# maxjaritz/mvpnet

Hardware: AMD Instinct MI355X
Metric: chunks/sec (8192 pts, 3x160x120 views) fwd+bwd (higher is better)
Workload: dtype f32; 1 GPU; configs[2]: MVPNet lifting (unproject + pixel k-NN + gather) + FeatureAggregation + PN2SSG full train step (fwd+loss+bwd+Adam), 2D CNN replaced by a resident 64-ch feature map; cfg=mvpnet_3d_unet_resnet34_pn2ssg.yaml, chunks_per_gpu=32, points=8192, views=3x160x120, feature_channels=64, k=3, parallelism=dp1 (one process per GPU, 1 grad all-reduce/step), launch=eager, cpu_affinity=32 logical cpus of 256 (0 .. 183)

## Files before the change

### include/mvp_hip.h

```cpp
#ifndef MVP_HIP_H_
#define MVP_HIP_H_

#include <stddef.h>
#include <stdint.h>

#ifdef __cplusplus
extern "C" {
#endif

typedef void* mvp_stream_t;

#define MVP_OK 0
#define MVP_EINVAL (-1)
#define MVP_EUNSUPPORTED (-2)
#define MVP_ENULL (-3)

const char* mvp_version(void);
const char* mvp_strerror(int code);

int mvp_set_fps_mode(int mode);

int mvp_fps_f32(const float* points, int64_t B, int64_t N, int64_t D, int64_t M, int64_t* index, mvp_stream_t stream);
int mvp_fps_f64(const double* points, int64_t B, int64_t N, int64_t D, int64_t M, int64_t* index, mvp_stream_t stream);
int mvp_fps_shape_f32(const float* points, int64_t B, int64_t N, int64_t D, int64_t M, int64_t* index, int shape, mvp_stream_t stream);
// ... 198 lines not shown
int mvp_gather_rows_backward_csr_f32(const float* grad_out, const int32_t* offsets, const int32_t* slots, const float* weight,
                                     int64_t B, int64_t N, int64_t C, int64_t E, int64_t S, int64_t ld, float* grad_feature,
                                     mvp_stream_t stream);
int mvp_gather_rows_backward_csr_finish_f32(const float* dz, const float* y, const float* mean, const float* invstd, const float* gamma,
                                            const double* stat, int training, const int32_t* offsets, const int32_t* slots, const float* weight,
                                            int64_t B, int64_t N, int64_t C, int64_t E, int64_t S, int64_t ld, float* grad_feature,
                                            mvp_stream_t stream);
int mvp_interp_add_rows_f32(const float* feature, const int64_t* index, const float* weight, const float* add, int64_t B, int64_t N1,
                            int64_t C, int64_t N2, float* out, double* stat, double* partial, mvp_stream_t stream);
int mvp_interp_add_rows_bn_f32(const float* feature, const int64_t* index, const float* weight, const float* add, int64_t B, int64_t N1,
                               int64_t C, int64_t N2, float* out, double* stat, double* partial, float eps, float momentum, float* mean,
                               float* invstd, float* running_mean, float* running_var, int64_t* num_batches_tracked, mvp_stream_t stream);
int mvp_interp_rows_backward_f32(const float* grad_out, const int64_t* index, const float* weight, int64_t B, int64_t N1,
                                 int64_t C, int64_t N2, int64_t ld, float* grad_feature, mvp_stream_t stream);
int mvp_bn_rows_forward_f32(const float* y, const float* gamma, const float* beta, int64_t G, int64_t K, int64_t C,
                            int training, float eps, float momentum, int relu, float* running_mean, float* running_var,
                            double* stat, float* mean, float* invstd, float* out, uint8_t* arg, double* partial,
                            mvp_stream_t stream);
int mvp_bn_rows_backward_f32(const float* dsrc, const float* out, const uint8_t* arg, const float* y, const float* mean,
                             const float* invstd, const float* gamma, const float* beta, int64_t G, int64_t K, int64_t C,
                             int relu, int training, double* stat, float* dy, float* dgamma, float* dbeta, double* partial,
                             mvp_stream_t stream);
int mvp_bn_rows_forward_dropout_f32(const float* y, const float* gamma, const float* beta, int64_t R, int64_t C, int training, float eps,
                                    float momentum, int relu, float* running_mean, float* running_var, double* stat, float* mean,
                                    float* invstd, float* out, double* partial, float drop_p, uint64_t seed, mvp_stream_t stream);
int mvp_bn_rows_backward_dropout_f32(const float* dsrc, const float* y, const float* mean, const float* invstd, const float* gamma,
                                     const float* beta, int64_t R, int64_t C, int relu, int training, double* stat, float* dy,
                                     float* dgamma, float* dbeta, double* partial, float drop_p, uint64_t seed, mvp_stream_t stream);
int mvp_bn_rows_backward_finish_f32(const float* dz, const float* y, const float* mean, const float* invstd,
                                    const float* gamma, const float* beta, int64_t R, int64_t C, int training,
                                    const double* stat, float* dy, float* dgamma, float* dbeta, mvp_stream_t stream);
int mvp_bn_finalize_f32(const double* stat, int64_t R, int64_t C, float eps, float momentum, float* mean, float* invstd,
                        float* running_mean, float* running_var, int64_t* num_batches_tracked, mvp_stream_t stream);
int mvp_sa_fused_forward_f32(const float* zf, const float* xyz, const float* centre, const int64_t* index, const float* wxyz, int64_t B,
                             int64_t N, int64_t M, int64_t K, int64_t C1, const float* bn1_mean, const float* bn1_invstd,
                             const float* bn1_gamma, const float* bn1_beta, const float* W2, int64_t C2, const float* bn2_mean,
                             const float* bn2_invstd, const float* bn2_gamma, const float* bn2_beta, const float* W3, int64_t C3,
                             const float* bn3_mean, const float* bn3_invstd, const float* bn3_gamma, const float* bn3_beta, float* out,
                             uint8_t* arg, mvp_stream_t stream);

int mvp_set_mlp_precision(int terms, int min_width);
int mvp_get_mlp_precision(void);
int mvp_set_mlp_precision_backward(int terms);
int mvp_get_mlp_precision_backward(void);
int mvp_mlp_precision_scope(int terms, int terms_backward);
int mvp_adam_step_f32(void* const* params, const void* const* grads, void* const* exp_avg, void* const* exp_avg_sq, const int64_t* numel,
                      int64_t n, double lr, double beta1, double beta2, double eps, double weight_decay, double step, mvp_stream_t stream);
int mvp_sgd_step_f32(void* const* params, const void* const* grads, void* const* momentum_buf, const int64_t* numel, const uint8_t* first,
                     int64_t n, double lr, double momentum, double dampening, double weight_decay, int nesterov, const float* grad_scale,
                     mvp_stream_t stream);
int64_t mvp_grad_clip_partials_count(const int64_t* numel, int64_t n);
int mvp_grad_sqnorm_partials_f32(const void* const* grads, const int64_t* numel, int64_t n, float* partials, int64_t* n_partials_out,
                                 mvp_stream_t stream);
int mvp_grad_clip_finish_f32(void* const* grads, const int64_t* numel, int64_t n, const float* partials, int64_t n_partials, double max_norm,
                             float* total_norm_out, float* coef_out, mvp_stream_t stream);

int mvp_mlp_forward_bf16(const uint16_t* X, int64_t R, int64_t Cin, int64_t ldx, const float* W, int64_t ldw, int64_t Cout,
                         const float* bias, const float* scale, const float* shift, int relu, uint16_t* Y, int64_t ldy,
                         mvp_stream_t stream);

int mvp_set_mlp_stream(int on);

int mvp_mlp_forward_f32(const float* X, int64_t R, int64_t Cin, int64_t ldx, const float* W, int64_t ldw, int64_t Cout,
                        const float* act_mean, const float* act_invstd, const float* act_gamma, const float* act_beta,
                        const float* bias, float* Y, double* stat, double* partial, mvp_stream_t stream);
int mvp_mlp_forward_bn_f32(const float* X, int64_t R, int64_t Cin, int64_t ldx, const float* W, int64_t ldw, int64_t Cout,
                           const float* act_mean, const float* act_invstd, const float* act_gamma, const float* act_beta, float* Y,
                           double* stat, double* partial, float eps, float momentum, float* mean, float* invstd, float* running_mean,
                           float* running_var, int64_t* num_batches_tracked, mvp_stream_t stream);
int mvp_mlp_forward_rel_bn_f32(const float* X, int64_t R, int64_t Cin, int64_t ldx, const float* W, int64_t ldw, int64_t Cout, const float* rel,
                               const float* wrel, float* Y, double* stat, double* partial, float eps, float momentum, float* mean,
                               float* invstd, float* running_mean, float* running_var, int64_t* num_batches_tracked, mvp_stream_t stream);
int mvp_relation4_rows_f32(const float* src_xyz, const float* tgt_xyz, int64_t R, int64_t K, float* out, mvp_stream_t stream);
int mvp_mlp_forward_pool_f32(const float* X, int64_t R, int64_t Cin, int64_t ldx, const float* W, int64_t ldw, int64_t Cout,
                             const float* act_mean, const float* act_invstd, const float* act_gamma, const float* act_beta, float* ymax,
                             float* ymin, uint8_t* amax, uint8_t* amin, double* stat, double* partial, float eps, float momentum,
                             float* mean, float* invstd, float* running_mean, float* running_var, int64_t* num_batches_tracked,
                             mvp_stream_t stream);
int mvp_pool_finalize_f32(const float* ymax, const float* ymin, const uint8_t* amax, const uint8_t* amin, const float* mean,
                          const float* invstd, const float* gamma, const float* beta, int64_t G, int64_t C, int relu, float* out,
                          uint8_t* arg, float* ysel, mvp_stream_t stream);
int mvp_pool_backward_stats_f32(const float* dout, const float* out, const float* ysel, const float* mean, const float* invstd,
                                int64_t G, int64_t C, int relu, double* stat, double* partial, mvp_stream_t stream);
int mvp_mlp_input_grad_f32(const float* dY, int64_t R, int64_t Cout, const float* W, int64_t Cin, const float* y_prev,
                           const float* mean, const float* invstd, const float* gamma, const float* beta, float* dZ,
                           double* stat, double* partial, mvp_stream_t stream);
int mvp_mlp_input_grad_dropout_f32(const float* dY, int64_t R, int64_t Cout, const float* W, int64_t Cin, const float* y_prev,
                                   const float* mean, const float* invstd, const float* gamma, const float* beta, float drop_p,
                                   uint64_t drop_seed, float* dZ, double* stat, double* partial, mvp_stream_t stream);

int64_t mvp_mlp_layer_backward_partial_count(int64_t R, int64_t Cp);
int mvp_mlp_layer_backward_f32(const float* G, const float* Yi, const float* mean_i, const float* invstd_i, const float* gamma_i,
                               const double* stat_i, float* dgamma_i, float* dbeta_i, int training, const float* X, int64_t ldx,
                               const float* act_mean, const float* act_invstd, const float* act_gamma, const float* act_beta,
                               const float* W, int64_t ldw, int64_t R, int64_t C, int64_t Cp, float* dW, int64_t lddw, float* dZ,
                               double* stat_prev, double* partial, const float* pool_dout, const float* pool_out,
                               const uint8_t* pool_arg, mvp_stream_t stream);
int mvp_mlp_layer_backward_ws_f32(const float* G, const float* Yi, const float* mean_i, const float* invstd_i, const float* gamma_i,
                               const double* stat_i, float* dgamma_i, float* dbeta_i, int training, const float* X, int64_t ldx,
                               const float* act_mean, const float* act_invstd, const float* act_gamma, const float* act_beta,
                               const float* W, int64_t ldw, int64_t R, int64_t C, int64_t Cp, float* dW, int64_t lddw, float* dZ,
                               double* stat_prev, double* partial, const float* pool_dout, const float* pool_out,
                               const uint8_t* pool_arg, float* workspace, int64_t workspace_floats, mvp_stream_t stream);
int mvp_mlp_layer_backward_wide_p_f32(const float* G, const float* Yi, const float* mean_i, const float* invstd_i, const float* gamma_i,
                                      const float* beta_i, const double* stat_i, float* dgamma_i, float* dbeta_i, int training, int mode,
                                      float drop_p, uint64_t drop_seed, const float* X, int64_t ldx, const float* act_mean,
                                      const float* act_invstd, const float* act_gamma, const float* act_beta, const float* W, int64_t ldw,
                                      int64_t R, int64_t C, int64_t Cp, float* dW, int64_t lddw, float* dZ, double* stat_prev, int* ticket,
                                      float* workspace, int64_t workspace_floats, int precision, int precision_backward, mvp_stream_t stream);
int mvp_mlp_layer_backward_wide_pooled_p_f32(const float* G, const float* Yi, const float* mean_i, const float* invstd_i, const float* gamma_i,
                                             const float* beta_i, const double* stat_i, float* dgamma_i, float* dbeta_i, int training, int mode,
                                             int64_t pool_k, float drop_p, uint64_t drop_seed, const float* X, int64_t ldx, const float* act_mean,
                                             const float* act_invstd, const float* act_gamma, const float* act_beta, const float* W, int64_t ldw,
                                             int64_t R, int64_t C, int64_t Cp, float* dW, int64_t lddw, float* dZ, double* stat_prev, int* ticket,
                                             float* workspace, int64_t workspace_floats, int precision, int precision_backward, mvp_stream_t stream);
int mvp_mlp_weight_grad_finish_p_f32(const float* dZ, const float* Y, const float* mean, const float* invstd, const float* gamma, const double* stat,
                                     int training, const float* X, int64_t R, int64_t Cout, int64_t Cin, int64_t ldx, float* dW, int64_t lddw,
                                     float* workspace, int64_t workspace_floats, int precision, int precision_backward, mvp_stream_t stream);
int mvp_mlp_weight_grad_finish_rel_p_f32(const float* dZ, const float* Y, const float* mean, const float* invstd, const float* gamma, const double* stat,
                                         int training, const float* X, int64_t R, int64_t Cout, int64_t Cin, int64_t ldx, const float* REL, float* dW,
                                         float* dWrel, int64_t lddw, int precision, int precision_backward, mvp_stream_t stream);
int mvp_mlp_weight_grad_finish_act_p_f32(const float* dZ, const float* Y, const float* mean, const float* invstd, const float* gamma, const double* stat,
                                         int training, const float* X, int64_t R, int64_t Cout, int64_t Cin, int64_t ldx, const float* act_mean,
                                         const float* act_invstd, const float* act_gamma, const float* act_beta, float* dW, int64_t lddw,
                                         float* workspace, int64_t workspace_floats, int precision, int precision_backward, mvp_stream_t stream);
int64_t mvp_mlp_input_grad_wide_workspace_bytes(int64_t C, int64_t Cp);
int mvp_mlp_input_grad_wide_p_f32(const float* G, const float* Yi, const float* mean_i, const float* invstd_i, const float* gamma_i,
                                  const double* stat_i, float* dgamma_i, float* dbeta_i, int training, const float* X, int64_t ldx,
                                  const float* act_mean, const float* act_invstd, const float* act_gamma, const float* act_beta, const float* W,
                                  int64_t ldw, int64_t R, int64_t C, int64_t Cp, float* dZ, double* stat_prev, void* workspace,
                                  int64_t workspace_bytes, int precision, int precision_backward, mvp_stream_t stream);
int mvp_mlp_weight_grad_f32(const float* dY, const float* X, int64_t R, int64_t Cout, int64_t Cin, int64_t ldx,
                            const float* act_mean, const float* act_invstd, const float* act_gamma, const float* act_beta,
                            float* dW, int64_t lddw, mvp_stream_t stream);
int64_t mvp_mlp_weight_grad_workspace_floats(void);
int mvp_mlp_weight_grad_ws_f32(const float* dY, const float* X, int64_t R, int64_t Cout, int64_t Cin, int64_t ldx,
                               const float* act_mean, const float* act_invstd, const float* act_gamma, const float* act_beta,
                               float* dW, int64_t lddw, float* workspace, int64_t workspace_floats, mvp_stream_t stream);

int mvp_sa_train_forward_f32(int stage, const float* zf, const float* xyz, const float* centre, const int64_t* index, const float* wxyz,
                             int64_t B, int64_t N, int64_t M, int64_t K, int64_t C1, const float* bn1_mean, const float* bn1_invstd,
                             const float* bn1_gamma, const float* bn1_beta, const float* W2, int64_t C2, const float* bn2_mean,
                             const float* bn2_invstd, const float* bn2_gamma, const float* bn2_beta, const float* W3, int64_t C3,
                             double* stat, float eps, float momentum, float* mean, float* invstd, float* running_mean,
                             float* running_var, int64_t* num_batches_tracked, float* ymax, float* ymin, uint8_t* amax, uint8_t* amin,
                             mvp_stream_t stream);
int mvp_sa_train_backward_f32(int layer, const float* zf, const float* xyz, const float* centre, const int64_t* index, const float* wxyz,
                              int64_t B, int64_t N, int64_t M, int64_t K, int64_t C1, const float* bn1_mean, const float* bn1_invstd,
                              const float* bn1_gamma, const float* bn1_beta, const float* W2, int64_t C2, const float* bn2_mean,
                              const float* bn2_invstd, const float* bn2_gamma, const float* bn2_beta, const float* W3, int64_t C3,
                              const float* mean_i, const float* invstd_i, const float* gamma_i, const double* stat_i, float* dgamma_i,
                              float* dbeta_i, int training, const float* G, const float* pool_dout, const float* pool_out,
                              const uint8_t* pool_arg, float* dW, int64_t lddw, float* dZ, double* stat_prev, float* tsum, mvp_stream_t stream);
int mvp_sa_train_backward1_f32(const float* dz1, const int32_t* offsets, const int32_t* slots, const float* zf, const float* dsum,
                               const float* wxyz, const float* tsum, const double* zsum, const double* gsum, int64_t B, int64_t N, int64_t M,
                               int64_t K, int64_t C1, const float* mean, const float* invstd, const float* gamma, const double* stat,
                               int training, float* dgamma, float* dbeta, float* gz, float* dWxyz, int64_t lddw, mvp_stream_t stream);
int mvp_sa_geom_sums_f32(const int32_t* offsets, const int32_t* slots, const float* xyz, const float* centre, int64_t B, int64_t N, int64_t M,
                         int64_t K, float* dsum, double* gsum, mvp_stream_t stream);
int mvp_sa_train_stats1_f32(const float* zf, const float* dsum, const float* wxyz, const double* gsum, int64_t B, int64_t N, int64_t M, int64_t K,
                            int64_t C1, double* stat, double* zsum, float eps, float momentum, float* mean, float* invstd, float* running_mean,
                            float* running_var, int64_t* num_batches_tracked, mvp_stream_t stream);
int mvp_sa_train_stats1_ws_f32(const float* zf, const float* dsum, const float* wxyz, const double* gsum, int64_t B, int64_t N, int64_t M, int64_t K,
                               int64_t C1, double* stat, double* zsum, float eps, float momentum, float* mean, float* invstd, float* running_mean,
                               float* running_var, int64_t* num_batches_tracked, double* scratch, int64_t scratch_doubles, mvp_stream_t stream);

int mvp_mlp_forward_p_f32(const float* X, int64_t R, int64_t Cin, int64_t ldx, const float* W, int64_t ldw, int64_t Cout, const
    float* act_mean, const float* act_invstd, const float* act_gamma, const float* act_beta, const float* bias, float* Y,
    double* stat, double* partial, int precision, int precision_backward, mvp_stream_t stream);
int mvp_mlp_forward_bn_p_f32(const float* X, int64_t R, int64_t Cin, int64_t ldx, const float* W, int64_t ldw, int64_t Cout,
    const float* act_mean, const float* act_invstd, const float* act_gamma, const float* act_beta, float* Y, double* stat,
    double* partial, float eps, float momentum, float* mean, float* invstd, float* running_mean, float* running_var, int64_t*
    num_batches_tracked, int precision, int precision_backward, mvp_stream_t stream);
int mvp_mlp_forward_rel_bn_p_f32(const float* X, int64_t R, int64_t Cin, int64_t ldx, const float* W, int64_t ldw, int64_t Cout,
    const float* rel, const float* wrel, float* Y, double* stat, double* partial, float eps, float momentum, float* mean, float*
    invstd, float* running_mean, float* running_var, int64_t* num_batches_tracked, int precision, int precision_backward,
    mvp_stream_t stream);
int mvp_mlp_forward_pool_p_f32(const float* X, int64_t R, int64_t Cin, int64_t ldx, const float* W, int64_t ldw, int64_t Cout,
    const float* act_mean, const float* act_invstd, const float* act_gamma, const float* act_beta, float* ymax, float* ymin,
    uint8_t* amax, uint8_t* amin, double* stat, double* partial, float eps, float momentum, float* mean, float* invstd, float*
    running_mean, float* running_var, int64_t* num_batches_tracked, int precision, int precision_backward, mvp_stream_t stream);
int mvp_mlp_input_grad_p_f32(const float* dY, int64_t R, int64_t Cout, const float* W, int64_t Cin, const float* y_prev, const
    float* mean, const float* invstd, const float* gamma, const float* beta, float* dZ, double* stat, double* partial, int
    precision, int precision_backward, mvp_stream_t stream);
int mvp_mlp_input_grad_dropout_p_f32(const float* dY, int64_t R, int64_t Cout, const float* W, int64_t Cin, const float* y_prev, const
    float* mean, const float* invstd, const float* gamma, const float* beta, float drop_p, uint64_t drop_seed, float* dZ, double* stat,
    double* partial, int precision, int precision_backward, mvp_stream_t stream);
int mvp_mlp_weight_grad_p_f32(const float* dY, const float* X, int64_t R, int64_t Cout, int64_t Cin, int64_t ldx, const float*
    act_mean, const float* act_invstd, const float* act_gamma, const float* act_beta, float* dW, int64_t lddw, int precision,
    int precision_backward, mvp_stream_t stream);
int mvp_mlp_weight_grad_ws_p_f32(const float* dY, const float* X, int64_t R, int64_t Cout, int64_t Cin, int64_t ldx, const
    float* act_mean, const float* act_invstd, const float* act_gamma, const float* act_beta, float* dW, int64_t lddw, float*
    workspace, int64_t workspace_floats, int precision, int precision_backward, mvp_stream_t stream);
int mvp_mlp_layer_backward_p_f32(const float* G, const float* Yi, const float* mean_i, const float* invstd_i, const float*
    gamma_i, const double* stat_i, float* dgamma_i, float* dbeta_i, int training, const float* X, int64_t ldx, const float*
    act_mean, const float* act_invstd, const float* act_gamma, const float* act_beta, const float* W, int64_t ldw, int64_t R,
    int64_t C, int64_t Cp, float* dW, int64_t lddw, float* dZ, double* stat_prev, double* partial, const float* pool_dout, const
    float* pool_out, const uint8_t* pool_arg, int precision, int precision_backward, mvp_stream_t stream);
int mvp_mlp_layer_backward_ws_p_f32(const float* G, const float* Yi, const float* mean_i, const float* invstd_i, const float*
    gamma_i, const double* stat_i, float* dgamma_i, float* dbeta_i, int training, const float* X, int64_t ldx, const float*
    act_mean, const float* act_invstd, const float* act_gamma, const float* act_beta, const float* W, int64_t ldw, int64_t R,
    int64_t C, int64_t Cp, float* dW, int64_t lddw, float* dZ, double* stat_prev, double* partial, const float* pool_dout, const
    float* pool_out, const uint8_t* pool_arg, float* workspace, int64_t workspace_floats, int precision, int precision_backward,
    mvp_stream_t stream);
int mvp_sa_fused_forward_p_f32(const float* zf, const float* xyz, const float* centre, const int64_t* index, const float* wxyz,
    int64_t B, int64_t N, int64_t M, int64_t K, int64_t C1, const float* bn1_mean, const float* bn1_invstd, const float*
    bn1_gamma, const float* bn1_beta, const float* W2, int64_t C2, const float* bn2_mean, const float* bn2_invstd, const float*
    bn2_gamma, const float* bn2_beta, const float* W3, int64_t C3, const float* bn3_mean, const float* bn3_invstd, const float*
    bn3_gamma, const float* bn3_beta, float* out, uint8_t* arg, int precision, int precision_backward, mvp_stream_t stream);

int mvp_sa_train_forward_p_f32(int stage, const float* zf, const float* xyz, const float* centre, const int64_t* index, const
    float* wxyz, int64_t B, int64_t N, int64_t M, int64_t K, int64_t C1, const float* bn1_mean, const float* bn1_invstd, const
    float* bn1_gamma, const float* bn1_beta, const float* W2, int64_t C2, const float* bn2_mean, const float* bn2_invstd, const
    float* bn2_gamma, const float* bn2_beta, const float* W3, int64_t C3, double* stat, float eps, float momentum, float* mean,
    float* invstd, float* running_mean, float* running_var, int64_t* num_batches_tracked, float* ymax, float* ymin, uint8_t*
    amax, uint8_t* amin, int precision, int precision_backward, mvp_stream_t stream);
int mvp_sa_train_backward_p_f32(int layer, const float* zf, const float* xyz, const float* centre, const int64_t* index, const
    float* wxyz, int64_t B, int64_t N, int64_t M, int64_t K, int64_t C1, const float* bn1_mean, const float* bn1_invstd, const
    float* bn1_gamma, const float* bn1_beta, const float* W2, int64_t C2, const float* bn2_mean, const float* bn2_invstd, const
    float* bn2_gamma, const float* bn2_beta, const float* W3, int64_t C3, const float* mean_i, const float* invstd_i, const
    float* gamma_i, const double* stat_i, float* dgamma_i, float* dbeta_i, int training, const float* G, const float* pool_dout,
    const float* pool_out, const uint8_t* pool_arg, float* dW, int64_t lddw, float* dZ, double* stat_prev, float* tsum, int precision, int
    precision_backward, mvp_stream_t stream);

int mvp_pn2_plan_f32(const float* xyz, int64_t B, int64_t N, int64_t levels, const int64_t* centroids, const float* radius,
                     const int64_t* neighbours, const int32_t* geom, int fps_shape, int flags, float knn_eps, void* const* buffers,
                     int64_t n_buffers, void* const* events, int* fps_status, mvp_stream_t stream);

int mvp_vote_accumulate_f32(const float* logit, int64_t ld_r, int64_t ld_c, const int64_t* chunk_ind, int64_t n,
                            int64_t C, float* sum, int32_t* count, mvp_stream_t stream);
int mvp_vote_gather_f32(const float* logit, int64_t ld_chunk, int64_t ld_r, int64_t ld_c, const int64_t* chunk_offsets, int64_t num_chunks,
                        const int32_t* point_offsets, const int32_t* point_slots, int64_t n_pts, int64_t C, float* sum, int32_t* count,
                        mvp_stream_t stream);
int mvp_vote_finish_f32(const float* sum, const int32_t* count, int64_t n_pts, int64_t C, float* mean, int64_t* label,
                        mvp_stream_t stream);
int64_t mvp_vote_nearest_workspace(int64_t V, int64_t nb);
int mvp_vote_nearest_f32(const float* points, int64_t n, const float* key, int64_t V, int64_t nb, const float* logit, int64_t ld_vote,
                         int64_t ld_r, int64_t ld_c, int64_t C, float* sum, int64_t* nn_index, int32_t* swept, void* workspace,
                         int64_t workspace_bytes, mvp_stream_t stream);

int mvp_seg_loss_f32(const float* logit, int64_t B, int64_t C, int64_t N, int64_t ld_b, int64_t ld_c, int64_t ld_n,
                     const int64_t* label, const float* weight, int64_t ignore_index, double* acc, float* loss, mvp_stream_t stream);
int mvp_seg_loss_backward_f32(const float* logit, int64_t B, int64_t C, int64_t N, int64_t ld_b, int64_t ld_c, int64_t ld_n,
                              const int64_t* label, const float* weight, int64_t ignore_index, const double* acc,
                              const float* grad_out, float* grad_logit, int64_t gld_b, int64_t gld_c, int64_t gld_n,
                              mvp_stream_t stream);
int mvp_seg_confusion_f32(const float* logit, int64_t B, int64_t C, int64_t N, int64_t ld_b, int64_t ld_c, int64_t ld_n,
                          const int64_t* label, int64_t ignore_index, int64_t* mat, mvp_stream_t stream);

#ifdef __cplusplus
}
#endif
#endif
```

### mvpnet_amd/_lib.py

```python
import ctypes
import os

import torch

_HERE = os.path.dirname(os.path.abspath(__file__))
LIB_PATH = os.environ.get('MVP_LIBRARY') or os.path.join(_HERE, 'libmvp_hip.so')
_lib = None
MLP_PRECISIONS = {'fp32': 0, 'bf16': 1, 'bf16x3': 3, 'bf16x6': 6}

_i64 = ctypes.c_int64
_ptr = ctypes.c_void_p
_f32 = ctypes.c_float

_SIGNATURES = {
    'mvp_fps_f32': [_ptr, _i64, _i64, _i64, _i64, _ptr, _ptr],
    'mvp_fps_f64': [_ptr, _i64, _i64, _i64, _i64, _ptr, _ptr],
    'mvp_fps_shape_f32': [_ptr, _i64, _i64, _i64, _i64, _ptr, ctypes.c_int, _ptr],
    'mvp_fps_shape_f64': [_ptr, _i64, _i64, _i64, _i64, _ptr, ctypes.c_int, _ptr],
    'mvp_fps_checked_f32': [_ptr, _i64, _i64, _i64, _i64, _ptr, ctypes.c_int, _ptr, _ptr],
    'mvp_fps_centroid_levels_f32': [_ptr, _ptr, _i64, _i64, _i64, _i64, _i64, _ptr, _ptr, _ptr],
    'mvp_ball_query_f32': [_ptr, _ptr, _i64, _i64, _i64, _f32, _i64, _ptr, _ptr],
    'mvp_ball_query_f64': [_ptr, _ptr, _i64, _i64, _i64, _f32, _i64, _ptr, _ptr],
    'mvp_ball_query_distance_f32': [_ptr, _ptr, _i64, _i64, _i64, _f32, _i64, _ptr, _ptr, _ptr],
    'mvp_ball_query_distance_f64': [_ptr, _ptr, _i64, _i64, _i64, _f32, _i64, _ptr, _ptr, _ptr],
    'mvp_ball_query_grid_f32': [_ptr, _ptr, _i64, _i64, _i64, _f32, _i64, _ptr, _ptr, _ptr, _i64, _ptr],
    'mvp_knn3_grid_f32': [_ptr, _ptr, _i64, _i64, _i64, _f32, _ptr, _ptr, _ptr, _ptr, _i64, _ptr],
    'mvp_group_points_forward_strided_f32': [_ptr, _i64, _i64, _i64, _ptr, _i64, _i64, _i64, _i64, _i64, _ptr, _ptr],
    'mvp_group_points_backward_strided_f32': [_ptr, _i64, _i64, _i64, _i64, _ptr, _i64, _i64, _i64, _i64, _i64, _ptr, _ptr],
    'mvp_interpolate_forward_strided_f32': [_ptr, _i64, _i64, _i64, _ptr, _ptr, _i64, _i64, _i64, _i64, _ptr, _ptr],
    'mvp_interpolate_backward_strided_f32': [_ptr, _i64, _i64, _i64, _ptr, _ptr, _i64, _i64, _i64, _i64, _ptr, _ptr],
    'mvp_group_points_forward_strided_f64': [_ptr, _i64, _i64, _i64, _ptr, _i64, _i64, _i64, _i64, _i64, _ptr, _ptr],
    'mvp_group_points_forward_strided_bf16': [_ptr, _i64, _i64, _i64, _ptr, _i64, _i64, _i64, _i64, _i64, _ptr, _ptr],
    'mvp_group_points_backward_strided_f64': [_ptr, _i64, _i64, _i64, _i64, _ptr, _i64, _i64, _i64, _i64, _i64, _ptr, _ptr],
    'mvp_group_points_backward_strided_bf16': [_ptr, _i64, _i64, _i64, _i64, _ptr, _i64, _i64, _i64, _i64, _i64, _ptr, _ptr],
    'mvp_interpolate_forward_strided_f64': [_ptr, _i64, _i64, _i64, _ptr, _ptr, _i64, _i64, _i64, _i64, _ptr, _ptr],
    'mvp_interpolate_forward_strided_bf16': [_ptr, _i64, _i64, _i64, _ptr, _ptr, _i64, _i64, _i64, _i64, _ptr, _ptr],
    'mvp_interpolate_backward_strided_f64': [_ptr, _i64, _i64, _i64, _ptr, _ptr, _i64, _i64, _i64, _i64, _ptr, _ptr],
    'mvp_interpolate_backward_strided_bf16': [_ptr, _i64, _i64, _i64, _ptr, _ptr, _i64, _i64, _i64, _i64, _ptr, _ptr],
    'mvp_group_points_forward_f32': [_ptr, _ptr, _i64, _i64, _i64, _i64, _i64, _ptr, _ptr],
    'mvp_group_points_forward_f64': [_ptr, _ptr, _i64, _i64, _i64, _i64, _i64, _ptr, _ptr],
    'mvp_group_points_forward_bf16': [_ptr, _ptr, _i64, _i64, _i64, _i64, _i64, _ptr, _ptr],
    'mvp_group_points_backward_f32': [_ptr, _ptr, _i64, _i64, _i64, _i64, _i64, _ptr, _ptr],
    'mvp_group_points_backward_f64': [_ptr, _ptr, _i64, _i64, _i64, _i64, _i64, _ptr, _ptr],
    'mvp_group_points_backward_bf16': [_ptr, _ptr, _i64, _i64, _i64, _i64, _i64, _ptr, _ptr],
    'mvp_knn_distance_f32': [_ptr, _ptr, _i64, _i64, _i64, _i64, _ptr, _ptr, _ptr],
    'mvp_knn_distance_f64': [_ptr, _ptr, _i64, _i64, _i64, _i64, _ptr, _ptr, _ptr],
    'mvp_knn3_weights_f32': [_ptr, _ptr, _i64, _i64, _i64, _f32, _ptr, _ptr, _ptr, _ptr],
    'mvp_interpolate_forward_f32': [_ptr, _ptr, _ptr, _i64, _i64, _i64, _i64, _ptr, _ptr],
    'mvp_interpolate_forward_f64': [_ptr, _ptr, _ptr, _i64, _i64, _i64, _i64, _ptr, _ptr],
    'mvp_interpolate_forward_bf16': [_ptr, _ptr, _ptr, _i64, _i64, _i64, _i64, _ptr, _ptr],
    'mvp_interpolate_backward_f32': [_ptr, _ptr, _ptr, _i64, _i64, _i64, _i64, _ptr, _ptr],
    'mvp_interpolate_backward_f64': [_ptr, _ptr, _ptr, _i64, _i64, _i64, _i64, _ptr, _ptr],
    'mvp_interpolate_backward_bf16': [_ptr, _ptr, _ptr, _i64, _i64, _i64, _i64, _ptr, _ptr],
    'mvp_unproject_f32': [_ptr, _ptr, _ptr, _ptr, _i64, _i64, _i64, _i64, _ptr, _ptr, _ptr],
    'mvp_unproject_u16': [_ptr, _ptr, _ptr, _ptr, _i64, _i64, _i64, _i64, _ptr, _ptr, _ptr],
    'mvp_pixel_knn_bruteforce_f32': [_ptr, _ptr, _ptr, _i64, _i64, _i64, _i64, _ptr, _ptr, _ptr],
    'mvp_pixel_knn_projective_f32': [_ptr, _ptr, _ptr, _ptr, _ptr, _i64, _i64, _i64, _i64, _i64, _i64, _ptr, _ptr, _ptr],
    'mvp_lift_gather_f32': [_ptr, _ptr, _ptr, _i64, _i64, _i64, _i64, _i64, _ptr, _ptr, _ptr],
    'mvp_lift_gather_backward_f32': [_ptr, _ptr, _i64, _i64, _i64, _i64, _i64, _ptr, _ptr],
    'mvp_lift_f32': [_ptr, ctypes.c_int, _ptr, _ptr, _ptr, _ptr, _ptr, _ptr, _i64, _i64, _i64, _i64, _i64, _i64, _i64, _ptr,
                     _ptr, _ptr, _ptr, _ptr, _ptr, _ptr],
    'mvp_lift_aug_f32': [_ptr, ctypes.c_int, _ptr, _ptr, _ptr, _ptr, _ptr, _ptr, _i64, _i64, _i64, _i64, _i64, _i64, _i64, _ptr,
                         _ptr, _ptr, _ptr, _ptr, _ptr, _ptr, _ptr, _ptr, _ptr],
    'mvp_rotate_rows_f32': [_ptr, _ptr, _i64, _i64, _ptr, _ptr],
    'mvp_copy_slices_f32': [_ptr, _i64, _ptr],
    'mvp_group_rows_f32': [_ptr, _ptr, _ptr, _ptr, _i64, _i64, _i64, _i64, _i64, _i64, _ptr, _ptr],
    'mvp_group_rows_backward_f32': [_ptr, _ptr, _i64, _i64, _i64, _i64, _i64, _i64, _ptr, _ptr],
    'mvp_group_lin_rows_f32': [_ptr, _ptr, _ptr, _ptr, _ptr, _i64, _i64, _i64, _i64, _i64, _ptr, _ptr, _ptr, _ptr, _ptr],
    'mvp_group_lin_rows_bn_f32': [_ptr, _ptr, _ptr, _ptr, _ptr, _i64, _i64, _i64, _i64, _i64, _ptr, _ptr, _ptr, _ptr, _f32, _f32, _ptr, _ptr, _ptr, _ptr, _ptr, _ptr],
    'mvp_colstats_f32': [_ptr, _i64, _i64, _ptr, _ptr, _ptr],
    'mvp_relation_rows_f32': [_ptr, _ptr, _ptr, _i64, _i64, _i64, _ptr, _ptr],
    'mvp_interp_rows_f32': [_ptr, _ptr, _ptr, _i64, _i64, _i64, _i64, _i64, _ptr, _ptr],
    'mvp_mlp_forward_bf16': [_ptr, _i64, _i64, _i64, _ptr, _i64, _i64, _ptr, _ptr, _ptr, ctypes.c_int, _ptr, _i64, _ptr],
    'mvp_adam_step_f32': [_ptr, _ptr, _ptr, _ptr, _ptr, _i64] + [ctypes.c_double] * 6 + [_ptr],
    'mvp_sgd_step_f32': [_ptr, _ptr, _ptr, _ptr, _ptr, _i64] + [ctypes.c_double] * 4 + [ctypes.c_int, _ptr, _ptr],
    'mvp_grad_sqnorm_partials_f32': [_ptr, _ptr, _i64, _ptr, _ptr, _ptr],
    'mvp_grad_clip_finish_f32': [_ptr, _ptr, _i64, _ptr, _i64, ctypes.c_double, _ptr, _ptr, _ptr],
    'mvp_csr_build_i64': [_ptr, _i64, _i64, _i64, _ptr, _ptr, _ptr, _ptr],
    'mvp_csr_build_sorted_i64': [_ptr, _i64, _i64, _i64, _ptr, _ptr, _ptr, _ptr],
    'mvp_gather_rows_backward_csr_f32': [_ptr, _ptr, _ptr, _ptr, _i64, _i64, _i64, _i64, _i64, _i64, _ptr, _ptr],
    'mvp_gather_rows_backward_csr_finish_f32': [_ptr, _ptr, _ptr, _ptr, _ptr, _ptr, ctypes.c_int, _ptr, _ptr, _ptr, _i64, _i64, _i64, _i64, _i64, _i64, _ptr, _ptr],
    'mvp_interp_add_rows_f32': [_ptr, _ptr, _ptr, _ptr, _i64, _i64, _i64, _i64, _ptr, _ptr, _ptr, _ptr],
    'mvp_interp_add_rows_bn_f32': [_ptr, _ptr, _ptr, _ptr, _i64, _i64, _i64, _i64, _ptr, _ptr, _ptr, _f32, _f32, _ptr, _ptr, _ptr, _ptr, _ptr, _ptr],
    'mvp_interp_rows_backward_f32': [_ptr, _ptr, _ptr, _i64, _i64, _i64, _i64, _i64, _ptr, _ptr],
    'mvp_bn_rows_forward_f32': [_ptr, _ptr, _ptr, _i64, _i64, _i64, ctypes.c_int, _f32, _f32, ctypes.c_int, _ptr, _ptr, _ptr, _ptr,
                                _ptr, _ptr, _ptr, _ptr, _ptr],
    'mvp_bn_rows_backward_f32': [_ptr, _ptr, _ptr, _ptr, _ptr, _ptr, _ptr, _ptr, _i64, _i64, _i64, ctypes.c_int, ctypes.c_int, _ptr,
                                 _ptr, _ptr, _ptr, _ptr, _ptr],
    'mvp_bn_rows_forward_dropout_f32': [_ptr, _ptr, _ptr, _i64, _i64, ctypes.c_int, _f32, _f32, ctypes.c_int, _ptr, _ptr, _ptr, _ptr, _ptr, _ptr,
                                        _ptr, _f32, ctypes.c_uint64, _ptr],
    'mvp_bn_rows_backward_dropout_f32': [_ptr, _ptr, _ptr, _ptr, _ptr, _ptr, _i64, _i64, ctypes.c_int, ctypes.c_int, _ptr, _ptr, _ptr, _ptr,
                                         _ptr, _f32, ctypes.c_uint64, _ptr],
    'mvp_bn_rows_backward_finish_f32': [_ptr, _ptr, _ptr, _ptr, _ptr, _ptr, _i64, _i64, ctypes.c_int, _ptr, _ptr, _ptr, _ptr, _ptr],
    'mvp_bn_finalize_f32': [_ptr, _i64, _i64, _f32, _f32, _ptr, _ptr, _ptr, _ptr, _ptr, _ptr],
    'mvp_mlp_weight_grad_f32': [_ptr, _ptr, _i64, _i64, _i64, _i64, _ptr, _ptr, _ptr, _ptr, _ptr, _i64, _ptr],
    'mvp_mlp_weight_grad_ws_f32': [_ptr, _ptr, _i64, _i64, _i64, _i64, _ptr, _ptr, _ptr, _ptr, _ptr, _i64, _ptr, _i64, _ptr],
    'mvp_mlp_input_grad_f32': [_ptr, _i64, _i64, _ptr, _i64, _ptr, _ptr, _ptr, _ptr, _ptr, _ptr, _ptr, _ptr, _ptr],
    'mvp_mlp_input_grad_dropout_f32': [_ptr, _i64, _i64, _ptr, _i64, _ptr, _ptr, _ptr, _ptr, _ptr, _f32, ctypes.c_uint64, _ptr, _ptr, _ptr, _ptr],
    'mvp_mlp_layer_backward_f32': [_ptr, _ptr, _ptr, _ptr, _ptr, _ptr, _ptr, _ptr, ctypes.c_int, _ptr, _i64, _ptr, _ptr, _ptr, _ptr, _ptr, _i64,
                                   _i64, _i64, _i64, _ptr, _i64, _ptr, _ptr, _ptr, _ptr, _ptr, _ptr, _ptr],
    'mvp_mlp_layer_backward_ws_f32': [_ptr, _ptr, _ptr, _ptr, _ptr, _ptr, _ptr, _ptr, ctypes.c_int, _ptr, _i64, _ptr, _ptr, _ptr, _ptr, _ptr, _i64,
                                   _i64, _i64, _i64, _ptr, _i64, _ptr, _ptr, _ptr, _ptr, _ptr, _ptr, _ptr, _i64, _ptr],
    'mvp_mlp_forward_pool_f32': [_ptr, _i64, _i64, _i64, _ptr, _i64, _i64, _ptr, _ptr, _ptr, _ptr, _ptr, _ptr, _ptr, _ptr, _ptr, _ptr, _f32, _f32,
                                 _ptr, _ptr, _ptr, _ptr, _ptr, _ptr],
    'mvp_pool_finalize_f32': [_ptr, _ptr, _ptr, _ptr, _ptr, _ptr, _ptr, _ptr, _i64, _i64, ctypes.c_int, _ptr, _ptr, _ptr, _ptr],
    'mvp_pool_backward_stats_f32': [_ptr, _ptr, _ptr, _ptr, _ptr, _i64, _i64, ctypes.c_int, _ptr, _ptr, _ptr],
    'mvp_sa_fused_forward_f32': [_ptr, _ptr, _ptr, _ptr, _ptr, _i64, _i64, _i64, _i64, _i64, _ptr, _ptr, _ptr, _ptr, _ptr, _i64, _ptr, _ptr, _ptr,
                                 _ptr, _ptr, _i64, _ptr, _ptr, _ptr, _ptr, _ptr, _ptr, _ptr],
    'mvp_sa_train_forward_f32': [ctypes.c_int, _ptr, _ptr, _ptr, _ptr, _ptr, _i64, _i64, _i64, _i64, _i64, _ptr, _ptr, _ptr, _ptr, _ptr, _i64, _ptr, _ptr,
                                 _ptr, _ptr, _ptr, _i64, _ptr, _f32, _f32, _ptr, _ptr, _ptr, _ptr, _ptr, _ptr, _ptr, _ptr, _ptr, _ptr],
    'mvp_sa_train_backward_f32': [ctypes.c_int, _ptr, _ptr, _ptr, _ptr, _ptr, _i64, _i64, _i64, _i64, _i64, _ptr, _ptr, _ptr, _ptr, _ptr, _i64, _ptr, _ptr,
                                  _ptr, _ptr, _ptr, _i64, _ptr, _ptr, _ptr, _ptr, _ptr, _ptr, ctypes.c_int, _ptr, _ptr, _ptr, _ptr, _ptr, _i64, _ptr, _ptr,
                                  _ptr, _ptr],
    'mvp_sa_train_backward1_f32': [_ptr, _ptr, _ptr, _ptr, _ptr, _ptr, _ptr, _ptr, _ptr, _i64, _i64, _i64, _i64, _i64, _ptr, _ptr, _ptr, _ptr,
                                   ctypes.c_int, _ptr, _ptr, _ptr, _ptr, _i64, _ptr],
    'mvp_pn2_plan_f32': [_ptr, _i64, _i64, _i64, _ptr, _ptr, _ptr, _ptr, ctypes.c_int, ctypes.c_int, _f32, _ptr, _i64, _ptr, _ptr, _ptr],
    'mvp_sa_geom_sums_f32': [_ptr, _ptr, _ptr, _ptr, _i64, _i64, _i64, _i64, _ptr, _ptr, _ptr],
    'mvp_sa_train_stats1_f32': [_ptr, _ptr, _ptr, _ptr, _i64, _i64, _i64, _i64, _i64, _ptr, _ptr, _f32, _f32, _ptr, _ptr, _ptr, _ptr, _ptr, _ptr],
    'mvp_sa_train_stats1_ws_f32': [_ptr, _ptr, _ptr, _ptr, _i64, _i64, _i64, _i64, _i64, _ptr, _ptr, _f32, _f32, _ptr, _ptr, _ptr, _ptr, _ptr, _ptr, _i64, _ptr],
    'mvp_mlp_forward_bn_f32': [_ptr, _i64, _i64, _i64, _ptr, _i64, _i64, _ptr, _ptr, _ptr, _ptr, _ptr, _ptr, _ptr, _f32, _f32, _ptr, _ptr, _ptr,
                               _ptr, _ptr, _ptr],
    'mvp_mlp_forward_rel_bn_f32': [_ptr, _i64, _i64, _i64, _ptr, _i64, _i64, _ptr, _ptr, _ptr, _ptr, _ptr, _f32, _f32, _ptr, _ptr, _ptr, _ptr, _ptr, _ptr],
    'mvp_relation4_rows_f32': [_ptr, _ptr, _i64, _i64, _ptr, _ptr],
    'mvp_mlp_forward_f32': [_ptr, _i64, _i64, _i64, _ptr, _i64, _i64, _ptr, _ptr, _ptr, _ptr, _ptr, _ptr, _ptr, _ptr, _ptr],
    'mvp_vote_accumulate_f32': [_ptr, _i64, _i64, _ptr, _i64, _i64, _ptr, _ptr, _ptr],
    'mvp_vote_gather_f32': [_ptr, _i64, _i64, _i64, _ptr, _i64, _ptr, _ptr, _i64, _i64, _ptr, _ptr, _ptr],
    'mvp_vote_finish_f32': [_ptr, _ptr, _i64, _i64, _ptr, _ptr, _ptr],
    'mvp_vote_nearest_f32': [_ptr, _i64, _ptr, _i64, _i64, _ptr, _i64, _i64, _i64, _i64, _ptr, _ptr, _ptr, _ptr, _i64, _ptr],
    'mvp_seg_loss_f32': [_ptr, _i64, _i64, _i64, _i64, _i64, _i64, _ptr, _ptr, _i64, _ptr, _ptr, _ptr],
    'mvp_seg_loss_backward_f32': [_ptr, _i64, _i64, _i64, _i64, _i64, _i64, _ptr, _ptr, _i64, _ptr, _ptr, _ptr, _i64, _i64, _i64, _ptr],
    'mvp_seg_confusion_f32': [_ptr, _i64, _i64, _i64, _i64, _i64, _i64, _ptr, _i64, _ptr, _ptr],
    'mvp_frame_overlap_f32': [_ptr, _ptr, _ptr, _ptr, _i64, _i64, _i64, _i64, _f32, _ptr, _ptr],
    'mvp_frame_overlap_u16': [_ptr, _ptr, _ptr, _ptr, _i64, _i64, _i64, _i64, _f32, _ptr, _ptr],
    'mvp_select_frames_u32': [_ptr, _ptr, _i64, _i64, _i64, _i64, _ptr, _ptr, _ptr],
    'mvp_select_frames_ranges_u32': [_ptr, _ptr, _ptr, _ptr, _i64, _i64, _i64, _i64, _ptr, _ptr, _ptr],
    'mvp_sample_chunks_f32': [_ptr] * 6 + [_i64] * 6 + [ctypes.c_double] * 5 + [ctypes.c_int, ctypes.c_uint64] + [_ptr] * 9 + [_i64, _ptr],
    'mvp_sample_scenes_f32': [_ptr, _ptr] + [_i64] * 4 + [ctypes.c_uint64] + [_ptr] * 4 + [_i64, _ptr],
    'mvp_gather_cloud_f32': [_ptr] * 7 + [_i64] * 4 + [_ptr] * 4,
    'mvp_scene_chunks_count_f32': [_ptr, _i64, _ptr, _i64] + [ctypes.c_double] * 4 + [_ptr, _ptr, _ptr],
    'mvp_scene_chunks_fill_f32': [_ptr, _i64, _ptr, _i64] + [ctypes.c_double] * 4 + [_ptr, _ptr, _i64, _ptr, _i64, _ptr, _i64, _ptr, _ptr, _ptr],
    'mvp_pack_chunks_f32': [_ptr, _i64, _ptr, _i64, _ptr, _i64, _ptr, _ptr, _ptr, _ptr, ctypes.c_uint64, _ptr, _i64, _ptr],
    'mvp_prepare_frames_u8': [_ptr, _i64, _i64, _i64, _ptr, _i64, _ptr, _ptr, _ptr, _ptr, ctypes.c_int, _ptr, _ptr, _ptr],
    'mvp_resize_bilinear_table': [_i64, _i64, _ptr, _ptr, _ptr, _ptr],
    'mvp_resize_nearest_table': [_i64, _i64, _ptr],
    'mvp_resize_frames_u8': [_ptr, _i64, _i64, _i64, _ptr, _i64, _i64, _i64, _ptr, _ptr, _ptr, _ptr],
    'mvp_prepare_labels_u16': [_ptr, _i64, _i64, _i64, _ptr, _i64, _i64, _i64, _ptr, _ptr, _ptr, _ptr, _i64, _i64, _ptr, _ptr],
}
for _n in ['mvp_mlp_forward_f32', 'mvp_mlp_forward_bn_f32', 'mvp_mlp_forward_rel_bn_f32', 'mvp_mlp_forward_pool_f32', 'mvp_mlp_input_grad_f32', 'mvp_mlp_input_grad_dropout_f32',
           'mvp_mlp_weight_grad_f32', 'mvp_mlp_weight_grad_ws_f32', 'mvp_mlp_layer_backward_f32', 'mvp_mlp_layer_backward_ws_f32',
           'mvp_sa_fused_forward_f32', 'mvp_sa_train_forward_f32', 'mvp_sa_train_backward_f32']:
    _SIGNATURES[_n[:-4] + '_p_f32'] = _SIGNATURES[_n][:-1] + [ctypes.c_int, ctypes.c_int, _ptr]
_SIGNATURES['mvp_mlp_layer_backward_wide_p_f32'] = [_ptr] * 9 + [ctypes.c_int, ctypes.c_int, _f32, ctypes.c_uint64, _ptr, _i64, _ptr, _ptr, _ptr, _ptr, _ptr, _i64,
                                                    _i64, _i64, _i64, _ptr, _i64, _ptr, _ptr, _ptr, _ptr, _i64, ctypes.c_int, ctypes.c_int, _ptr]
_SIGNATURES['mvp_mlp_layer_backward_wide_pooled_p_f32'] = [_ptr] * 9 + [ctypes.c_int, ctypes.c_int, _i64, _f32, ctypes.c_uint64, _ptr, _i64, _ptr, _ptr, _ptr, _ptr, _ptr, _i64,
                                                           _i64, _i64, _i64, _ptr, _i64, _ptr, _ptr, _ptr, _ptr, _i64, ctypes.c_int, ctypes.c_int, _ptr]
_SIGNATURES['mvp_mlp_weight_grad_finish_p_f32'] = [_ptr] * 6 + [ctypes.c_int, _ptr, _i64, _i64, _i64, _i64, _ptr, _i64, _ptr, _i64, ctypes.c_int, ctypes.c_int, _ptr]
_SIGNATURES['mvp_mlp_weight_grad_finish_rel_p_f32'] = [_ptr] * 6 + [ctypes.c_int, _ptr, _i64, _i64, _i64, _i64, _ptr, _ptr, _ptr, _i64, ctypes.c_int, ctypes.c_int, _ptr]
_SIGNATURES['mvp_mlp_weight_grad_finish_act_p_f32'] = [_ptr] * 6 + [ctypes.c_int, _ptr, _i64, _i64, _i64, _i64, _ptr, _ptr, _ptr, _ptr, _ptr, _i64, _ptr, _i64, ctypes.c_int,
                                                        ctypes.c_int, _ptr]
_SIGNATURES['mvp_mlp_input_grad_wide_p_f32'] = [_ptr] * 8 + [ctypes.c_int, _ptr, _i64, _ptr, _ptr, _ptr, _ptr, _ptr, _i64, _i64, _i64, _i64, _ptr, _ptr, _ptr, _i64,
                                                 ctypes.c_int, ctypes.c_int, _ptr]
EXPORTS = ['mvp_version', 'mvp_strerror', 'mvp_lift_workspace_bytes', 'mvp_ball_query_grid_workspace', 'mvp_knn3_grid_workspace', 'mvp_vote_nearest_workspace', 'mvp_sample_chunks_workspace', 'mvp_sample_scenes_workspace', 'mvp_prepare_frames_workspace', 'mvp_mlp_weight_grad_workspace_floats', 'mvp_mlp_input_grad_wide_workspace_bytes', 'mvp_group_lin_partial_count', 'mvp_colstats_partial_count', 'mvp_grad_clip_partials_count',
           'mvp_set_mlp_precision', 'mvp_get_mlp_precision', 'mvp_mlp_layer_backward_partial_count', 'mvp_set_mlp_stream', 'mvp_set_mlp_precision_backward', 'mvp_get_mlp_precision_backward', 'mvp_mlp_precision_scope', 'mvp_set_fps_mode', 'mvp_fps_debug_spin_limit', 'mvp_fps_last_kernel'] + sorted(_SIGNATURES)


def lib():
    global _lib
    if _lib is None:
        if not os.path.exists(LIB_PATH):
            raise RuntimeError('libmvp_hip.so is not built: run `python -c "import __graft_entry__ as g; g.build()"` '
                               'or `make -C mvpnet_amd/csrc` ({})'.format(LIB_PATH))
        handle = ctypes.CDLL(LIB_PATH)
        handle.mvp_version.restype = ctypes.c_char_p
        handle.mvp_strerror.restype = ctypes.c_char_p
        handle.mvp_strerror.argtypes = [ctypes.c_int]
        handle.mvp_lift_workspace_bytes.restype = ctypes.c_int64
        handle.mvp_lift_workspace_bytes.argtypes = [_i64, _i64, _i64, _i64, _i64]
        handle.mvp_ball_query_grid_workspace.restype = ctypes.c_int64
        handle.mvp_ball_query_grid_workspace.argtypes = [_i64, _i64, _i64]
        handle.mvp_knn3_grid_workspace.restype = ctypes.c_int64
        handle.mvp_knn3_grid_workspace.argtypes = [_i64, _i64, _i64]
        handle.mvp_vote_nearest_workspace.restype = ctypes.c_int64
        handle.mvp_vote_nearest_workspace.argtypes = [_i64, _i64]
        handle.mvp_sample_chunks_workspace.restype = ctypes.c_int64
        handle.mvp_sample_chunks_workspace.argtypes = [_i64, _i64, _i64, _i64]
        handle.mvp_sample_scenes_workspace.restype = ctypes.c_int64
        handle.mvp_sample_scenes_workspace.argtypes = [_i64, _i64, _i64]
        handle.mvp_prepare_frames_workspace.restype = ctypes.c_size_t
        handle.mvp_prepare_frames_workspace.argtypes = [_i64]
        handle.mvp_group_lin_partial_count.restype = ctypes.c_int64
        handle.mvp_group_lin_partial_count.argtypes = [_i64, _i64, _i64, _i64]
        handle.mvp_mlp_weight_grad_workspace_floats.restype = ctypes.c_int64
        handle.mvp_mlp_weight_grad_workspace_floats.argtypes = []
        handle.mvp_mlp_input_grad_wide_workspace_bytes.restype = ctypes.c_int64
        handle.mvp_mlp_input_grad_wide_workspace_bytes.argtypes = [ctypes.c_int64, ctypes.c_int64]
        handle.mvp_colstats_partial_count.restype = ctypes.c_int64
        handle.mvp_colstats_partial_count.argtypes = [_i64, _i64]
        handle.mvp_grad_clip_partials_count.restype = ctypes.c_int64
        handle.mvp_grad_clip_partials_count.argtypes = [_ptr, _i64]
        handle.mvp_set_mlp_precision.restype = ctypes.c_int
        handle.mvp_set_mlp_precision.argtypes = [ctypes.c_int, ctypes.c_int]
        handle.mvp_get_mlp_precision.restype = ctypes.c_int
        handle.mvp_get_mlp_precision.argtypes = []
        handle.mvp_mlp_layer_backward_partial_count.restype = ctypes.c_int64
        handle.mvp_mlp_layer_backward_partial_count.argtypes = [_i64, _i64]
        for name, argtypes in _SIGNATURES.items():
            fn = getattr(handle, name)
            fn.argtypes = argtypes
            fn.restype = ctypes.c_int
        _lib = handle
        handle.mvp_set_mlp_stream.restype = ctypes.c_int
        handle.mvp_set_mlp_stream.argtypes = [ctypes.c_int]
        handle.mvp_set_fps_mode.restype = ctypes.c_int
        handle.mvp_set_fps_mode.argtypes = [ctypes.c_int]
        handle.mvp_fps_debug_spin_limit.restype = ctypes.c_int
        handle.mvp_fps_debug_spin_limit.argtypes = [ctypes.c_int]
        handle.mvp_fps_last_kernel.restype = ctypes.c_int
        handle.mvp_fps_last_kernel.argtypes = []
        if os.environ.get('MVP_MLP_STREAM') is not None:
            handle.mvp_set_mlp_stream(int(os.environ['MVP_MLP_STREAM']))
        handle.mvp_set_mlp_precision_backward.restype = ctypes.c_int
        handle.mvp_set_mlp_precision_backward.argtypes = [ctypes.c_int]
        handle.mvp_get_mlp_precision_backward.restype = ctypes.c_int
        handle.mvp_get_mlp_precision_backward.argtypes = []
        handle.mvp_mlp_precision_scope.restype = ctypes.c_int
        handle.mvp_mlp_precision_scope.argtypes = [ctypes.c_int, ctypes.c_int]
        if os.environ.get('MVP_MLP_PRECISION_BWD'):
            check(handle.mvp_set_mlp_precision_backward(MLP_PRECISIONS[os.environ['MVP_MLP_PRECISION_BWD']]), 'mvp_set_mlp_precision_backward')
        env = os.environ.get('MVP_MLP_PRECISION')
        if env:
            set_mlp_precision(env, int(os.environ.get('MVP_MLP_MIN_WIDTH', '0')))
    return _lib




def set_mlp_precision(name, min_width=0):
    if name not in MLP_PRECISIONS:
        raise ValueError('mlp precision must be one of {}'.format(sorted(MLP_PRECISIONS)))
    check(lib().mvp_set_mlp_precision(MLP_PRECISIONS[name], int(min_width)), 'mvp_set_mlp_precision')
    global _mlp_min_width
    _mlp_min_width = int(min_width)


_mlp_min_width = 0


def mlp_min_width():
    return _mlp_min_width


def set_mlp_precision_backward(name):
    if name not in ('bf16', 'bf16x3', 'bf16x6'):
        raise ValueError("backward mlp precision must be 'bf16', 'bf16x3' or 'bf16x6'")
    check(lib().mvp_set_mlp_precision_backward(MLP_PRECISIONS[name]), 'mvp_set_mlp_precision_backward')


class mlp_precision:

    def __init__(self, forward=None, backward=None):
        self.terms = -1 if forward is None else MLP_PRECISIONS[forward]
        self.bwd = -1 if backward is None else MLP_PRECISIONS[backward]
        if self.bwd == 0:
            raise ValueError("backward mlp precision must be 'bf16', 'bf16x3' or 'bf16x6'")

    def __enter__(self):
        old = lib().mvp_mlp_precision_scope(self.terms, self.bwd)
        if old < 0:
            check(old, 'mvp_mlp_precision_scope')
        self.old = (old // 16 - 1, old % 16 - 1)
        return self

    def __exit__(self, *exc):
        lib().mvp_mlp_precision_scope(*self.old)


def current_precision():
    h = lib()
    return (h.mvp_get_mlp_precision(), h.mvp_get_mlp_precision_backward())


def get_mlp_precision():
    terms = lib().mvp_get_mlp_precision()
    return {v: k for k, v in MLP_PRECISIONS.items()}[terms]


_FPS_STATUS = {}


def fps_status(device):
    t = _FPS_STATUS.get(device)
    if t is None:
        t = _FPS_STATUS[device] = torch.zeros(1, dtype=torch.int32, device=device)
    return t


def fps_timed_out(device=None, reset=False):
    device = torch.device('cuda', torch.cuda.current_device()) if device is None else torch.device(device)
    t = _FPS_STATUS.get(device)
    if t is None:
        return False
    hit = bool(int(t.item()))
    if reset:
        t.zero_()
    return hit


def check(code, what):
    if code != 0:
        raise RuntimeError('{} failed: {} (code {})'.format(what, lib().mvp_strerror(code).decode(), code))


def stream_of(t):
    return ctypes.c_void_p(torch.cuda.current_stream(t.device).cuda_stream)


def ptr(t):
    return None if t is None else t.data_ptr()


def ptr_at(t, element_offset):
    return t.data_ptr() + int(element_offset) * t.element_size()


def require_gpu(*tensors):
    for t in tensors:
        if t is None:
            continue
        if not t.is_cuda:
            raise RuntimeError('mvpnet_amd ops run on the GPU only (got a {} tensor); there is no CPU fallback'.format(t.device))
        if not t.is_contiguous():
            raise RuntimeError('tensor must be contiguous')


def suffix(t):
    if t.dtype == torch.float32:
        return 'f32'
    if t.dtype == torch.float64:
        return 'f64'
    raise RuntimeError('expected a float32 or float64 tensor, got {}'.format(t.dtype))


def value_suffix(t):
    return 'bf16' if t.dtype == torch.bfloat16 else suffix(t)


_FN = {}
_raw_stream = getattr(torch._C, '_cuda_getCurrentRawStream', None)
_raw_device = getattr(torch._C, '_cuda_getDevice', None)


def _fn(name):
    f = _FN.get(name)
    if f is None:
        f = _FN[name] = getattr(_lib if _lib is not None else lib(), name)
    return f


DW_WORKSPACE = os.environ.get('MVP_DETERMINISTIC', '0') == '1'


def set_deterministic(flag):
    global DW_WORKSPACE
    old, DW_WORKSPACE = DW_WORKSPACE, bool(flag)
    return old


_DW_WS = {}
_DW_WS_NAMES = {'mvp_mlp_weight_grad_f32': 'mvp_mlp_weight_grad_ws_f32', 'mvp_mlp_layer_backward_f32': 'mvp_mlp_layer_backward_ws_f32'}


def dw_workspace(index, stream_handle):
    ws = _DW_WS.get((index, stream_handle))
    if ws is None:
        ws = _DW_WS[(index, stream_handle)] = torch.empty(lib().mvp_mlp_weight_grad_workspace_floats(), dtype=torch.float32,
                                                          device=torch.device('cuda', index))
    return ws


def current_dw_workspace(device):
    if not DW_WORKSPACE:
        return None, 0
    index = device.index
    handle = _raw_stream(index) if (_raw_stream is not None and index == _raw_device()) else torch.cuda.current_stream(device).cuda_stream
    ws = dw_workspace(index, handle)
    return ws.data_ptr(), ws.numel()


def _with_dw_workspace(index, stream_handle, args):
    ws = dw_workspace(index, stream_handle)
    return args + (ws.data_ptr(), ws.numel())


def call_on(stream, name, *args, prec=None):
    if DW_WORKSPACE and name in _DW_WS_NAMES:
        name, args = _DW_WS_NAMES[name], _with_dw_workspace(stream.device.index, stream.cuda_stream, args)
    if prec is not None:
        name, args = name[:-4] + '_p_f32', args + prec
    code = _fn(name)(*args, stream.cuda_stream)
    if code != 0:
        check(code, name)


def call(name, tensor_for_device, *args, prec=None):
    index = tensor_for_device.device.index
    if DW_WORKSPACE and name in _DW_WS_NAMES:
        handle = _raw_stream(index) if _raw_stream is not None else torch.cuda.current_stream(tensor_for_device.device).cuda_stream
        name, args = _DW_WS_NAMES[name], _with_dw_workspace(index, handle, args)
    if prec is not None:
        name, args = name[:-4] + '_p_f32', args + prec
    if _raw_stream is not None and index == _raw_device():
        code = _fn(name)(*args, _raw_stream(index))
    elif index == torch.cuda.current_device():
        code = _fn(name)(*args, torch.cuda.current_stream(tensor_for_device.device).cuda_stream)
    else:
        with torch.cuda.device(tensor_for_device.device):
            code = _fn(name)(*args, stream_of(tensor_for_device))
    if code != 0:
        check(code, name)
```

### mvpnet_amd/csrc/mlp_prec.hip

```cpp
#include "mlp_common.h"

namespace {
struct PrecisionArg {
  int old_terms, old_bwd;
  bool ok;
  PrecisionArg(int terms, int bwd) : old_terms(tl_mlp_terms), old_bwd(tl_mlp_terms_bwd) {
    ok = (terms == -1 || terms == 0 || terms == 1 || terms == 3 || terms == 6) && (bwd == -1 || bwd == 1 || bwd == 3 || bwd == 6);
    if (ok && terms >= 0) tl_mlp_terms = terms;
    if (ok && bwd >= 0) tl_mlp_terms_bwd = bwd;
  }
  ~PrecisionArg() {
    tl_mlp_terms = old_terms;
    tl_mlp_terms_bwd = old_bwd;
  }
};
}

#define MVP_WITH_PRECISION(call)             \
  PrecisionArg scope(precision, precision_backward); \
  if (!scope.ok) return MVP_EINVAL;          \
  return call

MVP_API int mvp_mlp_forward_p_f32(const float* X, int64_t R, int64_t Cin, int64_t ldx, const float* W, int64_t ldw, int64_t Cout,
                                  const float* act_mean, const float* act_invstd, const float* act_gamma, const float* act_beta,
                                  const float* bias, float* Y, double* stat, double* partial, int precision, int precision_backward,
                                  mvp_stream_t stream) {
  MVP_WITH_PRECISION(mvp_mlp_forward_f32(X, R, Cin, ldx, W, ldw, Cout, act_mean, act_invstd, act_gamma, act_beta, bias, Y, stat, partial, stream));
}
MVP_API int mvp_mlp_forward_bn_p_f32(const float* X, int64_t R, int64_t Cin, int64_t ldx, const float* W, int64_t ldw, int64_t Cout,
                                     const float* act_mean, const float* act_invstd, const float* act_gamma, const float* act_beta, float* Y,
                                     double* stat, double* partial, float eps, float momentum, float* mean, float* invstd,
                                     float* running_mean, float* running_var, int64_t* num_batches_tracked, int precision,
                                     int precision_backward, mvp_stream_t stream) {
  MVP_WITH_PRECISION(mvp_mlp_forward_bn_f32(X, R, Cin, ldx, W, ldw, Cout, act_mean, act_invstd, act_gamma, act_beta, Y, stat, partial, eps, momentum,
                                            mean, invstd, running_mean, running_var, num_batches_tracked, stream));
}
MVP_API int mvp_mlp_forward_rel_bn_p_f32(const float* X, int64_t R, int64_t Cin, int64_t ldx, const float* W, int64_t ldw, int64_t Cout,
                                         const float* rel, const float* wrel, float* Y, double* stat, double* partial, float eps, float momentum,
                                         float* mean, float* invstd, float* running_mean, float* running_var, int64_t* num_batches_tracked,
                                         int precision, int precision_backward, mvp_stream_t stream) {
  MVP_WITH_PRECISION(mvp_mlp_forward_rel_bn_f32(X, R, Cin, ldx, W, ldw, Cout, rel, wrel, Y, stat, partial, eps, momentum, mean, invstd, running_mean,
                                                running_var, num_batches_tracked, stream));
}
MVP_API int mvp_mlp_forward_pool_p_f32(const float* X, int64_t R, int64_t Cin, int64_t ldx, const float* W, int64_t ldw, int64_t Cout,
                                       const float* act_mean, const float* act_invstd, const float* act_gamma, const float* act_beta,
                                       float* ymax, float* ymin, uint8_t* amax, uint8_t* amin, double* stat, double* partial, float eps,
                                       float momentum, float* mean, float* invstd, float* running_mean, float* running_var,
                                       int64_t* num_batches_tracked, int precision, int precision_backward, mvp_stream_t stream) {
  MVP_WITH_PRECISION(mvp_mlp_forward_pool_f32(X, R, Cin, ldx, W, ldw, Cout, act_mean, act_invstd, act_gamma, act_beta, ymax, ymin, amax, amin, stat,
                                              partial, eps, momentum, mean, invstd, running_mean, running_var, num_batches_tracked, stream));
}
MVP_API int mvp_mlp_input_grad_p_f32(const float* dY, int64_t R, int64_t Cout, const float* W, int64_t Cin, const float* y_prev,
                                     const float* mean, const float* invstd, const float* gamma, const float* beta, float* dZ, double* stat,
                                     double* partial, int precision, int precision_backward, mvp_stream_t stream) {
  MVP_WITH_PRECISION(mvp_mlp_input_grad_f32(dY, R, Cout, W, Cin, y_prev, mean, invstd, gamma, beta, dZ, stat, partial, stream));
}
MVP_API int mvp_mlp_input_grad_dropout_p_f32(const float* dY, int64_t R, int64_t Cout, const float* W, int64_t Cin, const float* y_prev,
                                             const float* mean, const float* invstd, const float* gamma, const float* beta, float drop_p,
                                             uint64_t drop_seed, float* dZ, double* stat, double* partial, int precision, int precision_backward,
                                             mvp_stream_t stream) {
  MVP_WITH_PRECISION(mvp_mlp_input_grad_dropout_f32(dY, R, Cout, W, Cin, y_prev, mean, invstd, gamma, beta, drop_p, drop_seed, dZ, stat, partial, stream));
}
MVP_API int mvp_mlp_weight_grad_p_f32(const float* dY, const float* X, int64_t R, int64_t Cout, int64_t Cin, int64_t ldx,
                                      const float* act_mean, const float* act_invstd, const float* act_gamma, const float* act_beta,
                                      float* dW, int64_t lddw, int precision, int precision_backward, mvp_stream_t stream) {
  MVP_WITH_PRECISION(mvp_mlp_weight_grad_f32(dY, X, R, Cout, Cin, ldx, act_mean, act_invstd, act_gamma, act_beta, dW, lddw, stream));
}
MVP_API int mvp_mlp_weight_grad_ws_p_f32(const float* dY, const float* X, int64_t R, int64_t Cout, int64_t Cin, int64_t ldx,
                                         const float* act_mean, const float* act_invstd, const float* act_gamma, const float* act_beta,
                                         float* dW, int64_t lddw, float* workspace, int64_t workspace_floats, int precision,
                                         int precision_backward, mvp_stream_t stream) {
  MVP_WITH_PRECISION(mvp_mlp_weight_grad_ws_f32(dY, X, R, Cout, Cin, ldx, act_mean, act_invstd, act_gamma, act_beta, dW, lddw, workspace,
                                                workspace_floats, stream));
}
MVP_API int mvp_mlp_layer_backward_p_f32(const float* G, const float* Yi, const float* mean_i, const float* invstd_i, const float* gamma_i,
                                         const double* stat_i, float* dgamma_i, float* dbeta_i, int training, const float* X, int64_t ldx,
                                         const float* act_mean, const float* act_invstd, const float* act_gamma, const float* act_beta,
                                         const float* W, int64_t ldw, int64_t R, int64_t C, int64_t Cp, float* dW, int64_t lddw, float* dZ,
                                         double* stat_prev, double* partial, const float* pool_dout, const float* pool_out,
                                         const uint8_t* pool_arg, int precision, int precision_backward, mvp_stream_t stream) {
  MVP_WITH_PRECISION(mvp_mlp_layer_backward_f32(G, Yi, mean_i, invstd_i, gamma_i, stat_i, dgamma_i, dbeta_i, training, X, ldx, act_mean, act_invstd,
                                                act_gamma, act_beta, W, ldw, R, C, Cp, dW, lddw, dZ, stat_prev, partial, pool_dout,
                                                    pool_out, pool_arg,
                                                stream));
}
MVP_API int mvp_mlp_layer_backward_ws_p_f32(const float* G, const float* Yi, const float* mean_i, const float* invstd_i, const float* gamma_i,
                                            const double* stat_i, float* dgamma_i, float* dbeta_i, int training, const float* X, int64_t ldx,
                                            const float* act_mean, const float* act_invstd, const float* act_gamma, const float* act_beta,
                                            const float* W, int64_t ldw, int64_t R, int64_t C, int64_t Cp, float* dW, int64_t lddw, float* dZ,
                                            double* stat_prev, double* partial, const float* pool_dout, const float* pool_out,
                                            const uint8_t* pool_arg, float* workspace, int64_t workspace_floats, int precision,
                                            int precision_backward, mvp_stream_t stream) {
  MVP_WITH_PRECISION(mvp_mlp_layer_backward_ws_f32(G, Yi, mean_i, invstd_i, gamma_i, stat_i, dgamma_i, dbeta_i, training, X, ldx, act_mean,
      act_invstd,
                                                   act_gamma, act_beta, W, ldw, R, C, Cp, dW, lddw, dZ, stat_prev, partial, pool_dout, pool_out,
                                                   pool_arg, workspace, workspace_floats, stream));
}
MVP_API int mvp_sa_fused_forward_p_f32(const float* zf, const float* xyz, const float* centre, const int64_t* index, const float* wxyz,
                                       int64_t B, int64_t N, int64_t M, int64_t K, int64_t C1, const float* bn1_mean, const float* bn1_invstd,
                                       const float* bn1_gamma, const float* bn1_beta, const float* W2, int64_t C2, const float* bn2_mean,
                                       const float* bn2_invstd, const float* bn2_gamma, const float* bn2_beta, const float* W3, int64_t C3,
                                       const float* bn3_mean, const float* bn3_invstd, const float* bn3_gamma, const float* bn3_beta,
                                       float* out, uint8_t* arg, int precision, int precision_backward, mvp_stream_t stream) {
  MVP_WITH_PRECISION(mvp_sa_fused_forward_f32(zf, xyz, centre, index, wxyz, B, N, M, K, C1, bn1_mean, bn1_invstd, bn1_gamma, bn1_beta, W2,
      C2, bn2_mean,
                                              bn2_invstd, bn2_gamma, bn2_beta, W3, C3, bn3_mean, bn3_invstd, bn3_gamma, bn3_beta, out, arg, stream));
}
MVP_API int mvp_sa_train_forward_p_f32(int stage, const float* zf, const float* xyz, const float* centre, const int64_t* index, const float*
    wxyz, int64_t B, int64_t N, int64_t M, int64_t K, int64_t C1, const float* bn1_mean, const float* bn1_invstd, const float* bn1_gamma,
    const float* bn1_beta, const float* W2, int64_t C2, const float* bn2_mean, const float* bn2_invstd, const float* bn2_gamma, const float*
    bn2_beta, const float* W3, int64_t C3, double* stat, float eps, float momentum, float* mean, float* invstd, float* running_mean, float*
    running_var, int64_t* num_batches_tracked, float* ymax, float* ymin, uint8_t* amax, uint8_t* amin, int precision, int
    precision_backward, mvp_stream_t stream) {
  MVP_WITH_PRECISION(mvp_sa_train_forward_f32(stage, zf, xyz, centre, index, wxyz, B, N, M, K, C1, bn1_mean, bn1_invstd, bn1_gamma,
      bn1_beta, W2, C2, bn2_mean, bn2_invstd, bn2_gamma, bn2_beta, W3, C3, stat, eps, momentum, mean, invstd, running_mean, running_var,
      num_batches_tracked, ymax, ymin, amax, amin, stream));
}

MVP_API int mvp_sa_train_backward_p_f32(int layer, const float* zf, const float* xyz, const float* centre, const int64_t* index, const
    float* wxyz, int64_t B, int64_t N, int64_t M, int64_t K, int64_t C1, const float* bn1_mean, const float* bn1_invstd, const float*
    bn1_gamma, const float* bn1_beta, const float* W2, int64_t C2, const float* bn2_mean, const float* bn2_invstd, const float* bn2_gamma,
    const float* bn2_beta, const float* W3, int64_t C3, const float* mean_i, const float* invstd_i, const float* gamma_i, const double*
    stat_i, float* dgamma_i, float* dbeta_i, int training, const float* G, const float* pool_dout, const float* pool_out, const uint8_t*
    pool_arg, float* dW, int64_t lddw, float* dZ, double* stat_prev, float* tsum, int precision, int precision_backward, mvp_stream_t stream) {
  MVP_WITH_PRECISION(mvp_sa_train_backward_f32(layer, zf, xyz, centre, index, wxyz, B, N, M, K, C1, bn1_mean, bn1_invstd, bn1_gamma,
      bn1_beta, W2, C2, bn2_mean, bn2_invstd, bn2_gamma, bn2_beta, W3, C3, mean_i, invstd_i, gamma_i, stat_i, dgamma_i, dbeta_i, training,
      G, pool_dout, pool_out, pool_arg, dW, lddw, dZ, stat_prev, tsum, stream));
}
```

### mvpnet_amd/csrc/sa_common.h

```cpp
#pragma once
#include "mlp_common.h"
#include <algorithm>
#include <climits>

namespace {

constexpr int kFT = 256;
constexpr int kFLd = 36;

__device__ __forceinline__ constexpr int acc_row(int q, int h) { return (q & 3) + 8 * (q >> 2) + 4 * h; }

template <int NS>
__device__ __forceinline__ void stage_weight(unsigned char* Wl, const float* __restrict__ W, int Cout, int Cin, int cols, int slabs, int tid) {
  for (int t = tid; t < cols * slabs * 8; t += kFT) {
    const int co = t % cols, kqi = t / cols;
    const int k = 4 * kqi;
    float v[4];
#pragma unroll
    for (int e = 0; e < 4; ++e) v[e] = (co < Cout && k + e < Cin) ? W[(size_t)co * Cin + k + e] : 0.f;
    unsigned lo[NS], hi[NS];
    split_pair<NS>(v[0], v[1], lo);
    split_pair<NS>(v[2], v[3], hi);
    const int slab = kqi >> 3, kq = (kqi & 7) * 4;
    const int tt = kq >> 3, hh = (kq >> 2) & 1;
// ... 71 lines not shown

template <int C1B>
struct BallRows {
  float4 z[C1B][4];
  float p[3], q[3];
  bool ok;
};
template <int C1B, bool NOZF = false>
__device__ __forceinline__ void gather_issue(const SaSrc& p, int g, int64_t j, int lh, BallRows<C1B>& r) {
  const int b = g / p.M;
  r.ok = j >= 0 && j < p.N;
  const unsigned jj = r.ok ? (unsigned)j : 0u;
  if (!NOZF || p.zf) {
    const float* zr = p.zf + (size_t)b * p.N * p.C1 + jj * (unsigned)p.C1;
#pragma unroll
    for (int sl = 0; sl < C1B; ++sl)
#pragma unroll
      for (int tt = 0; tt < 4; ++tt) r.z[sl][tt] = *reinterpret_cast<const float4*>(zr + min(32 * sl + 8 * tt + 4 * lh, p.C1 - 4));
  }
  const float* pp = p.xyz + (size_t)b * p.N * 3 + jj * 3u;
  const float* qc = p.centre + (size_t)g * 3;
  r.p[0] = pp[0]; r.p[1] = pp[1]; r.p[2] = pp[2];
  r.q[0] = qc[0]; r.q[1] = qc[1]; r.q[2] = qc[2];
}
template <int C1B>
__device__ __forceinline__ void gather_finish(const BallRows<C1B>& r, int lh, const float (*Wx)[4], float (&v)[C1B][4][4], float (&diff)[3]) {
  const bool ok = r.ok;
  const float dx = r.p[0] - r.q[0], dy = r.p[1] - r.q[1], dz = r.p[2] - r.q[2];
  diff[0] = ok ? dx : 0.f;
  diff[1] = ok ? dy : 0.f;
  diff[2] = ok ? dz : 0.f;
#pragma unroll
  for (int sl = 0; sl < C1B; ++sl)
#pragma unroll
    for (int tt = 0; tt < 4; ++tt) {
      const int k = 32 * sl + 8 * tt + 4 * lh;
      const float zz[4] = {r.z[sl][tt].x, r.z[sl][tt].y, r.z[sl][tt].z, r.z[sl][tt].w};
#pragma unroll
      for (int e = 0; e < 4; ++e) {
        const float4 w = *reinterpret_cast<const float4*>(&Wx[k + e][0]);
        float y = (w.x * dx + w.y * dy) + w.z * dz;
        y = y + zz[e];
        v[sl][tt][e] = ok ? y : 0.f;
      }
    }
}

template <int C1B, bool PF, bool NOZF = false>
struct BallPipe {
  BallRows<C1B> rn;
  int64_t jn;
  int64_t t_end;
  __device__ __forceinline__ int begin(const SaSrc& p, int64_t tiles_per_wg, int wave, int li, int lh) {
    const int64_t t_begin = (int64_t)blockIdx.x * tiles_per_wg;
    t_end = min(p.G, t_begin + tiles_per_wg);
    const int g = __builtin_amdgcn_readfirstlane((int)(t_begin + wave));
    jn = -1;
    if (PF) {
      if (g < t_end) gather_issue<C1B, NOZF>(p, g, p.index[(size_t)g * 32 + li], lh, rn);
      if (g + 4 < t_end) jn = p.index[(size_t)(g + 4) * 32 + li];
    } else if (g < t_end) {
      jn = p.index[(size_t)g * 32 + li];
    }
    return g;
  }
  __device__ __forceinline__ void rows(const SaSrc& p, int g, int li, int lh, BallRows<C1B>& rc) {
    if (PF) {
      rc = rn;
      if (g + 4 < t_end) {
        gather_issue<C1B, NOZF>(p, g + 4, jn, lh, rn);
        if (g + 8 < t_end) jn = p.index[(size_t)(g + 8) * 32 + li];
      }
    } else {
      const int64_t j = jn;
      if (g + 4 < t_end) jn = p.index[(size_t)(g + 4) * 32 + li];
      gather_issue<C1B, NOZF>(p, g, j, lh, rc);
    }
  }
};

template <int C1B>
__device__ __forceinline__ void act_rows(float (&v)[C1B][4][4], const float* P1, int lh) {
#pragma unroll
  for (int sl = 0; sl < C1B; ++sl)
#pragma unroll
    for (int tt = 0; tt < 4; ++tt) {
      const int k = 32 * sl + 8 * tt + 4 * lh;
      const float4 mm = *reinterpret_cast<const float4*>(P1 + 0 * (C1B * 32) + k), ii = *reinterpret_cast<const float4*>(P1 + 1 * (C1B * 32) + k);
      const float4 gg = *reinterpret_cast<const float4*>(P1 + 2 * (C1B * 32) + k), bb = *reinterpret_cast<const float4*>(P1 + 3 * (C1B * 32) + k);
      const float pm[4] = {mm.x, mm.y, mm.z, mm.w}, pi[4] = {ii.x, ii.y, ii.z, ii.w};
      const float pg[4] = {gg.x, gg.y, gg.z, gg.w}, pb[4] = {bb.x, bb.y, bb.z, bb.w};
#pragma unroll
      for (int e = 0; e < 4; ++e) {
        const float a = ((v[sl][tt][e] - pm[e]) * pi[e]) * pg[e] + pb[e];
        v[sl][tt][e] = a > 0.f ? a : 0.f;
      }
    }
}

template <int NB>
struct LaneBn {
  float m[NB], i[NB], g[NB], b[NB];
  __device__ __forceinline__ void load(const float* const (&bn)[4], int C, int li) {
#pragma unroll
    for (int j = 0; j < NB; ++j) {
      const int col = min(32 * j + li, C - 1);
      m[j] = bn[0][col]; i[j] = bn[1][col]; g[j] = bn[2][col]; b[j] = bn[3][col];
    }
  }
  __device__ __forceinline__ float act(int j, float y) const {
    const float a = ((y - m[j]) * i[j]) * g[j] + b[j];
    return a > 0.f ? a : 0.f;
  }
};

template <int NB>
__device__ __forceinline__ void act_tile_rows(const f32x16 (&acc)[NB], const LaneBn<NB>& bn, float* st, int li, int lh, float (&v)[NB][4][4]) {
#pragma unroll
  for (int jb = 0; jb < NB; ++jb) {
#pragma unroll
    for (int i = 0; i < 16; ++i) st[acc_row(i, lh) * kFLd + li] = bn.act(jb, acc[jb][i]);
    __builtin_amdgcn_wave_barrier();
#pragma unroll
    for (int tt = 0; tt < 4; ++tt) {
      const float4 a = *reinterpret_cast<const float4*>(st + li * kFLd + 8 * tt + 4 * lh);
      v[jb][tt][0] = a.x; v[jb][tt][1] = a.y; v[jb][tt][2] = a.z; v[jb][tt][3] = a.w;
    }
    __builtin_amdgcn_wave_barrier();
  }
}

template <int NS>
__device__ __forceinline__ void tile_row_frags(const float* tile, int c, int h, int s, u32x4 (&f)[NS]) {
  const float4 v0 = *reinterpret_cast<const float4*>(tile + c * kFLd + 16 * s + 4 * h);
  const float4 v1 = *reinterpret_cast<const float4*>(tile + c * kFLd + 16 * s + 8 + 4 * h);
  unsigned q0[NS], q1[NS], q2[NS], q3[NS];
  split_pair<NS>(v0.x, v0.y, q0);
  split_pair<NS>(v0.z, v0.w, q1);
  split_pair<NS>(v1.x, v1.y, q2);
  split_pair<NS>(v1.z, v1.w, q3);
#pragma unroll
  for (int pc = 0; pc < NS; ++pc) f[pc] = u32x4{q0[pc], q1[pc], q2[pc], q3[pc]};
}

inline int blocks_of(int64_t c) { return c <= 32 ? 1 : c <= 64 ? 2 : 4; }

struct SaLevel {
  SaSrc s;
  int c1b, c2b, c3b;
};

inline int sa_level(const float* zf, bool zf_required, const float* xyz, const float* centre, const int64_t* index, const float* wxyz, int64_t B,
                    int64_t N, int64_t M, int64_t K, int64_t C1, const float* const (&bn1)[4], const float* W2, int64_t C2, int64_t C3,
                    bool own_sizes, bool own_ok, SaLevel* lv) {
  if (zf_required) MVP_NONNULL(zf);
  MVP_NONNULL(xyz);
  MVP_NONNULL(centre);
  MVP_NONNULL(index);
  MVP_NONNULL(wxyz);
  for (const float* q : bn1) MVP_NONNULL(q);
  MVP_NONNULL(W2);
  MVP_REQUIRE(B >= 0 && N > 0 && M >= 0 && K > 0 && C1 > 0 && C2 > 0 && C3 >= 0 && own_sizes);
  const bool widths = K == 32 && C1 >= 4 && C1 <= 64 && C2 <= 64 && C3 <= 128 && C1 % 4 == 0 && C2 % 4 == 0 && C3 % 4 == 0;
  if (!own_ok || !widths) return MVP_EUNSUPPORTED;
  constexpr int64_t kBalls = (int64_t(1) << 31) - 16, kOffsets = (int64_t(1) << 32) - 1;
  if (N > INT_MAX || M > INT_MAX || (M > 0 && B > kBalls / M) || N > kOffsets / std::max<int64_t>(C1, 3)) return MVP_EUNSUPPORTED;
  lv->s = SaSrc{zf, xyz, centre, index, wxyz, {bn1[0], bn1[1], bn1[2], bn1[3]}, B * M, (int)N, (int)M, (int)C1};
  lv->c1b = blocks_of(C1); lv->c2b = blocks_of(C2); lv->c3b = C3 ? blocks_of(C3) : 1;
  return MVP_OK;
}

template <int... V>
struct SaRow { static constexpr int v[sizeof...(V)] = {V...}; };
template <class... Rows>
struct SaTable {};
template <int... V>
inline bool sa_row_is(SaRow<V...>, const int (&key)[sizeof...(V)]) {
  int i = 0;
  return ((key[i++] == V) && ...);
}
template <class... Rows, int N, class F>
inline bool sa_pick(SaTable<Rows...>, const int (&key)[N], F&& f) {
  return ((sa_row_is(Rows{}, key) ? (f(Rows{}), true) : false) || ...);
}
using SaShapes3 = SaTable<SaRow<1, 1, 1>, SaRow<1, 1, 2>, SaRow<1, 2, 1>, SaRow<1, 2, 2>, SaRow<2, 1, 1>, SaRow<2, 1, 2>, SaRow<2, 2, 1>, SaRow<2, 2, 2>,
                          SaRow<2, 2, 4>>;
using SaShapes2 = SaTable<SaRow<1, 1, 1>, SaRow<1, 2, 1>, SaRow<2, 1, 1>, SaRow<2, 2, 1>>;
using SaPieces = SaTable<SaRow<1>, SaRow<2>, SaRow<3>>;

inline unsigned sa_grid(int64_t G, int64_t lds_bytes, int64_t max_per_cu, int64_t max_wgs, int64_t* tiles_per_wg) {
  const int64_t per_cu = std::max<int64_t>(1, std::min<int64_t>(max_per_cu, (150 * 1024) / lds_bytes));
  const int64_t wgs = std::max<int64_t>(1, std::min<int64_t>(std::min<int64_t>(max_wgs, 256 * per_cu), cdiv(G, 16)));
  *tiles_per_wg = cdiv(cdiv(G, wgs), 4) * 4;
  return (unsigned)cdiv(G, *tiles_per_wg);
}

}
```

### mvpnet_amd/csrc/sa_train.hip

```cpp
#include "sa_common.h"
#include "stats_reduce.h"
#include <algorithm>
#include <stdlib.h>

namespace {

template <int NB>
__device__ __forceinline__ void stats_tail(const float (&ssum)[NB], const float (&qsum)[NB], double (*sred)[4][NB * 32], double* stat, int C,
                                           const BnFinalize& fin, bool finalize) {
  const int tid = threadIdx.x, lane = tid & 63, wave = tid >> 6, li = lane & 31;
#pragma unroll
  for (int j = 0; j < NB; ++j) {
    const float s = ssum[j] + __shfl_xor(ssum[j], 32, kWave), q = qsum[j] + __shfl_xor(qsum[j], 32, kWave);
    if (lane < 32) {
      sred[0][wave][32 * j + li] = (double)s;
      sred[1][wave][32 * j + li] = (double)q;
    }
  }
  __syncthreads();
  for (int col = tid; col < NB * 32; col += kFT)
    if (col < C) {
      atomicAdd(stat + col, sred[0][0][col] + sred[0][1][col] + sred[0][2][col] + sred[0][3][col]);
      atomicAdd(stat + C + col, sred[1][0][col] + sred[1][1][col] + sred[1][2][col] + sred[1][3][col]);
    }
  if (!finalize) return;
  __shared__ unsigned last;
  wait_vm_complete();
  __syncthreads();
  unsigned* ticket = reinterpret_cast<unsigned*>(stat + 2 * C);
  if (tid == 0) last = atomicAdd(ticket, 1u) == gridDim.x - 1 ? 1u : 0u;
  __syncthreads();
  if (!last) return;
  for (int c = tid; c < C; c += kFT) {
    const double s1 = __hip_atomic_load(stat + c, __ATOMIC_RELAXED, __HIP_MEMORY_SCOPE_AGENT);
    const double s2 = __hip_atomic_load(stat + C + c, __ATOMIC_RELAXED, __HIP_MEMORY_SCOPE_AGENT);
    const double m = s1 / (double)fin.rows;
    double var = s2 / (double)fin.rows - m * m;
    if (var < 0.0) var = 0.0;
    fin.mean[c] = (float)m;
    fin.invstd[c] = (float)(1.0 / sqrt(var + (double)fin.eps));
    if (fin.running_mean) {
      const double unbiased = fin.rows > 1 ? var * ((double)fin.rows / (double)(fin.rows - 1)) : var;
      fin.running_mean[c] = (float)((1.0 - fin.momentum) * (double)fin.running_mean[c] + fin.momentum * m);
      fin.running_var[c] = (float)((1.0 - fin.momentum) * (double)fin.running_var[c] + fin.momentum * unbiased);
    }
  }
  if (tid == 0) {
    if (fin.num_batches_tracked) *fin.num_batches_tracked += 1;
    *ticket = 0u;
  }
}

struct SaFwdArgs {
  SaSrc s;
  const float* W2;
  const float* bn2[4];
  const float* W3;
  int C2, C3;
  double* stat;
  BnFinalize fin;
  float* ymax;
  float* ymin;
  uint8_t* amax;
  uint8_t* amin;
  int64_t tiles_per_wg;
};

template <int C1B, int C2B, int C3B, int NS, int STAGE>
__global__ __launch_bounds__(kFT) void sa_train_fwd_kernel(SaFwdArgs p) {
  constexpr bool PF = STAGE == 2;
  constexpr int kW2 = C1B * NS * C2B * 32 * 64;
  constexpr int kW3 = STAGE == 3 ? C2B * NS * C3B * 32 * 64 : 16;
  constexpr int NBS = STAGE == 3 ? C3B : C2B;
  __shared__ __attribute__((aligned(16))) unsigned char W2l[kW2];
  __shared__ __attribute__((aligned(16))) unsigned char W3l[kW3];
  __shared__ __attribute__((aligned(16))) float P1[4 * C1B * 32];
  __shared__ __attribute__((aligned(16))) float Wx[C1B * 32][4];
  __shared__ __attribute__((aligned(16))) float tiles[4][32 * kFLd];
  __shared__ double sred[2][4][NBS * 32];
  const int tid = threadIdx.x, lane = tid & 63, wave = tid >> 6;
  const int li = lane & 31, lh = lane >> 5;
  const int C1 = p.s.C1, C2 = p.C2, C3 = p.C3;
  stage_weight<NS>(W2l, p.W2, C2, C1, C2B * 32, C1B, tid);
  if constexpr (STAGE == 3) stage_weight<NS>(W3l, p.W3, C3, C2, C3B * 32, C2B, tid);
  stage_layer1<C1B>(p.s, P1, Wx, tid);
  LaneBn<C2B> bn2;
  if constexpr (STAGE == 3) bn2.load(p.bn2, C2, li);
  float ssum[NBS], qsum[NBS];
#pragma unroll
  for (int j = 0; j < NBS; ++j) ssum[j] = qsum[j] = 0.f;
  __syncthreads();
  float* st = tiles[wave];
  BallPipe<C1B, PF> pipe;
  for (int g = pipe.begin(p.s, p.tiles_per_wg, wave, li, lh); g < pipe.t_end; g += 4) {
    BallRows<C1B> rc;
    pipe.rows(p.s, g, li, lh, rc);
    float v1[C1B][4][4], dif[3];
    gather_finish<C1B>(rc, lh, Wx, v1, dif);
    act_rows<C1B>(v1, P1, lh);
    f32x16 acc2[C2B];
    layer_mfma<C1B, C2B, NS>(v1, W2l, li, lh, acc2);
    if constexpr (STAGE == 2) {
#pragma unroll
      for (int jb = 0; jb < C2B; ++jb) {
        float s = 0.f, q = 0.f;
#pragma unroll
        for (int i = 0; i < 16; ++i) {
          const float y = acc2[jb][i];
          s += y;
          q += y * y;
        }
        ssum[jb] += s;
        qsum[jb] += q;
      }
    } else {
      float v2[C2B][4][4];
#pragma unroll
      for (int jb = 0; jb < C2B; ++jb) {
#pragma unroll
        for (int i = 0; i < 16; ++i) st[acc_row(i, lh) * kFLd + li] = bn2.act(jb, acc2[jb][i]);
        __builtin_amdgcn_wave_barrier();
#pragma unroll
        for (int tt = 0; tt < 4; ++tt) {
          const float4 a = *reinterpret_cast<const float4*>(st + li * kFLd + 8 * tt + 4 * lh);
          v2[jb][tt][0] = a.x; v2[jb][tt][1] = a.y; v2[jb][tt][2] = a.z; v2[jb][tt][3] = a.w;
        }
        __builtin_amdgcn_wave_barrier();
      }
      f32x16 acc3[C3B];
      layer_mfma<C2B, C3B, NS>(v2, W3l, li, lh, acc3);
#pragma unroll
      for (int jb = 0; jb < C3B; ++jb) {
        const bool cok = 32 * jb + li < C3;
        float s = 0.f, q = 0.f;
        float vmax = -INFINITY, vmin = INFINITY;
        int rmax = 0, rmin = 0;
#pragma unroll
        for (int i = 0; i < 16; ++i) {
          const int m = acc_row(i, lh);
          const float y = acc3[jb][i];
          s += y;
          q += y * y;
          if (y > vmax) { vmax = y; rmax = m; }
          if (y < vmin) { vmin = y; rmin = m; }
        }
        const float omax = __shfl_xor(vmax, 32, kWave), omin = __shfl_xor(vmin, 32, kWave);
        const int ormax = __shfl_xor(rmax, 32, kWave), ormin = __shfl_xor(rmin, 32, kWave);
        if (omax > vmax || (omax == vmax && ormax < rmax)) { vmax = omax; rmax = ormax; }
        if (omin < vmin || (omin == vmin && ormin < rmin)) { vmin = omin; rmin = ormin; }
        if (lh == 0 && cok) {
          const size_t ob = (size_t)g * C3;
          const unsigned o = (unsigned)(32 * jb + li);
          (p.ymax + ob)[o] = vmax;
          (p.ymin + ob)[o] = vmin;
          (p.amax + ob)[o] = (uint8_t)rmax;
          (p.amin + ob)[o] = (uint8_t)rmin;
        }
        if (!cok) s = q = 0.f;
        ssum[jb] += s;
        qsum[jb] += q;
      }
    }
  }
  stats_tail<NBS>(ssum, qsum, sred, p.stat, STAGE == 3 ? C3 : C2, p.fin, true);
}

struct SaBwdArgs {
  SaSrc s;
  const float* W2;
  const float* bn2[4];
  const float* W3;
  int C2, C3;
  const float* mean_i;
  const float* invstd_i;
  const float* gamma_i;
  const double* stat_i;
  float* dgamma_i;
  float* dbeta_i;
  float inv_rows;
  const float* G;
  const float* pool_dout;
  const float* pool_out;
  const uint8_t* pool_arg;
  float* dW;
  int lddw;
  float* dZ;
  double* stat_prev;
  float* tsum;
  int64_t tiles_per_wg;
};

template <int C1B, int C2B, int C3B, int NS, int LAYER, int NSF>
__global__ __launch_bounds__(kFT, ((LAYER == 3 ? C1B * C2B * C3B <= 2 : C1B * C2B == 1) ? 2 : 1)) void sa_train_bwd_kernel(SaBwdArgs p) {
  using SP = SplitPairs<NS>;
  constexpr bool PF = LAYER == 3;
  constexpr int CB = LAYER == 3 ? C3B : C2B;
  constexpr int CPB = LAYER == 3 ? C2B : C1B;
  constexpr int kW2f = C1B * NSF * C2B * 32 * 64;
  constexpr int kW3f = LAYER == 3 ? C2B * NS * C3B * 32 * 64 : 0;
  constexpr int kWb = NS * CB * CPB * 32 * 64;
  constexpr int kTileBytes = 4 * 32 * kFLd * 4;
  constexpr int kRedBytes = 2 * CB * CPB * 16 * 64 * 4;
  constexpr int kMain = kW2f + kW3f + kWb + kTileBytes;
  constexpr int kLds = kMain > kRedBytes ? kMain : kRedBytes;
  __shared__ __attribute__((aligned(16))) unsigned char lds[kLds];
  __shared__ __attribute__((aligned(16))) float P1[4 * C1B * 32];
  __shared__ __attribute__((aligned(16))) float Wx[C1B * 32][4];
  __shared__ __attribute__((aligned(16))) float dtile[4][32][4];
  __shared__ double sred[2][4][CPB * 32];
  unsigned char* W2f = lds;
  unsigned char* W3f = lds + kW2f;
  unsigned char* Wb = lds + kW2f + kW3f;
  const int tid = threadIdx.x, lane = tid & 63, wave = tid >> 6;
  const int c = lane & 31, h = lane >> 5;
  float* tile = reinterpret_cast<float*>(lds + kW2f + kW3f + kWb) + wave * 32 * kFLd;
  const int C1 = p.s.C1, C2 = p.C2, C3 = p.C3;
  const int C = LAYER == 3 ? C3 : C2, Cp = LAYER == 3 ? C2 : C1;
  const float* W = LAYER == 3 ? p.W3 : p.W2;

  stage_weight<NSF>(W2f, p.W2, C2, C1, C2B * 32, C1B, tid);
  if constexpr (LAYER == 3) stage_weight<NS>(W3f, p.W3, C3, C2, C3B * 32, C2B, tid);
  stage_layer1<C1B>(p.s, P1, Wx, tid);
  {
    const int quads = CB * 8;
    for (int t = tid; t < quads * CPB * 32; t += kFT) {
      const int ci = t % (CPB * 32), cq = t / (CPB * 32);
      const int co = 4 * cq;
      float v[4];
#pragma unroll
      for (int e = 0; e < 4; ++e) v[e] = (co + e < C && ci < Cp) ? W[(size_t)(co + e) * Cp + ci] : 0.f;
      unsigned lo[NS], hi[NS];
      split_pair<NS>(v[0], v[1], lo);
      split_pair<NS>(v[2], v[3], hi);
      const int a = cq >> 3, coq = cq & 7;
      const int tt = coq >> 1, hh = coq & 1;
      const int unit = 2 * (tt >> 1) + hh, half = tt & 1;
      const int sw = (ci >> 2) & 3;
#pragma unroll
      for (int pc = 0; pc < NS; ++pc)
        *reinterpret_cast<uint2*>(Wb + ((size_t)(pc * CB + a) * (CPB * 32) + ci) * 64 + ((unit ^ sw) * 16) + half * 8) = make_uint2(lo[pc], hi[pc]);
    }
  }
  if (p.dgamma_i && blockIdx.x == 0)
    for (int col = tid; col < C; col += kFT) {
      p.dbeta_i[col] = (float)p.stat_i[col];
      p.dgamma_i[col] = (float)p.stat_i[C + col];
    }
  float sc[CB], mu[CB], is[CB], db[CB], dg[CB];
  bool cok[CB];
#pragma unroll
  for (int a = 0; a < CB; ++a) {
    const int col = 32 * a + c;
    cok[a] = col < C;
    sc[a] = mu[a] = is[a] = db[a] = dg[a] = 0.f;
    if (cok[a]) {
      mu[a] = p.mean_i[col];
      is[a] = p.invstd_i[col];
      sc[a] = p.gamma_i[col] * is[a];
      db[a] = (float)p.stat_i[col] * p.inv_rows;
      dg[a] = (float)p.stat_i[C + col] * p.inv_rows;
    }
  }
  const float* const act_mean = LAYER == 3 ? p.bn2[0] : p.s.bn1[0];
  const float* const act_invstd = LAYER == 3 ? p.bn2[1] : p.s.bn1[1];
  const float* const act_gamma = LAYER == 3 ? p.bn2[2] : p.s.bn1[2];
  const float* const act_beta = LAYER == 3 ? p.bn2[3] : p.s.bn1[3];
  float pm[CPB], pi[CPB], pg[CPB], pb[CPB];
  bool xok[CPB];
#pragma unroll
  for (int b = 0; b < CPB; ++b) {
    const int col = 32 * b + c;
    xok[b] = col < Cp;
    pm[b] = pi[b] = pg[b] = pb[b] = 0.f;
    if (xok[b]) {
      pm[b] = act_mean[col];
      pi[b] = act_invstd[col];
      pg[b] = act_gamma[col];
      pb[b] = act_beta[col];
    }
  }
  f32x16 accw[CB][CPB];
#pragma unroll
  for (int a = 0; a < CB; ++a)
#pragma unroll
    for (int b = 0; b < CPB; ++b)
#pragma unroll
      for (int i = 0; i < 16; ++i) accw[a][b][i] = 0.f;
  float ssum[CPB], tsum[CPB], txs[CPB][3];
#pragma unroll
  for (int b = 0; b < CPB; ++b) ssum[b] = tsum[b] = txs[b][0] = txs[b][1] = txs[b][2] = 0.f;
  __syncthreads();

  BallPipe<C1B, PF> pipe;
  for (int g = pipe.begin(p.s, p.tiles_per_wg, wave, c, h); g < pipe.t_end; g += 4) {
    BallRows<C1B> rc;
    pipe.rows(p.s, g, c, h, rc);
    float gn[16];
    auto load_g = [&](int a) {
      const float* Gt = p.G + (size_t)g * 32 * C;
      const int col = min(32 * a + c, C - 1);
#pragma unroll
      for (int q = 0; q < 16; ++q) gn[q] = Gt[(unsigned)(acc_row(q, h) * C + col)];
    };
    if constexpr (LAYER == 2) load_g(0);
    float v1[C1B][4][4], dif[3];
    gather_finish<C1B>(rc, h, Wx, v1, dif);
    if constexpr (LAYER == 2) {
      if (h == 0) *reinterpret_cast<float4*>(&dtile[wave][c][0]) = make_float4(dif[0], dif[1], dif[2], 0.f);
    }
    float x[CPB][16];
    f32x16 y2[C2B];
    if constexpr (LAYER == 2) {
#pragma unroll
      for (int sl = 0; sl < C1B; ++sl) {
#pragma unroll
        for (int tt = 0; tt < 4; ++tt)
          *reinterpret_cast<float4*>(tile + c * kFLd + 8 * tt + 4 * h) = make_float4(v1[sl][tt][0], v1[sl][tt][1], v1[sl][tt][2], v1[sl][tt][3]);
        __builtin_amdgcn_wave_barrier();
#pragma unroll
        for (int q = 0; q < 16; ++q) x[sl][q] = tile[acc_row(q, h) * kFLd + c];
        __builtin_amdgcn_wave_barrier();
      }
    }
    act_rows<C1B>(v1, P1, h);
    layer_mfma<C1B, C2B, NSF>(v1, W2f, c, h, y2);
    if constexpr (LAYER == 3) {
#pragma unroll
      for (int b = 0; b < CPB; ++b)
#pragma unroll
        for (int q = 0; q < 16; ++q) x[b][q] = y2[b][q];
    }
    u32x4 fb[CPB][2][NS];
    u32x4 far[LAYER == 3 ? CPB : 1][2][NS];
#pragma unroll
    for (int b = 0; b < CPB; ++b) {
      float av[16];
#pragma unroll
      for (int q = 0; q < 16; ++q) {
        const float z = ((x[b][q] - pm[b]) * pi[b]) * pg[b] + pb[b];
        av[q] = (xok[b] && z > 0.f) ? z : 0.f;
      }
#pragma unroll
      for (int s = 0; s < 2; ++s) {
        unsigned qq[4][NS];
#pragma unroll
        for (int jj = 0; jj < 4; ++jj) split_pair<NS>(av[8 * s + 2 * jj], av[8 * s + 2 * jj + 1], qq[jj]);
#pragma unroll
        for (int pc = 0; pc < NS; ++pc) fb[b][s][pc] = u32x4{qq[0][pc], qq[1][pc], qq[2][pc], qq[3][pc]};
      }
      if constexpr (LAYER == 3) {
#pragma unroll
        for (int q = 0; q < 16; ++q) tile[acc_row(q, h) * kFLd + c] = av[q];
        __builtin_amdgcn_wave_barrier();
#pragma unroll
        for (int s = 0; s < 2; ++s) tile_row_frags<NS>(tile, c, h, s, far[b][s]);
        __builtin_amdgcn_wave_barrier();
      }
    }
    f32x16 accz[CPB];
#pragma unroll
    for (int b = 0; b < CPB; ++b)
#pragma unroll
      for (int i = 0; i < 16; ++i) accz[b][i] = 0.f;
#pragma unroll
    for (int a = 0; a < CB; ++a) {
      __builtin_amdgcn_sched_barrier(0);
      float dyv[16];
      if constexpr (LAYER == 3) {
        f32x16 yl;
#pragma unroll
        for (int i = 0; i < 16; ++i) yl[i] = 0.f;
        const int co = 32 * a + c;
#pragma unroll
        for (int b = 0; b < CPB; ++b)
#pragma unroll
          for (int s = 0; s < 2; ++s) {
            u32x4 wf[NS];
#pragma unroll
            for (int pc = 0; pc < NS; ++pc)
              wf[pc] = *reinterpret_cast<const u32x4*>(W3f + ((size_t)(b * NS + pc) * (C3B * 32) + co) * 64 + (((2 * s + h) ^ ((co >> 2) & 3)) * 16));
#pragma unroll
            for (int qd = 0; qd < SP::N; ++qd)
              yl = __builtin_amdgcn_mfma_f32_32x32x16_bf16(__builtin_bit_cast(bf16x8, far[b][s][SP::A[qd]]),
                                                          __builtin_bit_cast(bf16x8, wf[SP::B[qd]]), yl, 0, 0, 0);
          }
        const size_t gb = (size_t)g * C;
        const unsigned go = (unsigned)min(co, C - 1);
        const float dd = ((p.pool_out + gb)[go] > 0.f) ? (p.pool_dout + gb)[go] : 0.f;
        const int ar = (int)(p.pool_arg + gb)[go];
#pragma unroll
        for (int q = 0; q < 16; ++q) {
          const float xh = (yl[q] - mu[a]) * is[a];
          const float d = sc[a] * (((ar == acc_row(q, h) ? dd : 0.f) - db[a]) - xh * dg[a]);
          dyv[q] = cok[a] ? d : 0.f;
        }
      } else {
#pragma unroll
        for (int q = 0; q < 16; ++q) {
          const float xh = (y2[a][q] - mu[a]) * is[a];
          const float d = sc[a] * ((gn[q] - db[a]) - xh * dg[a]);
          dyv[q] = cok[a] ? d : 0.f;
        }
        if (a + 1 < CB) load_g(a + 1);
      }
#pragma unroll
      for (int s = 0; s < 2; ++s) {
        unsigned qq[4][NS];
#pragma unroll
        for (int jj = 0; jj < 4; ++jj) split_pair<NS>(dyv[8 * s + 2 * jj], dyv[8 * s + 2 * jj + 1], qq[jj]);
        u32x4 fa[NS];
#pragma unroll
        for (int pc = 0; pc < NS; ++pc) fa[pc] = u32x4{qq[0][pc], qq[1][pc], qq[2][pc], qq[3][pc]};
#pragma unroll
        for (int qd = 0; qd < SP::N; ++qd)
#pragma unroll
          for (int b = 0; b < CPB; ++b)
            accw[a][b] = __builtin_amdgcn_mfma_f32_32x32x16_bf16(__builtin_bit_cast(bf16x8, fa[SP::A[qd]]),
                                                                __builtin_bit_cast(bf16x8, fb[b][s][SP::B[qd]]), accw[a][b], 0, 0, 0);
      }
#pragma unroll
      for (int q = 0; q < 16; ++q) tile[acc_row(q, h) * kFLd + c] = dyv[q];
      __builtin_amdgcn_wave_barrier();
#pragma unroll
      for (int s = 0; s < 2; ++s) {
        u32x4 fr[NS];
        tile_row_frags<NS>(tile, c, h, s, fr);
#pragma unroll
        for (int b = 0; b < CPB; ++b) {
          const int ci = 32 * b + c;
          u32x4 wf[NS];
#pragma unroll
          for (int pc = 0; pc < NS; ++pc)
            wf[pc] = *reinterpret_cast<const u32x4*>(Wb + ((size_t)(pc * CB + a) * (CPB * 32) + ci) * 64 + (((2 * s + h) ^ ((ci >> 2) & 3)) * 16));
#pragma unroll
          for (int qd = 0; qd < SP::N; ++qd)
            accz[b] = __builtin_amdgcn_mfma_f32_32x32x16_bf16(__builtin_bit_cast(bf16x8, fr[SP::A[qd]]),
                                                             __builtin_bit_cast(bf16x8, wf[SP::B[qd]]), accz[b], 0, 0, 0);
        }
      }
      __builtin_amdgcn_wave_barrier();
    }
    float* const Zb = p.dZ + (size_t)g * 32 * Cp;
#pragma unroll
    for (int b = 0; b < CPB; ++b) {
      float s = 0.f, tq = 0.f;
#pragma unroll
      for (int q = 0; q < 16; ++q) {
        float d = accz[b][q];
        const float xh = (x[b][q] - pm[b]) * pi[b];
        d = (xok[b] && xh * pg[b] + pb[b] > 0.f) ? d : 0.f;
        s += d;
        tq += d * xh;
        tile[acc_row(q, h) * kFLd + c] = d;
        if constexpr (LAYER == 2) {
          const float4 dd = *reinterpret_cast<const float4*>(&dtile[wave][acc_row(q, h)][0]);
          txs[b][0] += d * dd.x;
          txs[b][1] += d * dd.y;
          txs[b][2] += d * dd.z;
        }
      }
      ssum[b] += s;
      tsum[b] += tq;
      __builtin_amdgcn_wave_barrier();
#pragma unroll
      for (int pp = 0; pp < 4; ++pp) {
        const int row = pp * 8 + (lane >> 3), c4 = (lane & 7) * 4;
        const f32x4 v = *reinterpret_cast<const f32x4*>(tile + row * kFLd + c4);
        const int cc = 32 * b + c4;
        if (cc < Cp) __builtin_nontemporal_store(v, reinterpret_cast<f32x4*>(Zb + (unsigned)(row * Cp + cc)));
      }
      __builtin_amdgcn_wave_barrier();
    }
  }

  stats_tail<CPB>(ssum, tsum, sred, p.stat_prev, Cp, BnFinalize{}, false);
  if constexpr (LAYER == 2) {
    __syncthreads();
    float* tred = reinterpret_cast<float*>(&sred[0][0][0]);
#pragma unroll
    for (int b = 0; b < CPB; ++b) {
      const float v0 = txs[b][0] + __shfl_xor(txs[b][0], 32, kWave), v1 = txs[b][1] + __shfl_xor(txs[b][1], 32, kWave);
      const float v2 = txs[b][2] + __shfl_xor(txs[b][2], 32, kWave);
      if (lane < 32) *reinterpret_cast<float4*>(tred + ((size_t)wave * (CPB * 32) + 32 * b + c) * 4) = make_float4(v0, v1, v2, 0.f);
    }
    __syncthreads();
    float* dst = p.tsum + (size_t)(blockIdx.x & 15) * (Cp * 4);
    for (int t = tid; t < Cp * 4; t += kFT)
      if ((t & 3) < 3) atomicAdd(dst + t, (tred[t] + tred[CPB * 32 * 4 + t]) + (tred[2 * CPB * 32 * 4 + t] + tred[3 * CPB * 32 * 4 + t]));
  }
  float* red = reinterpret_cast<float*>(lds);
  constexpr int kSlot = CB * CPB * 16 * 64;
  auto publish = [&](int slot) {
#pragma unroll
    for (int a = 0; a < CB; ++a)
#pragma unroll
      for (int b = 0; b < CPB; ++b)
#pragma unroll
        for (int i = 0; i < 16; ++i) red[slot * kSlot + ((a * CPB + b) * 16 + i) * 64 + lane] = accw[a][b][i];
  };
  auto absorb = [&](int slot) {
#pragma unroll
    for (int a = 0; a < CB; ++a)
#pragma unroll
      for (int b = 0; b < CPB; ++b)
#pragma unroll
        for (int i = 0; i < 16; ++i) accw[a][b][i] += red[slot * kSlot + ((a * CPB + b) * 16 + i) * 64 + lane];
  };
  if (wave >= 2) publish(wave - 2);
  __syncthreads();
  if (wave < 2) absorb(wave);
  __syncthreads();
  if (wave == 1) publish(0);
  __syncthreads();
  if (wave == 0) {
    absorb(0);
#pragma unroll
    for (int a = 0; a < CB; ++a)
#pragma unroll
      for (int b = 0; b < CPB; ++b) {
        const int ci = 32 * b + c;
#pragma unroll
        for (int i = 0; i < 16; ++i) {
          const int co = 32 * a + acc_row(i, h);
          if (co < C && ci < Cp) atomicAdd(p.dW + (size_t)co * p.lddw + ci, accw[a][b][i]);
        }
      }
  }
}

__global__ __launch_bounds__(256) void sa_geom_sums_kernel(const int* __restrict__ offsets, const int* __restrict__ slots, const float* __restrict__ xyz,
                                                           const float* __restrict__ centre, int B, int N, int M, float4* __restrict__ dsum,
                                                           double* __restrict__ gsum) {
  __shared__ float red[256][9];
  const int64_t E = (int64_t)M * 32, total = (int64_t)B * N;
  float acc[9];
#pragma unroll
  for (int u = 0; u < 9; ++u) acc[u] = 0.f;
  for (int64_t t = (int64_t)blockIdx.x * 256 + threadIdx.x; t < total; t += (int64_t)gridDim.x * 256) {
    const int64_t b = t / N;
    const int j = (int)(t - b * N);
    const int* o = offsets + (size_t)b * (N + 1) + j;
    const int p0 = o[0], p1 = o[1];
    const int* sl = slots + (size_t)b * E;
    const float* cen = centre + (size_t)b * M * 3;
    const float px = xyz[(size_t)t * 3 + 0], py = xyz[(size_t)t * 3 + 1], pz = xyz[(size_t)t * 3 + 2];
    float dx = 0.f, dy = 0.f, dz = 0.f;
    auto add_slot = [&](const float* c0) {
      const float ex = px - c0[0], ey = py - c0[1], ez = pz - c0[2];
      dx += ex; dy += ey; dz += ez;
      acc[3] += ex * ex; acc[4] += ex * ey; acc[5] += ex * ez; acc[6] += ey * ey; acc[7] += ey * ez; acc[8] += ez * ez;
    };
    int q = p0;
    for (; q + 3 < p1; q += 4) {
      const int e0 = sl[q], e1 = sl[q + 1], e2 = sl[q + 2], e3 = sl[q + 3];
      const float* c0 = cen + (size_t)(e0 >> 5) * 3;
      const float* c1 = cen + (size_t)(e1 >> 5) * 3;
      const float* c2 = cen + (size_t)(e2 >> 5) * 3;
      const float* c3 = cen + (size_t)(e3 >> 5) * 3;
      const float a0[3] = {c0[0], c0[1], c0[2]}, a1[3] = {c1[0], c1[1], c1[2]}, a2[3] = {c2[0], c2[1], c2[2]}, a3[3] = {c3[0], c3[1], c3[2]};
      add_slot(a0); add_slot(a1); add_slot(a2); add_slot(a3);
    }
    for (; q < p1; ++q) add_slot(cen + (size_t)(sl[q] >> 5) * 3);
    dsum[t] = make_float4(dx, dy, dz, (float)(p1 - p0));
    acc[0] += dx; acc[1] += dy; acc[2] += dz;
  }
#pragma unroll
  for (int u = 0; u < 9; ++u) red[threadIdx.x][u] = acc[u];
  __syncthreads();
  if (threadIdx.x < 9) {
    double tsum = 0.0;
    for (int i = 0; i < 256; ++i) tsum += (double)red[i][threadIdx.x];
    atomicAdd(gsum + threadIdx.x, tsum);
  }
}

struct SaStats1Args {
  const float* zf;
  const float4* dsum;
  const float* wxyz;
  const double* gsum;
  double* stat;
  double* zsum;
  double* rep;
  int nrep;
  BnFinalize fin;
  int64_t total;
  int C1;
};

__global__ __launch_bounds__(256) void sa_train_stats1_kernel(SaStats1Args p) {
  __shared__ float red[256][20];
  const int C1 = p.C1, C4 = C1 >> 2;
  const int ppw = 256 / C4;
  const int c4 = threadIdx.x % C4, pg = threadIdx.x / C4;
  const int c = c4 * 4;
  float w[4][3];
#pragma unroll
  for (int i = 0; i < 4; ++i)
#pragma unroll
    for (int k = 0; k < 3; ++k) w[i][k] = p.wxyz[(c + i) * 3 + k];
  float acc[20];
#pragma unroll
  for (int u = 0; u < 20; ++u) acc[u] = 0.f;
  auto add_point = [&](const float4& z4, const float4& d) {
    const float z[4] = {z4.x, z4.y, z4.z, z4.w};
#pragma unroll
    for (int i = 0; i < 4; ++i) {
      const float wd = (w[i][0] * d.x + w[i][1] * d.y) + w[i][2] * d.z;
      acc[i] += d.w * z[i];
      acc[4 + i] += z[i] * (d.w * z[i] + 2.f * wd);
      acc[8 + 3 * i + 0] += z[i] * d.x;
      acc[8 + 3 * i + 1] += z[i] * d.y;
      acc[8 + 3 * i + 2] += z[i] * d.z;
    }
  };
  if (pg < ppw) {
    const int64_t stride = (int64_t)gridDim.x * ppw;
    int64_t t = (int64_t)blockIdx.x * ppw + pg;
    for (; t + 3 * stride < p.total; t += 4 * stride) {
      float4 z4[4], d[4];
#pragma unroll
      for (int u = 0; u < 4; ++u) {
        z4[u] = *reinterpret_cast<const float4*>(p.zf + (size_t)(t + u * stride) * C1 + c);
        d[u] = p.dsum[t + u * stride];
      }
#pragma unroll
      for (int u = 0; u < 4; ++u) add_point(z4[u], d[u]);
    }
    for (; t < p.total; t += stride) add_point(*reinterpret_cast<const float4*>(p.zf + (size_t)t * C1 + c), p.dsum[t]);
  }
#pragma unroll
  for (int u = 0; u < 20; ++u) red[threadIdx.x][u] = acc[u];
  __syncthreads();
  if (pg == 0) {
    double tot[20];
#pragma unroll
    for (int u = 0; u < 20; ++u) tot[u] = 0.0;
    for (int gq = 0; gq < ppw; ++gq)
#pragma unroll
      for (int u = 0; u < 20; ++u) tot[u] += (double)red[gq * C4 + c4][u];
    if (blockIdx.x == 0) {
      const double* S = p.gsum;
#pragma unroll
      for (int i = 0; i < 4; ++i) {
        const double a = w[i][0], b = w[i][1], cc = w[i][2];
        tot[i] += a * S[0] + b * S[1] + cc * S[2];
        tot[4 + i] += a * a * S[3] + b * b * S[6] + cc * cc * S[8] + 2.0 * (a * b * S[4] + a * cc * S[5] + b * cc * S[7]);
      }
    }
    double* s1 = p.rep ? p.rep + (size_t)(blockIdx.x % p.nrep) * 5 * C1 : p.stat;
    double* zz = p.rep ? s1 + 2 * C1 : p.zsum;
#pragma unroll
    for (int i = 0; i < 4; ++i) {
      atomicAdd(s1 + c + i, tot[i]);
      atomicAdd(s1 + C1 + c + i, tot[4 + i]);
#pragma unroll
      for (int k = 0; k < 3; ++k) atomicAdd(zz + (c + i) * 3 + k, tot[8 + 3 * i + k]);
    }
  }
  __shared__ unsigned last;
  wait_vm_complete();
  __syncthreads();
  unsigned* ticket = reinterpret_cast<unsigned*>(p.stat + 2 * C1);
  if (threadIdx.x == 0) last = atomicAdd(ticket, 1u) == gridDim.x - 1 ? 1u : 0u;
  __syncthreads();
  if (!last) return;
  const BnFinalize& fin = p.fin;
  if (p.rep) {
    for (int e = threadIdx.x; e < 5 * C1; e += 256) {
      double t = 0.0;
      for (int r = 0; r < p.nrep; ++r) t += __hip_atomic_load(p.rep + (size_t)r * 5 * C1 + e, __ATOMIC_RELAXED, __HIP_MEMORY_SCOPE_AGENT);
      if (e < 2 * C1) __hip_atomic_store(p.stat + e, t, __ATOMIC_RELAXED, __HIP_MEMORY_SCOPE_AGENT);
      else p.zsum[e - 2 * C1] = t;
    }
    __syncthreads();
  }
  for (int col = threadIdx.x; col < C1; col += 256) {
    const double s1 = __hip_atomic_load(p.stat + col, __ATOMIC_RELAXED, __HIP_MEMORY_SCOPE_AGENT);
    const double s2 = __hip_atomic_load(p.stat + C1 + col, __ATOMIC_RELAXED, __HIP_MEMORY_SCOPE_AGENT);
    const double m = s1 / (double)fin.rows;
    double var = s2 / (double)fin.rows - m * m;
    if (var < 0.0) var = 0.0;
    fin.mean[col] = (float)m;
    fin.invstd[col] = (float)(1.0 / sqrt(var + (double)fin.eps));
    if (fin.running_mean) {
      const double unbiased = fin.rows > 1 ? var * ((double)fin.rows / (double)(fin.rows - 1)) : var;
      fin.running_mean[col] = (float)((1.0 - fin.momentum) * (double)fin.running_mean[col] + fin.momentum * m);
      fin.running_var[col] = (float)((1.0 - fin.momentum) * (double)fin.running_var[col] + fin.momentum * unbiased);
    }
  }
  if (threadIdx.x == 0) {
    if (fin.num_batches_tracked) *fin.num_batches_tracked += 1;
    *ticket = 0u;
  }
}

struct SaBwd1Args {
  const float* dz1;
  const int* offsets;
  const int* slots;
  const float* zf;
  const float4* dsum;
  const float* wxyz;
  const float* mean;
  const float* invstd;
  const float* gamma;
  const double* stat;
  const float* tsum;
  const double* zsum;
  const double* gsum;
  float inv_rows;
  float* dgamma;
  float* dbeta;
  float* gz;
  float* dWx;
  int lddw;
  int B, N, M, C1;
};

__global__ __launch_bounds__(256) void sa_train_bwd1_kernel(SaBwd1Args p) {
  const int C1 = p.C1, C4 = C1 >> 2;
  if (blockIdx.x == 0 && blockIdx.y == 0) {
    const double* S = p.gsum;
    for (int t = threadIdx.x; t < C1 * 3; t += 256) {
      const int col = t / 3, k = t - col * 3;
      const double is = p.invstd[col], sc = (double)p.gamma[col] * is, mu = p.mean[col];
      const double db = p.stat[col] * (double)p.inv_rows, dg = p.stat[C1 + col] * (double)p.inv_rows;
      const double w0 = p.wxyz[col * 3 + 0], w1 = p.wxyz[col * 3 + 1], w2 = p.wxyz[col * 3 + 2];
      const double s2k0 = k == 0 ? S[3] : k == 1 ? S[4] : S[5], s2k1 = k == 0 ? S[4] : k == 1 ? S[6] : S[7], s2k2 = k == 0 ? S[5] : k == 1 ? S[7] : S[8];
      const double q = is * (p.zsum[col * 3 + k] + (w0 * s2k0 + w1 * s2k1 + w2 * s2k2) - mu * S[k]);
      double T = 0.0;
      for (int slot = 0; slot < 16; ++slot) T += (double)p.tsum[(size_t)slot * C1 * 4 + col * 4 + k];
      const double g = sc * ((T - db * S[k]) - dg * q);
      p.dWx[(size_t)col * p.lddw + k] += (float)g;
    }
    if (p.dgamma)
      for (int col = threadIdx.x; col < C1; col += 256) {
        p.dbeta[col] = (float)p.stat[col];
        p.dgamma[col] = (float)p.stat[C1 + col];
      }
  }
  const int b = blockIdx.y;
  const int64_t t = (int64_t)blockIdx.x * 256 + threadIdx.x;
  const int64_t j = t / C4;
  const int c = (int)(t - j * C4) * 4;
  if (j >= p.N) return;
  const int64_t E = (int64_t)p.M * 32;
  const int* o = p.offsets + (size_t)b * (p.N + 1) + j;
  const int p0 = o[0], p1 = o[1];
  const int* sl = p.slots + (size_t)b * E;
  const float* g = p.dz1 + (size_t)b * E * C1;
  float4 acc = make_float4(0.f, 0.f, 0.f, 0.f);
  int q = p0;
  for (; q + 3 < p1; q += 4) {
    int e[4];
#pragma unroll
    for (int u = 0; u < 4; ++u) e[u] = sl[q + u];
    float4 a[4];
#pragma unroll
    for (int u = 0; u < 4; ++u) a[u] = *reinterpret_cast<const float4*>(g + (size_t)e[u] * C1 + c);
#pragma unroll
    for (int u = 0; u < 4; ++u) {
      acc.x += a[u].x; acc.y += a[u].y; acc.z += a[u].z; acc.w += a[u].w;
    }
  }
  for (; q < p1; ++q) {
    const float4 a = *reinterpret_cast<const float4*>(g + (size_t)sl[q] * C1 + c);
    acc.x += a.x; acc.y += a.y; acc.z += a.z; acc.w += a.w;
  }
  const size_t pt = (size_t)b * p.N + j;
  const float4 z4 = *reinterpret_cast<const float4*>(p.zf + pt * C1 + c);
  const float4 d = p.dsum[pt];
  const float A[4] = {acc.x, acc.y, acc.z, acc.w}, z[4] = {z4.x, z4.y, z4.z, z4.w};
  float out[4];
#pragma unroll
  for (int i = 0; i < 4; ++i) {
    const int col = c + i;
    const float is = p.invstd[col], sc = p.gamma[col] * is, mu = p.mean[col];
    const float db = (float)p.stat[col] * p.inv_rows, dg = (float)p.stat[C1 + col] * p.inv_rows;
    const float wd = (p.wxyz[col * 3 + 0] * d.x + p.wxyz[col * 3 + 1] * d.y) + p.wxyz[col * 3 + 2] * d.z;
    const float xs = is * (d.w * (z[i] - mu) + wd);
    out[i] = sc * ((A[i] - d.w * db) - dg * xs);
  }
  *reinterpret_cast<float4*>(p.gz + pt * C1 + c) = make_float4(out[0], out[1], out[2], out[3]);
}

}

MVP_API int mvp_sa_train_forward_f32(int stage, const float* zf, const float* xyz, const float* centre, const int64_t* index, const float* wxyz,
                                     int64_t B, int64_t N, int64_t M, int64_t K, int64_t C1, const float* bn1_mean, const float* bn1_invstd,
                                     const float* bn1_gamma, const float* bn1_beta, const float* W2, int64_t C2, const float* bn2_mean,
                                     const float* bn2_invstd, const float* bn2_gamma, const float* bn2_beta, const float* W3, int64_t C3,
                                     double* stat, float eps, float momentum, float* mean, float* invstd, float* running_mean,
                                     float* running_var, int64_t* num_batches_tracked, float* ymax, float* ymin, uint8_t* amax,
                                     uint8_t* amin, mvp_stream_t stream) {
  MVP_NONNULL(stat);
  MVP_NONNULL(mean);
  MVP_NONNULL(invstd);
  if (stage == 3) {
    MVP_NONNULL(bn2_mean);
    MVP_NONNULL(bn2_invstd);
    MVP_NONNULL(bn2_gamma);
    MVP_NONNULL(bn2_beta);
    MVP_NONNULL(W3);
    MVP_NONNULL(ymax);
    MVP_NONNULL(ymin);
    MVP_NONNULL(amax);
    MVP_NONNULL(amin);
  }
  const bool sizes = stage == 3 ? C3 > 0 : stage == 2;
  if (stage != 3) C3 = 0;
  const int ns = mlp_fwd_pieces();
  SaLevel lv;
  const int rc = sa_level(zf, true, xyz, centre, index, wxyz, B, N, M, K, C1, {bn1_mean, bn1_invstd, bn1_gamma, bn1_beta}, W2, C2, C3,
                          sizes, ns != 0 && (uintptr_t)zf % 16 == 0, &lv);
  if (rc != MVP_OK || lv.s.G == 0) return rc;
  SaFwdArgs a{lv.s, W2, {bn2_mean, bn2_invstd, bn2_gamma, bn2_beta}, W3, (int)C2, (int)C3, stat,
              BnFinalize{B * M * K, eps, momentum, mean, invstd, running_mean, running_var, num_batches_tracked}, ymax, ymin, amax, amin, 0};
  const int64_t lds = (int64_t)ns * 2048 * (lv.c1b * lv.c2b + (stage == 3 ? lv.c2b * lv.c3b : 0)) + 32 * 1024;
  const unsigned grid = sa_grid(lv.s.G, lds, 4, 1024, &a.tiles_per_wg);
  hipStream_t s = static_cast<hipStream_t>(stream);
  auto launch = [&](auto shapes, auto st) {
    return sa_pick(shapes, {lv.c1b, lv.c2b, lv.c3b}, [&](auto sh) {
      sa_pick(SaPieces{}, {ns}, [&](auto pc) {
        hipLaunchKernelGGL((sa_train_fwd_kernel<decltype(sh)::v[0], decltype(sh)::v[1], decltype(sh)::v[2], decltype(pc)::v[0], decltype(st)::v[0]>),
                           dim3(grid), dim3(kFT), 0, s, a);
      });
    });
  };
  const bool found = stage == 3 ? launch(SaShapes3{}, SaRow<3>{}) : launch(SaShapes2{}, SaRow<2>{});
  return found ? mvp_launch_status() : MVP_EUNSUPPORTED;
}

MVP_API int mvp_sa_train_backward_f32(int layer, const float* zf, const float* xyz, const float* centre, const int64_t* index,
                                      const float* wxyz, int64_t B, int64_t N, int64_t M, int64_t K, int64_t C1, const float* bn1_mean,
                                      const float* bn1_invstd, const float* bn1_gamma, const float* bn1_beta, const float* W2, int64_t C2,
                                      const float* bn2_mean, const float* bn2_invstd, const float* bn2_gamma, const float* bn2_beta,
                                      const float* W3, int64_t C3, const float* mean_i, const float* invstd_i, const float* gamma_i,
                                      const double* stat_i, float* dgamma_i, float* dbeta_i, int training, const float* G,
                                      const float* pool_dout, const float* pool_out, const uint8_t* pool_arg, float* dW, int64_t lddw,
                                      float* dZ, double* stat_prev, float* tsum, mvp_stream_t stream) {
  MVP_NONNULL(mean_i);
  MVP_NONNULL(invstd_i);
  MVP_NONNULL(gamma_i);
  MVP_NONNULL(stat_i);
  MVP_NONNULL(dW);
  MVP_NONNULL(dZ);
  MVP_NONNULL(stat_prev);
  if (layer == 3) {
    MVP_NONNULL(bn2_mean);
    MVP_NONNULL(bn2_invstd);
    MVP_NONNULL(bn2_gamma);
    MVP_NONNULL(bn2_beta);
    MVP_NONNULL(W3);
    MVP_NONNULL(pool_dout);
    MVP_NONNULL(pool_out);
    MVP_NONNULL(pool_arg);
  } else if (layer == 2) {
    MVP_NONNULL(G);
    MVP_NONNULL(tsum);
  }
  const bool sizes = lddw > 0 && lddw < (1 << 24) && (layer == 3 ? C3 > 0 && lddw >= C2 : layer == 2 && lddw >= C1);
  if (layer != 3) C3 = 0;
  const int ns = mlp_bwd_pieces();
  SaLevel lv;
  const int rc = sa_level(zf, true, xyz, centre, index, wxyz, B, N, M, K, C1, {bn1_mean, bn1_invstd, bn1_gamma, bn1_beta}, W2, C2, C3,
                          sizes, ns != 0 && (uintptr_t)zf % 16 == 0 && (uintptr_t)dZ % 16 == 0, &lv);
  if (rc != MVP_OK || lv.s.G == 0) return rc;
  SaBwdArgs a{lv.s, W2, {bn2_mean, bn2_invstd, bn2_gamma, bn2_beta}, W3, (int)C2, (int)C3, mean_i, invstd_i, gamma_i, stat_i,
              dbeta_i ? dgamma_i : nullptr, dbeta_i, training ? 1.0f / (float)(B * M * K) : 0.f, G, pool_dout, pool_out, pool_arg, dW, (int)lddw, dZ,
              stat_prev, tsum, 0};
  const int c1b = lv.c1b, c2b = lv.c2b, c3b = lv.c3b;
  const int cb = layer == 3 ? c3b : c2b, cpb = layer == 3 ? c2b : c1b;
  const int nsf = (mlp_fwd_pieces() == 3) ? 3 : ns;
  const int64_t lds = (int64_t)2048 * (nsf * c1b * c2b + ns * ((layer == 3 ? c2b * c3b : 0) + cb * cpb)) + 32 * 1024;
  const bool narrow = layer == 3 ? c1b * c2b * c3b <= 2 : c1b * c2b == 1;
  const unsigned grid = sa_grid(lv.s.G, lds, narrow ? 2 : 1, 1024, &a.tiles_per_wg);
  hipStream_t s = static_cast<hipStream_t>(stream);
  using Pieces = SaTable<SaRow<1, 1>, SaRow<1, 3>, SaRow<2, 2>, SaRow<2, 3>, SaRow<3, 3>>;
  auto launch = [&](auto shapes, auto ly) {
    return sa_pick(shapes, {c1b, c2b, c3b}, [&](auto sh) {
      sa_pick(Pieces{}, {ns, nsf}, [&](auto pc) {
        hipLaunchKernelGGL((sa_train_bwd_kernel<decltype(sh)::v[0], decltype(sh)::v[1], decltype(sh)::v[2], decltype(pc)::v[0], decltype(ly)::v[0],
                                                decltype(pc)::v[1]>), dim3(grid), dim3(kFT), 0, s, a);
      });
    });
  };
  const bool found = layer == 3 ? launch(SaShapes3{}, SaRow<3>{}) : launch(SaShapes2{}, SaRow<2>{});
  return found ? mvp_launch_status() : MVP_EUNSUPPORTED;
}

MVP_API int mvp_sa_geom_sums_f32(const int32_t* offsets, const int32_t* slots, const float* xyz, const float* centre, int64_t B, int64_t N,
                                 int64_t M, int64_t K, float* dsum, double* gsum, mvp_stream_t stream) {
  MVP_NONNULL(offsets);
  MVP_NONNULL(slots);
  MVP_NONNULL(xyz);
  MVP_NONNULL(centre);
  MVP_NONNULL(dsum);
  MVP_NONNULL(gsum);
  MVP_REQUIRE(B >= 0 && N > 0 && M >= 0);
  if (K != 32 || ((uintptr_t)dsum % 16) != 0) return MVP_EUNSUPPORTED;
  if (B == 0) return MVP_OK;
  const unsigned grid = (unsigned)std::max<int64_t>(1, std::min<int64_t>(1024, cdiv(B * N, 256)));
  hipLaunchKernelGGL(sa_geom_sums_kernel, dim3(grid), dim3(256), 0, static_cast<hipStream_t>(stream), offsets, slots, xyz, centre, (int)B, (int)N,
                     (int)M, reinterpret_cast<float4*>(dsum), gsum);
  return mvp_launch_status();
}

MVP_API int mvp_sa_train_stats1_ws_f32(const float* zf, const float* dsum, const float* wxyz, const double* gsum, int64_t B, int64_t N, int64_t M,
                                       int64_t K, int64_t C1, double* stat, double* zsum, float eps, float momentum, float* mean, float* invstd,
                                       float* running_mean, float* running_var, int64_t* num_batches_tracked, double* scratch,
                                       int64_t scratch_doubles, mvp_stream_t stream) {
  MVP_NONNULL(zf);
  MVP_NONNULL(dsum);
  MVP_NONNULL(wxyz);
  MVP_NONNULL(gsum);
  MVP_NONNULL(stat);
  MVP_NONNULL(zsum);
  MVP_NONNULL(mean);
  MVP_NONNULL(invstd);
  MVP_REQUIRE(B >= 0 && N > 0 && M >= 0 && K > 0 && C1 > 0);
  if (C1 % 4 != 0 || C1 > 1024 || 256 % (C1 / 4) != 0 || ((uintptr_t)zf % 16) != 0 || ((uintptr_t)dsum % 16) != 0) return MVP_EUNSUPPORTED;
  if (B == 0 || M == 0) return MVP_OK;
  MVP_REQUIRE(scratch_doubles >= 0 && (scratch != nullptr || scratch_doubles == 0));
  const int nrep = scratch ? (int)std::min<int64_t>(16, scratch_doubles / (5 * C1)) : 0;
  SaStats1Args a{zf, reinterpret_cast<const float4*>(dsum), wxyz, gsum, stat, zsum, nrep >= 2 ? scratch : nullptr, nrep,
                 BnFinalize{B * M * K, eps, momentum, mean, invstd, running_mean, running_var, num_batches_tracked}, B * N, (int)C1};
  const int64_t ppw = 256 / (C1 / 4);
  static const int wgs = []() { const char* e = getenv("MVP_SA_STATS1_WGS"); return e ? atoi(e) : 256; }();
  const unsigned grid = (unsigned)std::max<int64_t>(1, std::min<int64_t>(wgs, cdiv(B * N, ppw * 8)));
  hipLaunchKernelGGL(sa_train_stats1_kernel, dim3(grid), dim3(256), 0, static_cast<hipStream_t>(stream), a);
  return mvp_launch_status();
}

MVP_API int mvp_sa_train_stats1_f32(const float* zf, const float* dsum, const float* wxyz, const double* gsum, int64_t B, int64_t N, int64_t M,
                                    int64_t K, int64_t C1, double* stat, double* zsum, float eps, float momentum, float* mean, float* invstd,
                                    float* running_mean, float* running_var, int64_t* num_batches_tracked, mvp_stream_t stream) {
  return mvp_sa_train_stats1_ws_f32(zf, dsum, wxyz, gsum, B, N, M, K, C1, stat, zsum, eps, momentum, mean, invstd, running_mean, running_var,
                                    num_batches_tracked, nullptr, 0, stream);
}

MVP_API int mvp_sa_train_backward1_f32(const float* dz1, const int32_t* offsets, const int32_t* slots, const float* zf, const float* dsum,
                                       const float* wxyz, const float* tsum, const double* zsum, const double* gsum, int64_t B, int64_t N,
                                       int64_t M, int64_t K, int64_t C1, const float* mean, const float* invstd, const float* gamma,
                                       const double* stat, int training, float* dgamma, float* dbeta, float* gz, float* dWxyz, int64_t lddw,
                                       mvp_stream_t stream) {
  MVP_NONNULL(dz1);
  MVP_NONNULL(offsets);
  MVP_NONNULL(slots);
  MVP_NONNULL(zf);
  MVP_NONNULL(dsum);
  MVP_NONNULL(wxyz);
  MVP_NONNULL(tsum);
  MVP_NONNULL(zsum);
  MVP_NONNULL(gsum);
  MVP_NONNULL(mean);
  MVP_NONNULL(invstd);
  MVP_NONNULL(gamma);
  MVP_NONNULL(stat);
  MVP_NONNULL(gz);
  MVP_NONNULL(dWxyz);
  MVP_REQUIRE(B >= 0 && B < 65536 && N > 0 && M >= 0 && C1 > 0 && lddw >= 3);
  if (K != 32 || C1 % 4 != 0 || ((uintptr_t)zf % 16) != 0 || ((uintptr_t)dsum % 16) != 0 || ((uintptr_t)dz1 % 16) != 0) return MVP_EUNSUPPORTED;
  if (B == 0) return MVP_OK;
  SaBwd1Args a{dz1, offsets, slots, zf, reinterpret_cast<const float4*>(dsum), wxyz, mean, invstd, gamma, stat, tsum, zsum, gsum,
               training ? 1.0f / (float)(B * M * K) : 0.f, dbeta ? dgamma : nullptr, dbeta, gz, dWxyz, (int)lddw, (int)B, (int)N, (int)M, (int)C1};
  hipLaunchKernelGGL(sa_train_bwd1_kernel, dim3((unsigned)cdiv(N * (C1 / 4), 256), (unsigned)B), dim3(256), 0, static_cast<hipStream_t>(stream), a);
  return mvp_launch_status();
}
```

### mvpnet_amd/rows.py

```python
import os
import weakref

import torch
import torch.nn.functional as F
from torch.autograd.function import once_differentiable

from . import _lib as L


FUSE_BWD_MAX_COUT = int(os.environ.get('MVP_BWD_FUSE_MAXC', '64'))
FUSE_BWD_MAX_CIN = int(os.environ.get('MVP_BWD_FUSE_MAXCIN', '96'))
PARTIAL_MIN_ROWS = int(os.environ.get('MVP_PARTIAL_MIN_ROWS', '65536'))
WIDE_BWD = os.environ.get('MVP_BWD_WIDE', '1') != '0'
WIDE_BWD_MIN_ROWS = int(os.environ.get('MVP_BWD_WIDE_MIN_ROWS', '16384'))


WIDE_BWD_64 = os.environ.get('MVP_BWD_WIDE64', '1') != '0'
WIDE_BWD_POOLED = os.environ.get('MVP_BWD_WIDE_POOLED', '1') != '0'
WIDE_BWD_64_MIN_ROWS = int(os.environ.get('MVP_BWD_WIDE64_MIN_ROWS', '262144'))


DX_WIDE = os.environ.get('MVP_DX_WIDE', '0') == '1'
DX_WIDE_MIN_ROWS = int(os.environ.get('MVP_DX_WIDE_MIN_ROWS', '16384'))
DX_WIDE_MAX_COUT = int(os.environ.get('MVP_DX_WIDE_MAXC', '512'))
# ... 1025 lines not shown
            if route == 'wide':
                step = wk.wide(i, gcur, pending, w, src)
            elif route == 'fuse':
                step = wk.fuse(i, gcur, pending, w, src, need_dz)
            elif route == 'tile':
                step = wk.tile(i, gcur, w, src, need_dz)
            elif route == 'dxw':
                step = wk.dxw(i, gcur, pending, w, src)
            elif w is not None:
                step = wk.rel(gcur, pending, w, src, need_dz, route)
            else:
                step = wk.defer(gcur, pending, ctx.defer) if route == 'defer' else (gcur, None, None, None, None)
            gcur, pending, grads[3 * i], dgam, dbet = step
            if dgam is not None:
                grads[3 * i + 1], grads[3 * i + 2] = dgam, dbet
        dx0 = gcur
        if dx0 is not None and dx0.size(1) != x0.size(1):
            dx0 = F.pad(dx0, (0, x0.size(1) - dx0.size(1)))
        if ctx.dw_use is not None:
            ctx.dw_use.done = True
        return (dx0, None, None, None, None, None, None) + tuple(grads)


class RelationRows(torch.autograd.Function):

    @staticmethod
    def forward(ctx, feature, src_xyz, tgt_xyz):
        L.require_gpu(feature, src_xyz, tgt_xyz)
        B, N, k, C = feature.shape
        out = torch.empty((B, N, k, C + 4), dtype=torch.float32, device=feature.device)
        L.call('mvp_relation_rows_f32', feature, L.ptr(feature), L.ptr(src_xyz), L.ptr(tgt_xyz), B * N, k, C, L.ptr(out))
        ctx.C = C
        return out

    @staticmethod
    @once_differentiable
    def backward(ctx, g):
        return g[..., :ctx.C].contiguous(), None, None


def relation_rows(feature, src_xyz, tgt_xyz):
    return RelationRows.apply(feature.contiguous(), src_xyz.contiguous(), tgt_xyz.contiguous())


class LinearRows(torch.autograd.Function):

    @staticmethod
    def forward(ctx, x, w_full, bias, c0=0, c1=None, sink=None, act_src=None):
        ctx.sink = sink
        info = None if act_src is None else act_src.info
        ctx.act_src = act_src if (info is not None and ActivationHandOver.ENABLED and x.is_cuda and tuple(info[0].shape) == tuple(x.shape)) else None
        prec = ctx.prec = L.current_precision()
        w2 = w_full.detach().reshape(w_full.size(0), -1)
        c1 = w2.size(1) if c1 is None else c1
        R, ldx = x.shape
        cin = c1 - c0
        if w2.is_cuda and w2.dtype == torch.float32:
            w = weight_slices.get(w_full, c0, c1, ldx)
        else:
            w = w2[:, c0:c1]
            if ldx != cin:
                w = torch.nn.functional.pad(w, (0, ldx - cin))
            w = w.contiguous()
        L.require_gpu(x, w, bias)
        cout = w.size(0)
        y = torch.empty((R, cout), dtype=torch.float32, device=x.device)
        L.call('mvp_mlp_forward_f32', x, L.ptr(x), R, ldx, ldx, L.ptr(w), ldx, cout, None, None, None, None, L.ptr(bias), L.ptr(y), None, None, prec=prec)
        ctx.save_for_backward(x, w)
        ctx.has_bias = bias is not None
        ctx.slice = (c0, cin, tuple(w_full.shape))
        ctx.bias_param = bias if (bias is not None and bias.is_leaf) else None
        ctx.dw_use = WeightUse([w_full]) if (DW_SIDE_STREAM and LINEAR_ASIDE and sink is None and c0 == 0 and c1 == w2.size(1) and ctx.needs_input_grad[1]) else None
        return y

    @staticmethod
    @once_differentiable
    def backward(ctx, gy):
        x, w = ctx.saved_tensors
        R, cin = x.shape
        cout = w.size(0)
        gy = gy.contiguous()
        gx = gw = gb = None
        aside = False
        if ctx.needs_input_grad[0]:
            gx = torch.empty_like(x)
            src = ctx.act_src
            if src is not None and src.info is not None:
                yp, pm, pi, pg, pb, drop_p, drop_seed = src.info
                stat = zero_pool.zeros(2 * cin, torch.float64, gy.device)
                part = L.ptr(_partial(R, cin, gy.device) if R > 65536 else None)
                if drop_p > 0:
                    L.call('mvp_mlp_input_grad_dropout_f32', gy, L.ptr(gy), R, cout, L.ptr(w), cin, L.ptr(yp), L.ptr(pm), L.ptr(pi), L.ptr(pg), L.ptr(pb),
                           drop_p, drop_seed, L.ptr(gx), L.ptr(stat), part, prec=ctx.prec)
                else:
                    L.call('mvp_mlp_input_grad_f32', gy, L.ptr(gy), R, cout, L.ptr(w), cin, L.ptr(yp), L.ptr(pm), L.ptr(pi), L.ptr(pg), L.ptr(pb), L.ptr(gx),
                           L.ptr(stat), part, prec=ctx.prec)
                src.stat = stat
            else:
                L.call('mvp_mlp_input_grad_f32', gy, L.ptr(gy), R, cout, L.ptr(w), cin, None, None, None, None, None, L.ptr(gx), None, None, prec=ctx.prec)
        if ctx.needs_input_grad[1]:
            c0, ncol, shape = ctx.slice
            sink = ctx.sink
            if sink is not None:
                buf = sink.buffer(gy.device)
                sink.run(gy.device, 'mvp_mlp_weight_grad_f32', (L.ptr(gy), L.ptr(x), R, cout, ncol, cin, None, None, None, None,
                                                                L.ptr_at(buf, c0), sink.numel // cout), (gy, x), prec=ctx.prec)
                gw = sink.done()
            else:
                gw = zero_pool.zeros(shape, torch.float32, w.device)
                wg_args = (L.ptr(gy), L.ptr(x), R, cout, ncol, cin, None, None, None, None, L.ptr_at(gw, c0), gw.numel() // cout)
                use = ctx.dw_use
                aside = use is not None and DW_SIDE_STREAM and use.aside_ok()
                _weight_grad(aside, gy.device, 'mvp_mlp_weight_grad_f32', wg_args, (gy, x), ctx.prec)
                if use is not None:
                    use.done = True
        if ctx.has_bias and ctx.needs_input_grad[2]:
            st = side_stream.streams.get(gy.device)
            bp = ctx.bias_param
            if (aside and st is not None and gy.device in side_stream.open and bp is not None and bp.grad is None and not bp._backward_hooks
                    and not bp._post_accumulate_grad_hooks):
                gb = torch.empty(cout, dtype=gy.dtype, device=gy.device)
                with torch.cuda.stream(st[0]):
                    torch.sum(gy, 0, out=gb)
            else:
                gb = gy.sum(0)
        return gx, gw, gb, None, None, None, None


def linear_rows(x, weight, bias=None, cols=None, sink=None, act_src=None):
    c0, c1 = (0, None) if cols is None else cols
    return LinearRows.apply(x.contiguous(), weight, bias, c0, c1, sink, act_src)


def linear_rows_bf16(x, weight, bias=None, scale=None, shift=None, relu=False):
    if not (x.is_cuda and weight.is_cuda):
        raise RuntimeError('mvpnet_amd ops run on the GPU only; there is no CPU fallback')
    if x.dtype != torch.bfloat16 or x.dim() != 2 or x.stride(1) != 1:
        raise RuntimeError('linear_rows_bf16: x must be a (R, C_in) bfloat16 tensor with unit column stride')
    w = weight.detach().reshape(weight.size(0), -1)
    if w.dtype != torch.float32 or not w.is_contiguous() or w.size(1) != x.size(1):
        raise RuntimeError('linear_rows_bf16: weight must be contiguous float32 (C_out, C_in)')
    R, cin = x.shape
    cout = w.size(0)
    f = lambda t: None if t is None else t.detach().float().contiguous()
    bias, scale, shift = f(bias), f(scale), f(shift)
    y = torch.empty((R, cout), dtype=torch.bfloat16, device=x.device)
    L.call('mvp_mlp_forward_bf16', x, L.ptr(x), R, cin, x.stride(0), L.ptr(w), cin, cout, L.ptr(bias), L.ptr(scale), L.ptr(shift), int(bool(relu)),
           L.ptr(y), cout)
    return y


SA_TRAIN_FUSED = os.environ.get('MVP_SA_TRAIN', '1') != '0'


STATS1_REPLICAS = int(os.environ.get('MVP_SA_STATS1_REPLICAS', '16'))


def sa_level_train_widths_ok(c1, c2, c3):
    return c1 >= 4 and max(c1, c2) <= 64 and (c3 <= 64 or (c3 <= 128 and min(c1, c2) > 32))


def sa_level_train_ok(zf, mlp, K):
    if not (SA_TRAIN_FUSED and zf is not None and zf.is_cuda and zf.dtype == torch.float32 and len(mlp) == 3 and K == 32 and mlp_chain_is_fused(mlp)):
        return False
    if L.DW_WORKSPACE:
        return False
    ps = parts(mlp)
    c1, c2, c3 = (q.w.size(0) for q in ps)
    return sa_level_train_widths_ok(c1, c2, c3) and all(q.bn.training for q in ps) and L.current_precision()[0] != 0 and \
        all(q.w.is_contiguous() for q in ps)


class SALevelTrain(torch.autograd.Function):

    @staticmethod
    def forward(ctx, zf, xyz, centre, index, offsets, slots, dsum, gsum, w1_full, sink, bns, W2, W3, g1, b1, g2, b2, g3, b3):
        L.require_gpu(zf, xyz, centre, index, W2, W3)
        prec = ctx.prec = L.current_precision()
        ctx.sink = sink
        B, N, C1 = zf.shape
        M, K = index.size(1), index.size(2)
        C2, C3 = W2.size(0), W3.size(0)
        dev = zf.device
        ctot = w1_full.numel() // w1_full.size(0)
        ctx.w_shape = tuple(w1_full.shape)
        wxyz = weight_slices.get(w1_full, ctot - 3, ctot, 3)
        nrep = STATS1_REPLICAS
        arena = zero_pool.zeros(2 * (C1 + C2 + C3) + 3 + 3 * C1 + nrep * 5 * C1, torch.float64, dev)
        stat1, stat2, stat3 = arena[:2 * C1 + 1], arena[2 * C1 + 1:2 * (C1 + C2) + 2], arena[2 * (C1 + C2) + 2:2 * (C1 + C2 + C3) + 3]
        zsum = arena[2 * (C1 + C2 + C3) + 3:2 * (C1 + C2 + C3) + 3 + 3 * C1]
        rep1 = arena[2 * (C1 + C2 + C3) + 3 + 3 * C1:]
        mi = torch.empty(2 * (C1 + C2 + C3), dtype=torch.float32, device=dev)
        m1, i1 = mi[:C1], mi[C1:2 * C1]
        m2, i2 = mi[2 * C1:2 * C1 + C2], mi[2 * C1 + C2:2 * (C1 + C2)]
        m3, i3 = mi[2 * (C1 + C2):2 * (C1 + C2) + C3], mi[2 * (C1 + C2) + C3:]
        (rm1, rv1, nb1, e1, mo1), (rm2, rv2, nb2, e2, mo2), (rm3, rv3, nb3, e3, mo3) = bns
        if offsets is None:
            offsets, slots = build_csr(index, N)
        if dsum is None:
            dsum, gsum = geom_sums(offsets, slots, xyz, centre, K)
        L.call('mvp_sa_train_stats1_ws_f32', zf, L.ptr(zf), L.ptr(dsum), L.ptr(wxyz), L.ptr(gsum), B, N, M, K, C1, L.ptr(stat1), L.ptr(zsum), float(e1),
               float(mo1), L.ptr(m1), L.ptr(i1), L.ptr(rm1), L.ptr(rv1), L.ptr(nb1), L.ptr(rep1) if nrep else None, rep1.numel())
        level = (L.ptr(zf), L.ptr(xyz), L.ptr(centre), L.ptr(index), L.ptr(wxyz), B, N, M, K, C1, L.ptr(m1), L.ptr(i1), L.ptr(g1), L.ptr(b1), L.ptr(W2), C2)
        L.call('mvp_sa_train_forward_f32', xyz, 2, *level, None, None, None, None, None, 0, L.ptr(stat2), float(e2), float(mo2), L.ptr(m2), L.ptr(i2),
               L.ptr(rm2), L.ptr(rv2), L.ptr(nb2), None, None, None, None, prec=prec)
        G = B * M
        ymax = torch.empty((G, C3), dtype=torch.float32, device=dev)
        ymin = torch.empty((G, C3), dtype=torch.float32, device=dev)
        amax = torch.empty((G, C3), dtype=torch.uint8, device=dev)
        amin = torch.empty((G, C3), dtype=torch.uint8, device=dev)
        L.call('mvp_sa_train_forward_f32', xyz, 3, *level, L.ptr(m2), L.ptr(i2), L.ptr(g2), L.ptr(b2), L.ptr(W3), C3, L.ptr(stat3), float(e3), float(mo3),
               L.ptr(m3), L.ptr(i3), L.ptr(rm3), L.ptr(rv3), L.ptr(nb3), L.ptr(ymax), L.ptr(ymin), L.ptr(amax), L.ptr(amin), prec=prec)
        out = torch.empty((G, C3), dtype=torch.float32, device=dev)
        arg = torch.empty((G, C3), dtype=torch.uint8, device=dev)
        ysel = torch.empty((G, C3), dtype=torch.float32, device=dev)
        L.call('mvp_pool_finalize_f32', ymax, L.ptr(ymax), L.ptr(ymin), L.ptr(amax), L.ptr(amin), L.ptr(m3), L.ptr(i3), L.ptr(g3), L.ptr(b3), G, C3, 1,
               L.ptr(out), L.ptr(arg), L.ptr(ysel))
        ctx.save_for_backward(zf, xyz, centre, index, offsets, slots, dsum, gsum, zsum, wxyz, mi, g1, b1, g2, b2, g3, W2, W3, out, arg, ysel)
        ctx.dims = (B, N, M, K, C1, C2, C3)
        return out.view(B, M, C3)

    @staticmethod
    @once_differentiable
    def backward(ctx, grad_out):
        zf, xyz, centre, index, offsets, slots, dsum, gsum, zsum, wxyz, mi, g1, b1, g2, b2, g3, W2, W3, out, arg, ysel = ctx.saved_tensors
        B, N, M, K, C1, C2, C3 = ctx.dims
        prec = ctx.prec
        dev = zf.device
        G, R = B * M, B * M * K
        g = grad_out.contiguous().view(G, C3)
        m1, i1 = mi[:C1], mi[C1:2 * C1]
        m2, i2 = mi[2 * C1:2 * C1 + C2], mi[2 * C1 + C2:2 * (C1 + C2)]
        m3, i3 = mi[2 * (C1 + C2):2 * (C1 + C2) + C3], mi[2 * (C1 + C2) + C3:]
        stat3 = torch.empty(2 * C3, dtype=torch.float64, device=dev)
        L.call('mvp_pool_backward_stats_f32', g, L.ptr(g), L.ptr(out), L.ptr(ysel), L.ptr(m3), L.ptr(i3), G, C3, 1, L.ptr(stat3),
               L.ptr(_cs_partial(G, C3, dev)))
        st = zero_pool.zeros(2 * (C2 + C1), torch.float64, dev)
        stat2, stat1 = st[:2 * C2], st[2 * C2:]
        dw = zero_pool.zeros(C3 * C2 + C2 * C1 + 16 * 4 * C1, torch.float32, dev)
        dW3, dW2, tsum = dw[:C3 * C2].view(C3, C2), dw[C3 * C2:C3 * C2 + C2 * C1].view(C2, C1), dw[C3 * C2 + C2 * C1:]
        dgb = torch.empty(2 * (C1 + C2 + C3), dtype=torch.float32, device=dev)
        dg1, db1 = dgb[:C1], dgb[C1:2 * C1]
        dg2, db2 = dgb[2 * C1:2 * C1 + C2], dgb[2 * C1 + C2:2 * (C1 + C2)]
        dg3, db3 = dgb[2 * (C1 + C2):2 * (C1 + C2) + C3], dgb[2 * (C1 + C2) + C3:]
        level = (L.ptr(zf), L.ptr(xyz), L.ptr(centre), L.ptr(index), L.ptr(wxyz), B, N, M, K, C1, L.ptr(m1), L.ptr(i1), L.ptr(g1), L.ptr(b1), L.ptr(W2), C2,
                 L.ptr(m2), L.ptr(i2), L.ptr(g2), L.ptr(b2))
        dz2 = torch.empty((R, C2), dtype=torch.float32, device=dev)
        L.call('mvp_sa_train_backward_f32', zf, 3, *level, L.ptr(W3), C3, L.ptr(m3), L.ptr(i3), L.ptr(g3), L.ptr(stat3), L.ptr(dg3), L.ptr(db3), 1, None,
               L.ptr(g), L.ptr(out), L.ptr(arg), L.ptr(dW3), C2, L.ptr(dz2), L.ptr(stat2), None, prec=prec)
        dz1 = torch.empty((R, C1), dtype=torch.float32, device=dev)
        L.call('mvp_sa_train_backward_f32', zf, 2, *level, None, 0, L.ptr(m2), L.ptr(i2), L.ptr(g2), L.ptr(stat2), L.ptr(dg2), L.ptr(db2), 1, L.ptr(dz2),
               None, None, None, L.ptr(dW2), C1, L.ptr(dz1), L.ptr(stat1), L.ptr(tsum), prec=prec)
        del dz2
        numel = 1
        for d in ctx.w_shape:
            numel *= d
        ctot = numel // C1
        sink = ctx.sink
        buf = sink.buffer(dev) if sink is not None else zero_pool.zeros(numel + 4, torch.float32, dev)
        gz = torch.empty((B, N, C1), dtype=torch.float32, device=dev)
        L.call('mvp_sa_train_backward1_f32', zf, L.ptr(dz1), L.ptr(offsets), L.ptr(slots), L.ptr(zf), L.ptr(dsum), L.ptr(wxyz), L.ptr(tsum), L.ptr(zsum),
               L.ptr(gsum), B, N, M, K, C1, L.ptr(m1), L.ptr(i1), L.ptr(g1), L.ptr(stat1), 1, L.ptr(dg1), L.ptr(db1), L.ptr(gz), L.ptr_at(buf, ctot - 3), ctot)
        gw1 = sink.done() if sink is not None else buf[:numel].view(ctx.w_shape)
        return (gz if ctx.needs_input_grad[0] else None, None, None, None, None, None, None, None, gw1, None, None, dW2, dW3, dg1, db1, dg2, db2, dg3, db3)


def sa_level_train(zf, xyz, centre, index, mlp, csr=None, sink=None):
    offsets, slots = (csr[0], csr[1]) if csr is not None else (None, None)
    dsum, gsum = (csr[2], csr[3]) if csr is not None and len(csr) >= 4 else (None, None)
    q1, q2, q3 = parts(mlp)
    bns = [(q.rm, q.rv, q.nbt, q.bn.eps, 0.1 if q.bn.momentum is None else q.bn.momentum) for q in (q1, q2, q3)]
    W2 = q2.w.reshape(q2.w.size(0), -1)
    W3 = q3.w.reshape(q3.w.size(0), -1)
    return SALevelTrain.apply(zf.contiguous(), xyz.contiguous(), centre.contiguous(), index.contiguous(), offsets, slots, dsum, gsum, q1.w, sink, bns,
                              W2, W3, q1.gamma, q1.beta, q2.gamma, q2.beta, q3.gamma, q3.beta)


SA_FUSED_EVAL = os.environ.get('MVP_SA_FUSED', '1') != '0'


def sa_fused_eval(zf, xyz, centre, index, mlp):
    if not (SA_FUSED_EVAL and len(mlp) == 3 and mlp_chain_is_fused(mlp) and index.size(2) == 32 and L.get_mlp_precision() != 'fp32'):
        return None
    c1, c2, c3 = (l.conv.weight.size(0) for l in mlp)
    if c1 > 64 or c2 > 64 or c3 > 128 or c1 % 4 or c2 % 4 or c3 % 4 or any(l.bn.training for l in mlp):
        return None
    blocks = lambda c: 1 if c <= 32 else 2 if c <= 64 else 4
    if (blocks(c1), blocks(c2), blocks(c3)) not in {(1, 1, 1), (1, 1, 2), (1, 2, 1), (1, 2, 2), (1, 2, 4), (2, 1, 1), (2, 1, 2), (2, 2, 1), (2, 2, 2),
                                                     (2, 2, 4)}:
        return None
    L.require_gpu(xyz, centre, index)
    B, N, _ = xyz.shape
    M = centre.size(1)
    bn = []
    for l in mlp:
        bn += [l.bn.running_mean, eval_invstd.get(l.bn.running_var, l.bn.eps), l.bn.weight, l.bn.bias]
    w1 = mlp[0].conv.weight
    ctot_ = w1.numel() // c1
    wxyz = weight_slices.get(w1, ctot_ - 3, ctot_, 3)
    w2 = mlp[1].conv.weight.detach().reshape(c2, c1).contiguous()
    w3 = mlp[2].conv.weight.detach().reshape(c3, c2).contiguous()
    out = torch.empty((B, M, c3), dtype=torch.float32, device=xyz.device)
    zfc = None if zf is None else zf.contiguous()
    L.call('mvp_sa_fused_forward_f32', xyz, L.ptr(zfc), L.ptr(xyz.contiguous()), L.ptr(centre.contiguous()), L.ptr(index.contiguous()), L.ptr(wxyz),
           B, N, M, 32, c1, *[L.ptr(t.detach().contiguous()) for t in bn[0:4]], L.ptr(w2), c2, *[L.ptr(t.detach().contiguous()) for t in bn[4:8]],
           L.ptr(w3), c3, *[L.ptr(t.detach().contiguous()) for t in bn[8:12]], L.ptr(out), None, prec=L.current_precision())
    return out


def mlp_chain_is_fused(mlp, dropout_p=0.0, ps=None):
    ps = parts(mlp) if ps is None else ps
    if not (dropout_p == 0 or len(ps) == 1):
        return False
    for q in ps:
        if q.bn is None or q.relu is None or q.bias is not None or q.rm is None or q.bn.momentum is None:
            return False
        c = q.w.size(0)
        if c % 4 or 256 % (c // 4):
            return False
    return True


def relation4_rows(src_xyz, tgt_xyz):
    L.require_gpu(src_xyz, tgt_xyz)
    B, N, k, _ = src_xyz.shape
    with torch.no_grad():
        s, t = src_xyz.contiguous(), tgt_xyz.contiguous()
        out = torch.empty((B, N, k, 4), dtype=torch.float32, device=s.device)
        L.call('mvp_relation4_rows_f32', s, L.ptr(s), L.ptr(t), B * N, k, L.ptr(out))
    return out


def shared_mlp_rows(x, mlp, K=1, dropout_p=0.0, training=False, first_done=False, first_stat=None, reduce='max', rel=None, dropout_last_only=False,
                    defer=None, act_out=None):
    n = len(mlp)
    ps = parts(mlp)
    fused = mlp_chain_is_fused(mlp, 0.0 if dropout_last_only else dropout_p, ps) and K <= 255
    assert fused or not dropout_last_only, 'dropout_last_only needs the fused chain'
    if fused:
        bn_training = ps[0].bn.training
        params, buffers, eps_mom = [], [], []
        for li, q in enumerate(ps):
            w = None if (first_done and li == 0) else (q.w if q.w.dim() == 2 else q.w.reshape(q.w.size(0), -1))
            params += [w, q.gamma, q.beta]
            buffers.append((q.rm, q.rv, q.nbt if bn_training else None))
            eps_mom.append((q.bn.eps, q.bn.momentum))
        opts = {'sum': bool(reduce == 'sum' and K > 1)}
        if rel is not None:
            assert not first_done and rel.dim() == 2 and rel.size(1) == 4 and rel.size(0) == x.size(0)
            opts['rel'] = (rel.contiguous(), ps[0].w)
        if defer is not None and first_done and bn_training:
            opts['defer'] = defer

        if DW_SIDE_STREAM and torch.is_grad_enabled():
            opts['use'] = WeightUse([q.w for li, q in enumerate(ps) if not (first_done and li == 0)])
        fold = dropout_p > 0 and training and K == 1 and 0 < dropout_p < 1 and FUSE_DROPOUT and x.size(0) * ps[-1].w.size(0) < 2 ** 32 and \
            not torch.cuda.is_current_stream_capturing()
        if fold:
            seed = int(torch.empty((), dtype=torch.int64).random_().item())
            opts['drop_p'], opts['drop_seed'] = float(dropout_p), seed & 0x7fffffffffffffff
        if act_out is not None and K == 1 and torch.is_grad_enabled() and (dropout_p == 0 or not training or fold):
            opts['act_out'] = act_out
        out = MLPChainRows.apply(x.contiguous(), bn_training, K, eps_mom, buffers, first_stat if bn_training else None, opts, *params)
        return F.dropout(out, p=dropout_p, training=training, inplace=False) if (dropout_p > 0 and not fold) else out
    assert not first_done and rel is None, 'first_done / rel need the fused path (BN + ReLU, no bias, no dropout)'
    if K > 255:
        x = shared_mlp_rows(x, mlp, 1, dropout_p, training)
        x = x.view(-1, K, x.size(1))
        return x.sum(dim=1) if reduce == 'sum' else x.max(dim=1)[0]
    for i, layer in enumerate(mlp):
        w = layer.conv.weight.reshape(layer.conv.weight.size(0), -1)
        if x.size(1) != w.size(1):
            w = F.pad(w, (0, x.size(1) - w.size(1)))
        y = linear_rows(x, w)
        if layer.bn is not None:
            x = bn_act_rows(y, layer.bn, relu=layer.relu is not None, K=K if (i == n - 1 and reduce != 'sum') else 1)
            if K > 1 and i == n - 1 and reduce == 'sum':
                x = x.view(-1, K, x.size(1)).sum(dim=1)
        else:
            if layer.conv.bias is not None:
                y = y + layer.conv.bias
            x = F.relu(y) if layer.relu is not None else y
            if K > 1 and i == n - 1:
                x = x.view(-1, K, x.size(1)).sum(dim=1) if reduce == 'sum' else x.view(-1, K, x.size(1)).max(dim=1)[0]
        if dropout_p > 0:
            x = F.dropout(x, p=dropout_p, training=training, inplace=False)
    return x
```

Baseline: 5251 chunks/s.

## Materialize SA layer-2 activations in forward and reuse them in later passes

The stage-2 forward pass now writes the pre-BN layer-2 activations (y2) to a global buffer. The stage-3 forward and layer-3 backward kernels load that buffer instead of re-gathering the ball neighbourhoods and recomputing layers 1 and 2. This trades the repeated gather and GEMM compute for extra HBM traffic and a buffer of B*M*K*C2 floats. A prefetch pipeline for the y2 tiles is included, and the reuse is gated per channel-width configuration and an environment variable.

```diff
diff --git a/include/mvp_hip.h b/include/mvp_hip.h
--- a/include/mvp_hip.h
+++ b/include/mvp_hip.h
@@ -374,6 +374,21 @@
                               const float* mean_i, const float* invstd_i, const float* gamma_i, const double* stat_i, float* dgamma_i,
                               float* dbeta_i, int training, const float* G, const float* pool_dout, const float* pool_out,
                               const uint8_t* pool_arg, float* dW, int64_t lddw, float* dZ, double* stat_prev, float* tsum, mvp_stream_t stream);
+int mvp_sa_train_forward_y2_f32(int stage, const float* zf, const float* xyz, const float* centre, const int64_t* index, const float* wxyz,
+                                int64_t B, int64_t N, int64_t M, int64_t K, int64_t C1, const float* bn1_mean, const float* bn1_invstd,
+                                const float* bn1_gamma, const float* bn1_beta, const float* W2, int64_t C2, const float* bn2_mean,
+                                const float* bn2_invstd, const float* bn2_gamma, const float* bn2_beta, const float* W3, int64_t C3,
+                                double* stat, float eps, float momentum, float* mean, float* invstd, float* running_mean,
+                                float* running_var, int64_t* num_batches_tracked, float* ymax, float* ymin, uint8_t* amax, uint8_t* amin,
+                                float* Y2, mvp_stream_t stream);
+int mvp_sa_train_backward_y2_f32(int layer, const float* zf, const float* xyz, const float* centre, const int64_t* index, const float* wxyz,
+                                 int64_t B, int64_t N, int64_t M, int64_t K, int64_t C1, const float* bn1_mean, const float* bn1_invstd,
+                                 const float* bn1_gamma, const float* bn1_beta, const float* W2, int64_t C2, const float* bn2_mean,
+                                 const float* bn2_invstd, const float* bn2_gamma, const float* bn2_beta, const float* W3, int64_t C3,
+                                 const float* mean_i, const float* invstd_i, const float* gamma_i, const double* stat_i, float* dgamma_i,
+                                 float* dbeta_i, int training, const float* G, const float* pool_dout, const float* pool_out,
+                                 const uint8_t* pool_arg, float* dW, int64_t lddw, float* dZ, double* stat_prev, float* tsum, const float* Y2,
+                                 mvp_stream_t stream);
 int mvp_sa_train_backward1_f32(const float* dz1, const int32_t* offsets, const int32_t* slots, const float* zf, const float* dsum,
                                const float* wxyz, const float* tsum, const double* zsum, const double* gsum, int64_t B, int64_t N, int64_t M,
                                int64_t K, int64_t C1, const float* mean, const float* invstd, const float* gamma, const double* stat,
@@ -444,6 +459,19 @@
     float* gamma_i, const double* stat_i, float* dgamma_i, float* dbeta_i, int training, const float* G, const float* pool_dout,
     const float* pool_out, const uint8_t* pool_arg, float* dW, int64_t lddw, float* dZ, double* stat_prev, float* tsum, int precision, int
     precision_backward, mvp_stream_t stream);
+int mvp_sa_train_forward_y2_p_f32(int stage, const float* zf, const float* xyz, const float* centre, const int64_t* index, const
+    float* wxyz, int64_t B, int64_t N, int64_t M, int64_t K, int64_t C1, const float* bn1_mean, const float* bn1_invstd, const
+    float* bn1_gamma, const float* bn1_beta, const float* W2, int64_t C2, const float* bn2_mean, const float* bn2_invstd, const
+    float* bn2_gamma, const float* bn2_beta, const float* W3, int64_t C3, double* stat, float eps, float momentum, float* mean,
+    float* invstd, float* running_mean, float* running_var, int64_t* num_batches_tracked, float* ymax, float* ymin, uint8_t*
+    amax, uint8_t* amin, float* Y2, int precision, int precision_backward, mvp_stream_t stream);
+int mvp_sa_train_backward_y2_p_f32(int layer, const float* zf, const float* xyz, const float* centre, const int64_t* index, const
+    float* wxyz, int64_t B, int64_t N, int64_t M, int64_t K, int64_t C1, const float* bn1_mean, const float* bn1_invstd, const
+    float* bn1_gamma, const float* bn1_beta, const float* W2, int64_t C2, const float* bn2_mean, const float* bn2_invstd, const
+    float* bn2_gamma, const float* bn2_beta, const float* W3, int64_t C3, const float* mean_i, const float* invstd_i, const
+    float* gamma_i, const double* stat_i, float* dgamma_i, float* dbeta_i, int training, const float* G, const float* pool_dout,
+    const float* pool_out, const uint8_t* pool_arg, float* dW, int64_t lddw, float* dZ, double* stat_prev, float* tsum, const float* Y2,
+    int precision, int precision_backward, mvp_stream_t stream);
 
 int mvp_pn2_plan_f32(const float* xyz, int64_t B, int64_t N, int64_t levels, const int64_t* centroids, const float* radius,
                      const int64_t* neighbours, const int32_t* geom, int fps_shape, int flags, float knn_eps, void* const* buffers,
diff --git a/mvpnet_amd/_lib.py b/mvpnet_amd/_lib.py
--- a/mvpnet_amd/_lib.py
+++ b/mvpnet_amd/_lib.py
@@ -112,6 +112,11 @@
     'mvp_sa_train_backward_f32': [ctypes.c_int, _ptr, _ptr, _ptr, _ptr, _ptr, _i64, _i64, _i64, _i64, _i64, _ptr, _ptr, _ptr, _ptr, _ptr, _i64, _ptr, _ptr,
                                   _ptr, _ptr, _ptr, _i64, _ptr, _ptr, _ptr, _ptr, _ptr, _ptr, ctypes.c_int, _ptr, _ptr, _ptr, _ptr, _ptr, _i64, _ptr, _ptr,
                                   _ptr, _ptr],
+    'mvp_sa_train_forward_y2_f32': [ctypes.c_int, _ptr, _ptr, _ptr, _ptr, _ptr, _i64, _i64, _i64, _i64, _i64, _ptr, _ptr, _ptr, _ptr, _ptr, _i64, _ptr, _ptr,
+                                    _ptr, _ptr, _ptr, _i64, _ptr, _f32, _f32, _ptr, _ptr, _ptr, _ptr, _ptr, _ptr, _ptr, _ptr, _ptr, _ptr, _ptr],
+    'mvp_sa_train_backward_y2_f32': [ctypes.c_int, _ptr, _ptr, _ptr, _ptr, _ptr, _i64, _i64, _i64, _i64, _i64, _ptr, _ptr, _ptr, _ptr, _ptr, _i64, _ptr, _ptr,
+                                     _ptr, _ptr, _ptr, _i64, _ptr, _ptr, _ptr, _ptr, _ptr, _ptr, ctypes.c_int, _ptr, _ptr, _ptr, _ptr, _ptr, _i64, _ptr, _ptr,
+                                     _ptr, _ptr, _ptr],
     'mvp_sa_train_backward1_f32': [_ptr, _ptr, _ptr, _ptr, _ptr, _ptr, _ptr, _ptr, _ptr, _i64, _i64, _i64, _i64, _i64, _ptr, _ptr, _ptr, _ptr,
                                    ctypes.c_int, _ptr, _ptr, _ptr, _ptr, _i64, _ptr],
     'mvp_pn2_plan_f32': [_ptr, _i64, _i64, _i64, _ptr, _ptr, _ptr, _ptr, ctypes.c_int, ctypes.c_int, _f32, _ptr, _i64, _ptr, _ptr, _ptr],
@@ -148,7 +153,8 @@
 }
 for _n in ['mvp_mlp_forward_f32', 'mvp_mlp_forward_bn_f32', 'mvp_mlp_forward_rel_bn_f32', 'mvp_mlp_forward_pool_f32', 'mvp_mlp_input_grad_f32', 'mvp_mlp_input_grad_dropout_f32',
            'mvp_mlp_weight_grad_f32', 'mvp_mlp_weight_grad_ws_f32', 'mvp_mlp_layer_backward_f32', 'mvp_mlp_layer_backward_ws_f32',
-           'mvp_sa_fused_forward_f32', 'mvp_sa_train_forward_f32', 'mvp_sa_train_backward_f32']:
+           'mvp_sa_fused_forward_f32', 'mvp_sa_train_forward_f32', 'mvp_sa_train_backward_f32', 'mvp_sa_train_forward_y2_f32',
+           'mvp_sa_train_backward_y2_f32']:
     _SIGNATURES[_n[:-4] + '_p_f32'] = _SIGNATURES[_n][:-1] + [ctypes.c_int, ctypes.c_int, _ptr]
 _SIGNATURES['mvp_mlp_layer_backward_wide_p_f32'] = [_ptr] * 9 + [ctypes.c_int, ctypes.c_int, _f32, ctypes.c_uint64, _ptr, _i64, _ptr, _ptr, _ptr, _ptr, _ptr, _i64,
                                                     _i64, _i64, _i64, _ptr, _i64, _ptr, _ptr, _ptr, _ptr, _i64, ctypes.c_int, ctypes.c_int, _ptr]
@@ -402,8 +408,10 @@
         check(code, name)
 
 
-def call(name, tensor_for_device, *args, prec=None):
+def call(name, tensor_for_device, *args, prec=None, y2=None):
     index = tensor_for_device.device.index
+    if y2 is not None:
+        name, args = name[:-4] + '_y2_f32', args + (y2,)
     if DW_WORKSPACE and name in _DW_WS_NAMES:
         handle = _raw_stream(index) if _raw_stream is not None else torch.cuda.current_stream(tensor_for_device.device).cuda_stream
         name, args = _DW_WS_NAMES[name], _with_dw_workspace(index, handle, args)
diff --git a/mvpnet_amd/csrc/mlp_prec.hip b/mvpnet_amd/csrc/mlp_prec.hip
--- a/mvpnet_amd/csrc/mlp_prec.hip
+++ b/mvpnet_amd/csrc/mlp_prec.hip
@@ -127,3 +127,26 @@
       bn1_beta, W2, C2, bn2_mean, bn2_invstd, bn2_gamma, bn2_beta, W3, C3, mean_i, invstd_i, gamma_i, stat_i, dgamma_i, dbeta_i, training,
       G, pool_dout, pool_out, pool_arg, dW, lddw, dZ, stat_prev, tsum, stream));
 }
+
+MVP_API int mvp_sa_train_forward_y2_p_f32(int stage, const float* zf, const float* xyz, const float* centre, const int64_t* index, const float*
+    wxyz, int64_t B, int64_t N, int64_t M, int64_t K, int64_t C1, const float* bn1_mean, const float* bn1_invstd, const float* bn1_gamma,
+    const float* bn1_beta, const float* W2, int64_t C2, const float* bn2_mean, const float* bn2_invstd, const float* bn2_gamma, const float*
+    bn2_beta, const float* W3, int64_t C3, double* stat, float eps, float momentum, float* mean, float* invstd, float* running_mean, float*
+    running_var, int64_t* num_batches_tracked, float* ymax, float* ymin, uint8_t* amax, uint8_t* amin, float* Y2, int precision, int
+    precision_backward, mvp_stream_t stream) {
+  MVP_WITH_PRECISION(mvp_sa_train_forward_y2_f32(stage, zf, xyz, centre, index, wxyz, B, N, M, K, C1, bn1_mean, bn1_invstd, bn1_gamma,
+      bn1_beta, W2, C2, bn2_mean, bn2_invstd, bn2_gamma, bn2_beta, W3, C3, stat, eps, momentum, mean, invstd, running_mean, running_var,
+      num_batches_tracked, ymax, ymin, amax, amin, Y2, stream));
+}
+
+MVP_API int mvp_sa_train_backward_y2_p_f32(int layer, const float* zf, const float* xyz, const float* centre, const int64_t* index, const
+    float* wxyz, int64_t B, int64_t N, int64_t M, int64_t K, int64_t C1, const float* bn1_mean, const float* bn1_invstd, const float*
+    bn1_gamma, const float* bn1_beta, const float* W2, int64_t C2, const float* bn2_mean, const float* bn2_invstd, const float* bn2_gamma,
+    const float* bn2_beta, const float* W3, int64_t C3, const float* mean_i, const float* invstd_i, const float* gamma_i, const double*
+    stat_i, float* dgamma_i, float* dbeta_i, int training, const float* G, const float* pool_dout, const float* pool_out, const uint8_t*
+    pool_arg, float* dW, int64_t lddw, float* dZ, double* stat_prev, float* tsum, const float* Y2, int precision, int precision_backward,
+    mvp_stream_t stream) {
+  MVP_WITH_PRECISION(mvp_sa_train_backward_y2_f32(layer, zf, xyz, centre, index, wxyz, B, N, M, K, C1, bn1_mean, bn1_invstd, bn1_gamma,
+      bn1_beta, W2, C2, bn2_mean, bn2_invstd, bn2_gamma, bn2_beta, W3, C3, mean_i, invstd_i, gamma_i, stat_i, dgamma_i, dbeta_i, training,
+      G, pool_dout, pool_out, pool_arg, dW, lddw, dZ, stat_prev, tsum, Y2, stream));
+}
diff --git a/mvpnet_amd/csrc/sa_common.h b/mvpnet_amd/csrc/sa_common.h
--- a/mvpnet_amd/csrc/sa_common.h
+++ b/mvpnet_amd/csrc/sa_common.h
@@ -247,7 +247,7 @@
 
 inline int sa_level(const float* zf, bool zf_required, const float* xyz, const float* centre, const int64_t* index, const float* wxyz, int64_t B,
                     int64_t N, int64_t M, int64_t K, int64_t C1, const float* const (&bn1)[4], const float* W2, int64_t C2, int64_t C3,
-                    bool own_sizes, bool own_ok, SaLevel* lv) {
+                    bool own_sizes, bool own_ok, SaLevel* lv, const float* y2 = nullptr) {
   if (zf_required) MVP_NONNULL(zf);
   MVP_NONNULL(xyz);
   MVP_NONNULL(centre);
@@ -257,7 +257,7 @@
   MVP_NONNULL(W2);
   MVP_REQUIRE(B >= 0 && N > 0 && M >= 0 && K > 0 && C1 > 0 && C2 > 0 && C3 >= 0 && own_sizes);
   const bool widths = K == 32 && C1 >= 4 && C1 <= 64 && C2 <= 64 && C3 <= 128 && C1 % 4 == 0 && C2 % 4 == 0 && C3 % 4 == 0;
-  if (!own_ok || !widths) return MVP_EUNSUPPORTED;
+  if (!own_ok || !widths || (uintptr_t)y2 % 16 != 0) return MVP_EUNSUPPORTED;
   constexpr int64_t kBalls = (int64_t(1) << 31) - 16, kOffsets = (int64_t(1) << 32) - 1;
   if (N > INT_MAX || M > INT_MAX || (M > 0 && B > kBalls / M) || N > kOffsets / std::max<int64_t>(C1, 3)) return MVP_EUNSUPPORTED;
   lv->s = SaSrc{zf, xyz, centre, index, wxyz, {bn1[0], bn1[1], bn1[2], bn1[3]}, B * M, (int)N, (int)M, (int)C1};
diff --git a/mvpnet_amd/csrc/sa_train.hip b/mvpnet_amd/csrc/sa_train.hip
--- a/mvpnet_amd/csrc/sa_train.hip
+++ b/mvpnet_amd/csrc/sa_train.hip
@@ -51,6 +51,78 @@
   }
 }
 
+enum { kY2Recompute = 0, kY2Store = 1, kY2Load = 2 };
+
+#ifndef MVP_SA_Y2_NT
+#define MVP_SA_Y2_NT 0
+#endif
+
+template <int C2B>
+__device__ __forceinline__ void y2_store(float* Y2, int g, int C2, float* st, int lane, const f32x16 (&y)[C2B]) {
+  const int c = lane & 31, h = lane >> 5;
+  float* Yt = Y2 + (size_t)g * 32 * C2;
+#pragma unroll
+  for (int b = 0; b < C2B; ++b) {
+#pragma unroll
+    for (int q = 0; q < 16; ++q) st[acc_row(q, h) * kFLd + c] = y[b][q];
+    __builtin_amdgcn_wave_barrier();
+#pragma unroll
+    for (int pp = 0; pp < 4; ++pp) {
+      const int row = pp * 8 + (lane >> 3), c4 = (lane & 7) * 4;
+      const f32x4 v = *reinterpret_cast<const f32x4*>(st + row * kFLd + c4);
+      const int cc = 32 * b + c4;
+      if (cc < C2) {
+#if MVP_SA_Y2_NT
+        __builtin_nontemporal_store(v, reinterpret_cast<f32x4*>(Yt + (unsigned)(row * C2 + cc)));
+#else
+        *reinterpret_cast<f32x4*>(Yt + (unsigned)(row * C2 + cc)) = v;
+#endif
+      }
+    }
+    __builtin_amdgcn_wave_barrier();
+  }
+}
+__device__ __forceinline__ void y2_load_block(const float* Y2, int g, int C2, int b, int c, int h, float (&y)[16]) {
+  const float* Yt = Y2 + (size_t)g * 32 * C2;
+  const int col = min(32 * b + c, C2 - 1);
+#pragma unroll
+  for (int q = 0; q < 16; ++q) y[q] = Yt[(unsigned)(acc_row(q, h) * C2 + col)];
+}
+template <int C2B>
+__device__ __forceinline__ void y2_load(const float* Y2, int g, int C2, int c, int h, f32x16 (&y)[C2B]) {
+#pragma unroll
+  for (int b = 0; b < C2B; ++b) {
+    float v[16];
+    y2_load_block(Y2, g, C2, b, c, h, v);
+#pragma unroll
+    for (int q = 0; q < 16; ++q) y[b][q] = v[q];
+  }
+}
+
+template <int C2B, bool PF>
+struct Y2Pipe {
+  f32x16 yn[C2B];
+  int64_t t_end;
+  __device__ __forceinline__ int begin(const float* Y2, int64_t G, int64_t tiles_per_wg, int C2, int wave, int c, int h) {
+    const int64_t t_begin = (int64_t)blockIdx.x * tiles_per_wg;
+    t_end = min(G, t_begin + tiles_per_wg);
+    const int g = __builtin_amdgcn_readfirstlane((int)(t_begin + wave));
+    if constexpr (PF) {
+      if (g < t_end) y2_load<C2B>(Y2, g, C2, c, h, yn);
+    }
+    return g;
+  }
+  __device__ __forceinline__ void rows(const float* Y2, int g, int C2, int c, int h, f32x16 (&y)[C2B]) {
+    if constexpr (PF) {
+#pragma unroll
+      for (int b = 0; b < C2B; ++b) y[b] = yn[b];
+      if (g + 4 < t_end) y2_load<C2B>(Y2, g + 4, C2, c, h, yn);
+    } else {
+      y2_load<C2B>(Y2, g, C2, c, h, y);
+    }
+  }
+};
+
 struct SaFwdArgs {
   SaSrc s;
   const float* W2;
@@ -63,27 +135,33 @@
   float* ymin;
   uint8_t* amax;
   uint8_t* amin;
+  float* Y2;
   int64_t tiles_per_wg;
 };
 
-template <int C1B, int C2B, int C3B, int NS, int STAGE>
-__global__ __launch_bounds__(kFT) void sa_train_fwd_kernel(SaFwdArgs p) {
+template <int C1B, int C2B, int C3B, int NS, int STAGE, int Y2M>
+__device__ __forceinline__ void sa_train_fwd_pass(const SaFwdArgs& p) {
+  static_assert(Y2M == kY2Recompute || (Y2M == kY2Store && STAGE == 2) || (Y2M == kY2Load && STAGE == 3), "stage 2 stores y_2, stage 3 loads it");
+  constexpr bool LOAD = Y2M == kY2Load;
   constexpr bool PF = STAGE == 2;
-  constexpr int kW2 = C1B * NS * C2B * 32 * 64;
+  constexpr bool PFY = C2B * C3B < 8 || NS > 1;
+  constexpr int kW2 = LOAD ? 16 : C1B * NS * C2B * 32 * 64;
   constexpr int kW3 = STAGE == 3 ? C2B * NS * C3B * 32 * 64 : 16;
   constexpr int NBS = STAGE == 3 ? C3B : C2B;
   __shared__ __attribute__((aligned(16))) unsigned char W2l[kW2];
   __shared__ __attribute__((aligned(16))) unsigned char W3l[kW3];
-  __shared__ __attribute__((aligned(16))) float P1[4 * C1B * 32];
-  __shared__ __attribute__((aligned(16))) float Wx[C1B * 32][4];
+  __shared__ __attribute__((aligned(16))) float P1[LOAD ? 4 : 4 * C1B * 32];
+  __shared__ __attribute__((aligned(16))) float Wx[LOAD ? 1 : C1B * 32][4];
   __shared__ __attribute__((aligned(16))) float tiles[4][32 * kFLd];
   __shared__ double sred[2][4][NBS * 32];
   const int tid = threadIdx.x, lane = tid & 63, wave = tid >> 6;
   const int li = lane & 31, lh = lane >> 5;
   const int C1 = p.s.C1, C2 = p.C2, C3 = p.C3;
-  stage_weight<NS>(W2l, p.W2, C2, C1, C2B * 32, C1B, tid);
+  if constexpr (!LOAD) {
+    stage_weight<NS>(W2l, p.W2, C2, C1, C2B * 32, C1B, tid);
+    stage_layer1<C1B>(p.s, P1, Wx, tid);
+  }
   if constexpr (STAGE == 3) stage_weight<NS>(W3l, p.W3, C3, C2, C3B * 32, C2B, tid);
-  stage_layer1<C1B>(p.s, P1, Wx, tid);
   LaneBn<C2B> bn2;
   if constexpr (STAGE == 3) bn2.load(p.bn2, C2, li);
   float ssum[NBS], qsum[NBS];
@@ -92,14 +170,24 @@
   __syncthreads();
   float* st = tiles[wave];
   BallPipe<C1B, PF> pipe;
-  for (int g = pipe.begin(p.s, p.tiles_per_wg, wave, li, lh); g < pipe.t_end; g += 4) {
-    BallRows<C1B> rc;
-    pipe.rows(p.s, g, li, lh, rc);
-    float v1[C1B][4][4], dif[3];
-    gather_finish<C1B>(rc, lh, Wx, v1, dif);
-    act_rows<C1B>(v1, P1, lh);
+  Y2Pipe<C2B, PFY> ypipe;
+  int g;
+  if constexpr (LOAD) g = ypipe.begin(p.Y2, p.s.G, p.tiles_per_wg, C2, wave, li, lh);
+  else g = pipe.begin(p.s, p.tiles_per_wg, wave, li, lh);
+  const int64_t t_end = LOAD ? ypipe.t_end : pipe.t_end;
+  for (; g < t_end; g += 4) {
     f32x16 acc2[C2B];
-    layer_mfma<C1B, C2B, NS>(v1, W2l, li, lh, acc2);
+    if constexpr (LOAD) {
+      ypipe.rows(p.Y2, g, C2, li, lh, acc2);
+    } else {
+      BallRows<C1B> rc;
+      pipe.rows(p.s, g, li, lh, rc);
+      float v1[C1B][4][4], dif[3];
+      gather_finish<C1B>(rc, lh, Wx, v1, dif);
+      act_rows<C1B>(v1, P1, lh);
+      layer_mfma<C1B, C2B, NS>(v1, W2l, li, lh, acc2);
+    }
+    if constexpr (Y2M == kY2Store) y2_store<C2B>(p.Y2, g, C2, st, lane, acc2);
     if constexpr (STAGE == 2) {
 #pragma unroll
       for (int jb = 0; jb < C2B; ++jb) {
@@ -165,6 +253,15 @@
   stats_tail<NBS>(ssum, qsum, sred, p.stat, STAGE == 3 ? C3 : C2, p.fin, true);
 }
 
+template <int C1B, int C2B, int C3B, int NS, int STAGE>
+__global__ __launch_bounds__(kFT) void sa_train_fwd_kernel(SaFwdArgs p) {
+  sa_train_fwd_pass<C1B, C2B, C3B, NS, STAGE, kY2Recompute>(p);
+}
+template <int C1B, int C2B, int C3B, int NS, int STAGE, int Y2M>
+__global__ __launch_bounds__(kFT, (Y2M != kY2Load ? 1 : C2B * C3B >= 8 ? (NS == 1 ? 2 : 1) : C2B == 2 ? 2 : 3)) void sa_train_fwd_y2_kernel(SaFwdArgs p) {
+  sa_train_fwd_pass<C1B, C2B, C3B, NS, STAGE, Y2M>(p);
+}
+
 struct SaBwdArgs {
   SaSrc s;
   const float* W2;
@@ -187,16 +284,19 @@
   float* dZ;
   double* stat_prev;
   float* tsum;
+  const float* Y2;
   int64_t tiles_per_wg;
 };
 
-template <int C1B, int C2B, int C3B, int NS, int LAYER, int NSF>
-__global__ __launch_bounds__(kFT, ((LAYER == 3 ? C1B * C2B * C3B <= 2 : C1B * C2B == 1) ? 2 : 1)) void sa_train_bwd_kernel(SaBwdArgs p) {
+template <int C1B, int C2B, int C3B, int NS, int LAYER, int NSF, bool Y2L>
+__device__ __forceinline__ void sa_train_bwd_pass(const SaBwdArgs& p) {
   using SP = SplitPairs<NS>;
   constexpr bool PF = LAYER == 3;
+  constexpr bool NOROWS = Y2L && LAYER == 3;
+  constexpr bool PFY = NS < 3 && C2B <= C1B;
   constexpr int CB = LAYER == 3 ? C3B : C2B;
   constexpr int CPB = LAYER == 3 ? C2B : C1B;
-  constexpr int kW2f = C1B * NSF * C2B * 32 * 64;
+  constexpr int kW2f = Y2L ? 0 : C1B * NSF * C2B * 32 * 64;
   constexpr int kW3f = LAYER == 3 ? C2B * NS * C3B * 32 * 64 : 0;
   constexpr int kWb = NS * CB * CPB * 32 * 64;
   constexpr int kTileBytes = 4 * 32 * kFLd * 4;
@@ -204,8 +304,8 @@
   constexpr int kMain = kW2f + kW3f + kWb + kTileBytes;
   constexpr int kLds = kMain > kRedBytes ? kMain : kRedBytes;
   __shared__ __attribute__((aligned(16))) unsigned char lds[kLds];
-  __shared__ __attribute__((aligned(16))) float P1[4 * C1B * 32];
-  __shared__ __attribute__((aligned(16))) float Wx[C1B * 32][4];
+  __shared__ __attribute__((aligned(16))) float P1[NOROWS ? 4 : 4 * C1B * 32];
+  __shared__ __attribute__((aligned(16))) float Wx[NOROWS ? 1 : C1B * 32][4];
   __shared__ __attribute__((aligned(16))) float dtile[4][32][4];
   __shared__ double sred[2][4][CPB * 32];
   unsigned char* W2f = lds;
@@ -218,9 +318,9 @@
   const int C = LAYER == 3 ? C3 : C2, Cp = LAYER == 3 ? C2 : C1;
   const float* W = LAYER == 3 ? p.W3 : p.W2;
 
-  stage_weight<NSF>(W2f, p.W2, C2, C1, C2B * 32, C1B, tid);
+  if constexpr (!Y2L) stage_weight<NSF>(W2f, p.W2, C2, C1, C2B * 32, C1B, tid);
   if constexpr (LAYER == 3) stage_weight<NS>(W3f, p.W3, C3, C2, C3B * 32, C2B, tid);
-  stage_layer1<C1B>(p.s, P1, Wx, tid);
+  if constexpr (!NOROWS) stage_layer1<C1B>(p.s, P1, Wx, tid);
   {
     const int quads = CB * 8;
     for (int t = tid; t < quads * CPB * 32; t += kFT) {
@@ -292,38 +392,48 @@
   __syncthreads();
 
   BallPipe<C1B, PF> pipe;
-  for (int g = pipe.begin(p.s, p.tiles_per_wg, wave, c, h); g < pipe.t_end; g += 4) {
-    BallRows<C1B> rc;
-    pipe.rows(p.s, g, c, h, rc);
-    float gn[16];
+  Y2Pipe<C2B, PFY> ypipe;
+  int g;
+  if constexpr (NOROWS) g = ypipe.begin(p.Y2, p.s.G, p.tiles_per_wg, C2, wave, c, h);
+  else g = pipe.begin(p.s, p.tiles_per_wg, wave, c, h);
+  const int64_t t_end = NOROWS ? ypipe.t_end : pipe.t_end;
+  for (; g < t_end; g += 4) {
+    float gn[16], yn[16];
     auto load_g = [&](int a) {
       const float* Gt = p.G + (size_t)g * 32 * C;
       const int col = min(32 * a + c, C - 1);
 #pragma unroll
       for (int q = 0; q < 16; ++q) gn[q] = Gt[(unsigned)(acc_row(q, h) * C + col)];
+      if constexpr (Y2L) y2_load_block(p.Y2, g, C2, a, c, h, yn);
     };
-    if constexpr (LAYER == 2) load_g(0);
-    float v1[C1B][4][4], dif[3];
-    gather_finish<C1B>(rc, h, Wx, v1, dif);
-    if constexpr (LAYER == 2) {
-      if (h == 0) *reinterpret_cast<float4*>(&dtile[wave][c][0]) = make_float4(dif[0], dif[1], dif[2], 0.f);
-    }
     float x[CPB][16];
     f32x16 y2[C2B];
-    if constexpr (LAYER == 2) {
-#pragma unroll
-      for (int sl = 0; sl < C1B; ++sl) {
-#pragma unroll
-        for (int tt = 0; tt < 4; ++tt)
-          *reinterpret_cast<float4*>(tile + c * kFLd + 8 * tt + 4 * h) = make_float4(v1[sl][tt][0], v1[sl][tt][1], v1[sl][tt][2], v1[sl][tt][3]);
-        __builtin_amdgcn_wave_barrier();
-#pragma unroll
-        for (int q = 0; q < 16; ++q) x[sl][q] = tile[acc_row(q, h) * kFLd + c];
-        __builtin_amdgcn_wave_barrier();
-      }
-    }
-    act_rows<C1B>(v1, P1, h);
-    layer_mfma<C1B, C2B, NSF>(v1, W2f, c, h, y2);
+    if constexpr (NOROWS) {
+      ypipe.rows(p.Y2, g, C2, c, h, y2);
+    } else {
+      BallRows<C1B> rc;
+      pipe.rows(p.s, g, c, h, rc);
+      if constexpr (LAYER == 2) load_g(0);
+      float v1[C1B][4][4], dif[3];
+      gather_finish<C1B>(rc, h, Wx, v1, dif);
+      if constexpr (LAYER == 2) {
+        if (h == 0) *reinterpret_cast<float4*>(&dtile[wave][c][0]) = make_float4(dif[0], dif[1], dif[2], 0.f);
+#pragma unroll
+        for (int sl = 0; sl < C1B; ++sl) {
+#pragma unroll
+          for (int tt = 0; tt < 4; ++tt)
+            *reinterpret_cast<float4*>(tile + c * kFLd + 8 * tt + 4 * h) = make_float4(v1[sl][tt][0], v1[sl][tt][1], v1[sl][tt][2], v1[sl][tt][3]);
+          __builtin_amdgcn_wave_barrier();
+#pragma unroll
+          for (int q = 0; q < 16; ++q) x[sl][q] = tile[acc_row(q, h) * kFLd + c];
+          __builtin_amdgcn_wave_barrier();
+        }
+      }
+      if constexpr (!Y2L) {
+        act_rows<C1B>(v1, P1, h);
+        layer_mfma<C1B, C2B, NSF>(v1, W2f, c, h, y2);
+      }
+    }
     if constexpr (LAYER == 3) {
 #pragma unroll
       for (int b = 0; b < CPB; ++b)
@@ -397,7 +507,7 @@
       } else {
 #pragma unroll
         for (int q = 0; q < 16; ++q) {
-          const float xh = (y2[a][q] - mu[a]) * is[a];
+          const float xh = ((Y2L ? yn[q] : y2[a][q]) - mu[a]) * is[a];
           const float d = sc[a] * ((gn[q] - db[a]) - xh * dg[a]);
           dyv[q] = cok[a] ? d : 0.f;
         }
@@ -526,6 +636,15 @@
         }
       }
   }
+}
+
+template <int C1B, int C2B, int C3B, int NS, int LAYER, int NSF>
+__global__ __launch_bounds__(kFT, ((LAYER == 3 ? C1B * C2B * C3B <= 2 : C1B * C2B == 1) ? 2 : 1)) void sa_train_bwd_kernel(SaBwdArgs p) {
+  sa_train_bwd_pass<C1B, C2B, C3B, NS, LAYER, NSF, false>(p);
+}
+template <int C1B, int C2B, int C3B, int NS, int LAYER>
+__global__ __launch_bounds__(kFT, ((LAYER == 3 ? C1B * C2B * C3B <= 2 && C2B <= C1B : C1B * C2B == 1) ? 2 : 1)) void sa_train_bwd_y2_kernel(SaBwdArgs p) {
+  sa_train_bwd_pass<C1B, C2B, C3B, NS, LAYER, NS, true>(p);
 }
 
 __global__ __launch_bounds__(256) void sa_geom_sums_kernel(const int* __restrict__ offsets, const int* __restrict__ slots, const float* __restrict__ xyz,
@@ -787,13 +906,13 @@
 
 }
 
-MVP_API int mvp_sa_train_forward_f32(int stage, const float* zf, const float* xyz, const float* centre, const int64_t* index, const float* wxyz,
+MVP_API int mvp_sa_train_forward_y2_f32(int stage, const float* zf, const float* xyz, const float* centre, const int64_t* index, const float* wxyz,
                                      int64_t B, int64_t N, int64_t M, int64_t K, int64_t C1, const float* bn1_mean, const float* bn1_invstd,
                                      const float* bn1_gamma, const float* bn1_beta, const float* W2, int64_t C2, const float* bn2_mean,
                                      const float* bn2_invstd, const float* bn2_gamma, const float* bn2_beta, const float* W3, int64_t C3,
                                      double* stat, float eps, float momentum, float* mean, float* invstd, float* running_mean,
                                      float* running_var, int64_t* num_batches_tracked, float* ymax, float* ymin, uint8_t* amax,
-                                     uint8_t* amin, mvp_stream_t stream) {
+                                     uint8_t* amin, float* Y2, mvp_stream_t stream) {
   MVP_NONNULL(stat);
   MVP_NONNULL(mean);
   MVP_NONNULL(invstd);
@@ -813,33 +932,50 @@
   const int ns = mlp_fwd_pieces();
   SaLevel lv;
   const int rc = sa_level(zf, true, xyz, centre, index, wxyz, B, N, M, K, C1, {bn1_mean, bn1_invstd, bn1_gamma, bn1_beta}, W2, C2, C3,
-                          sizes, ns != 0 && (uintptr_t)zf % 16 == 0, &lv);
+                          sizes, ns != 0 && (uintptr_t)zf % 16 == 0, &lv, Y2);
   if (rc != MVP_OK || lv.s.G == 0) return rc;
   SaFwdArgs a{lv.s, W2, {bn2_mean, bn2_invstd, bn2_gamma, bn2_beta}, W3, (int)C2, (int)C3, stat,
-              BnFinalize{B * M * K, eps, momentum, mean, invstd, running_mean, running_var, num_batches_tracked}, ymax, ymin, amax, amin, 0};
-  const int64_t lds = (int64_t)ns * 2048 * (lv.c1b * lv.c2b + (stage == 3 ? lv.c2b * lv.c3b : 0)) + 32 * 1024;
-  const unsigned grid = sa_grid(lv.s.G, lds, 4, 1024, &a.tiles_per_wg);
+              BnFinalize{B * M * K, eps, momentum, mean, invstd, running_mean, running_var, num_batches_tracked}, ymax, ymin, amax, amin, Y2, 0};
+  const bool load = Y2 && stage == 3;
+  const int64_t lds_re = (int64_t)ns * 2048 * (lv.c1b * lv.c2b + (stage == 3 ? lv.c2b * lv.c3b : 0)) + 32 * 1024;
+  const int64_t lds = load ? (int64_t)ns * 2048 * lv.c2b * lv.c3b + 18 * 1024 + 2048 * lv.c3b + 1024 : lds_re;
+  const unsigned grid = sa_grid(lv.s.G, lds, std::max<int64_t>(1, std::min<int64_t>(4, (150 * 1024) / lds_re)), 1024, &a.tiles_per_wg);
   hipStream_t s = static_cast<hipStream_t>(stream);
-  auto launch = [&](auto shapes, auto st) {
+  auto launch = [&](auto shapes, auto st, auto y2m) {
     return sa_pick(shapes, {lv.c1b, lv.c2b, lv.c3b}, [&](auto sh) {
       sa_pick(SaPieces{}, {ns}, [&](auto pc) {
-        hipLaunchKernelGGL((sa_train_fwd_kernel<decltype(sh)::v[0], decltype(sh)::v[1], decltype(sh)::v[2], decltype(pc)::v[0], decltype(st)::v[0]>),
-                           dim3(grid), dim3(kFT), 0, s, a);
+        constexpr int c1 = decltype(sh)::v[0], c2 = decltype(sh)::v[1], c3 = decltype(sh)::v[2], np = decltype(pc)::v[0], sg = decltype(st)::v[0];
+        constexpr int ym = decltype(y2m)::v[0];
+        if constexpr (ym == kY2Recompute) hipLaunchKernelGGL((sa_train_fwd_kernel<c1, c2, c3, np, sg>), dim3(grid), dim3(kFT), 0, s, a);
+        else hipLaunchKernelGGL((sa_train_fwd_y2_kernel<c1, c2, c3, np, sg, ym>), dim3(grid), dim3(kFT), 0, s, a);
       });
     });
   };
-  const bool found = stage == 3 ? launch(SaShapes3{}, SaRow<3>{}) : launch(SaShapes2{}, SaRow<2>{});
+  const bool found = stage == 3 ? (Y2 ? launch(SaShapes3{}, SaRow<3>{}, SaRow<kY2Load>{}) : launch(SaShapes3{}, SaRow<3>{}, SaRow<kY2Recompute>{}))
+                                : (Y2 ? launch(SaShapes2{}, SaRow<2>{}, SaRow<kY2Store>{}) : launch(SaShapes2{}, SaRow<2>{}, SaRow<kY2Recompute>{}));
   return found ? mvp_launch_status() : MVP_EUNSUPPORTED;
 }
 
-MVP_API int mvp_sa_train_backward_f32(int layer, const float* zf, const float* xyz, const float* centre, const int64_t* index,
+MVP_API int mvp_sa_train_forward_f32(int stage, const float* zf, const float* xyz, const float* centre, const int64_t* index, const float* wxyz,
+                                     int64_t B, int64_t N, int64_t M, int64_t K, int64_t C1, const float* bn1_mean, const float* bn1_invstd,
+                                     const float* bn1_gamma, const float* bn1_beta, const float* W2, int64_t C2, const float* bn2_mean,
+                                     const float* bn2_invstd, const float* bn2_gamma, const float* bn2_beta, const float* W3, int64_t C3,
+                                     double* stat, float eps, float momentum, float* mean, float* invstd, float* running_mean,
+                                     float* running_var, int64_t* num_batches_tracked, float* ymax, float* ymin, uint8_t* amax,
+                                     uint8_t* amin, mvp_stream_t stream) {
+  return mvp_sa_train_forward_y2_f32(stage, zf, xyz, centre, index, wxyz, B, N, M, K, C1, bn1_mean, bn1_invstd, bn1_gamma, bn1_beta, W2, C2, bn2_mean,
+                                     bn2_invstd, bn2_gamma, bn2_beta, W3, C3, stat, eps, momentum, mean, invstd, running_mean, running_var,
+                                     num_batches_tracked, ymax, ymin, amax, amin, nullptr, stream);
+}
+
+MVP_API int mvp_sa_train_backward_y2_f32(int layer, const float* zf, const float* xyz, const float* centre, const int64_t* index,
                                       const float* wxyz, int64_t B, int64_t N, int64_t M, int64_t K, int64_t C1, const float* bn1_mean,
                                       const float* bn1_invstd, const float* bn1_gamma, const float* bn1_beta, const float* W2, int64_t C2,
                                       const float* bn2_mean, const float* bn2_invstd, const float* bn2_gamma, const float* bn2_beta,
                                       const float* W3, int64_t C3, const float* mean_i, const float* invstd_i, const float* gamma_i,
                                       const double* stat_i, float* dgamma_i, float* dbeta_i, int training, const float* G,
                                       const float* pool_dout, const float* pool_out, const uint8_t* pool_arg, float* dW, int64_t lddw,
-                                      float* dZ, double* stat_prev, float* tsum, mvp_stream_t stream) {
+                                      float* dZ, double* stat_prev, float* tsum, const float* Y2, mvp_stream_t stream) {
   MVP_NONNULL(mean_i);
   MVP_NONNULL(invstd_i);
   MVP_NONNULL(gamma_i);
@@ -865,29 +1001,45 @@
   const int ns = mlp_bwd_pieces();
   SaLevel lv;
   const int rc = sa_level(zf, true, xyz, centre, index, wxyz, B, N, M, K, C1, {bn1_mean, bn1_invstd, bn1_gamma, bn1_beta}, W2, C2, C3,
-                          sizes, ns != 0 && (uintptr_t)zf % 16 == 0 && (uintptr_t)dZ % 16 == 0, &lv);
+                          sizes, ns != 0 && (uintptr_t)zf % 16 == 0 && (uintptr_t)dZ % 16 == 0, &lv, Y2);
   if (rc != MVP_OK || lv.s.G == 0) return rc;
   SaBwdArgs a{lv.s, W2, {bn2_mean, bn2_invstd, bn2_gamma, bn2_beta}, W3, (int)C2, (int)C3, mean_i, invstd_i, gamma_i, stat_i,
               dbeta_i ? dgamma_i : nullptr, dbeta_i, training ? 1.0f / (float)(B * M * K) : 0.f, G, pool_dout, pool_out, pool_arg, dW, (int)lddw, dZ,
-              stat_prev, tsum, 0};
+              stat_prev, tsum, Y2, 0};
   const int c1b = lv.c1b, c2b = lv.c2b, c3b = lv.c3b;
   const int cb = layer == 3 ? c3b : c2b, cpb = layer == 3 ? c2b : c1b;
-  const int nsf = (mlp_fwd_pieces() == 3) ? 3 : ns;
-  const int64_t lds = (int64_t)2048 * (nsf * c1b * c2b + ns * ((layer == 3 ? c2b * c3b : 0) + cb * cpb)) + 32 * 1024;
-  const bool narrow = layer == 3 ? c1b * c2b * c3b <= 2 : c1b * c2b == 1;
+  const int nsf = (mlp_fwd_pieces() == 3 && !Y2) ? 3 : ns;
+  const int64_t lds = (int64_t)2048 * ((Y2 ? 0 : nsf * c1b * c2b) + ns * ((layer == 3 ? c2b * c3b : 0) + cb * cpb)) + 32 * 1024;
+  const bool narrow = layer == 3 ? c1b * c2b * c3b <= 2 && (!Y2 || c2b <= c1b) : c1b * c2b == 1;
   const unsigned grid = sa_grid(lv.s.G, lds, narrow ? 2 : 1, 1024, &a.tiles_per_wg);
   hipStream_t s = static_cast<hipStream_t>(stream);
   using Pieces = SaTable<SaRow<1, 1>, SaRow<1, 3>, SaRow<2, 2>, SaRow<2, 3>, SaRow<3, 3>>;
-  auto launch = [&](auto shapes, auto ly) {
+  using PiecesY2 = SaTable<SaRow<1, 1>, SaRow<2, 2>, SaRow<3, 3>>;
+  auto launch = [&](auto shapes, auto ly, auto pieces, auto y2l) {
     return sa_pick(shapes, {c1b, c2b, c3b}, [&](auto sh) {
-      sa_pick(Pieces{}, {ns, nsf}, [&](auto pc) {
-        hipLaunchKernelGGL((sa_train_bwd_kernel<decltype(sh)::v[0], decltype(sh)::v[1], decltype(sh)::v[2], decltype(pc)::v[0], decltype(ly)::v[0],
-                                                decltype(pc)::v[1]>), dim3(grid), dim3(kFT), 0, s, a);
+      sa_pick(pieces, {ns, nsf}, [&](auto pc) {
+        constexpr int c1 = decltype(sh)::v[0], c2 = decltype(sh)::v[1], c3 = decltype(sh)::v[2], np = decltype(pc)::v[0], lr = decltype(ly)::v[0];
+        if constexpr (decltype(y2l)::v[0] != 0) hipLaunchKernelGGL((sa_train_bwd_y2_kernel<c1, c2, c3, np, lr>), dim3(grid), dim3(kFT), 0, s, a);
+        else hipLaunchKernelGGL((sa_train_bwd_kernel<c1, c2, c3, np, lr, decltype(pc)::v[1]>), dim3(grid), dim3(kFT), 0, s, a);
       });
     });
   };
-  const bool found = layer == 3 ? launch(SaShapes3{}, SaRow<3>{}) : launch(SaShapes2{}, SaRow<2>{});
+  const bool found = layer == 3 ? (Y2 ? launch(SaShapes3{}, SaRow<3>{}, PiecesY2{}, SaRow<1>{}) : launch(SaShapes3{}, SaRow<3>{}, Pieces{}, SaRow<0>{}))
+                                : (Y2 ? launch(SaShapes2{}, SaRow<2>{}, PiecesY2{}, SaRow<1>{}) : launch(SaShapes2{}, SaRow<2>{}, Pieces{}, SaRow<0>{}));
   return found ? mvp_launch_status() : MVP_EUNSUPPORTED;
+}
+
+MVP_API int mvp_sa_train_backward_f32(int layer, const float* zf, const float* xyz, const float* centre, const int64_t* index,
+                                      const float* wxyz, int64_t B, int64_t N, int64_t M, int64_t K, int64_t C1, const float* bn1_mean,
+                                      const float* bn1_invstd, const float* bn1_gamma, const float* bn1_beta, const float* W2, int64_t C2,
+                                      const float* bn2_mean, const float* bn2_invstd, const float* bn2_gamma, const float* bn2_beta,
+                                      const float* W3, int64_t C3, const float* mean_i, const float* invstd_i, const float* gamma_i,
+                                      const double* stat_i, float* dgamma_i, float* dbeta_i, int training, const float* G,
+                                      const float* pool_dout, const float* pool_out, const uint8_t* pool_arg, float* dW, int64_t lddw,
+                                      float* dZ, double* stat_prev, float* tsum, mvp_stream_t stream) {
+  return mvp_sa_train_backward_y2_f32(layer, zf, xyz, centre, index, wxyz, B, N, M, K, C1, bn1_mean, bn1_invstd, bn1_gamma, bn1_beta, W2, C2, bn2_mean,
+                                      bn2_invstd, bn2_gamma, bn2_beta, W3, C3, mean_i, invstd_i, gamma_i, stat_i, dgamma_i, dbeta_i, training, G,
+                                      pool_dout, pool_out, pool_arg, dW, lddw, dZ, stat_prev, tsum, nullptr, stream);
 }
 
 MVP_API int mvp_sa_geom_sums_f32(const int32_t* offsets, const int32_t* slots, const float* xyz, const float* centre, int64_t B, int64_t N,
diff --git a/mvpnet_amd/rows.py b/mvpnet_amd/rows.py
--- a/mvpnet_amd/rows.py
+++ b/mvpnet_amd/rows.py
@@ -1201,6 +1201,14 @@
 
 SA_TRAIN_FUSED = os.environ.get('MVP_SA_TRAIN', '1') != '0'
 
+SA_Y2 = os.environ.get('MVP_SA_Y2', '1') != '0'
+SA_Y2_PASSES = {(1, 1, 2): ('fwd3', 'bwd3'), (2, 2, 4): ('fwd3', 'bwd3')}
+
+
+def sa_y2_passes(c1, c2, c3):
+    blocks = lambda c: 1 if c <= 32 else 2 if c <= 64 else 4
+    return SA_Y2_PASSES.get((blocks(c1), blocks(c2), blocks(c3)), ()) if SA_Y2 else ()
+
 
 STATS1_REPLICAS = int(os.environ.get('MVP_SA_STATS1_REPLICAS', '16'))
 
@@ -1251,15 +1259,18 @@
         L.call('mvp_sa_train_stats1_ws_f32', zf, L.ptr(zf), L.ptr(dsum), L.ptr(wxyz), L.ptr(gsum), B, N, M, K, C1, L.ptr(stat1), L.ptr(zsum), float(e1),
                float(mo1), L.ptr(m1), L.ptr(i1), L.ptr(rm1), L.ptr(rv1), L.ptr(nb1), L.ptr(rep1) if nrep else None, rep1.numel())
         level = (L.ptr(zf), L.ptr(xyz), L.ptr(centre), L.ptr(index), L.ptr(wxyz), B, N, M, K, C1, L.ptr(m1), L.ptr(i1), L.ptr(g1), L.ptr(b1), L.ptr(W2), C2)
+        loads = sa_y2_passes(C1, C2, C3)
+        y2 = torch.empty((B * M * K, C2), dtype=torch.float32, device=dev) if loads else None
         L.call('mvp_sa_train_forward_f32', xyz, 2, *level, None, None, None, None, None, 0, L.ptr(stat2), float(e2), float(mo2), L.ptr(m2), L.ptr(i2),
-               L.ptr(rm2), L.ptr(rv2), L.ptr(nb2), None, None, None, None, prec=prec)
+               L.ptr(rm2), L.ptr(rv2), L.ptr(nb2), None, None, None, None, prec=prec, y2=L.ptr(y2))
         G = B * M
         ymax = torch.empty((G, C3), dtype=torch.float32, device=dev)
         ymin = torch.empty((G, C3), dtype=torch.float32, device=dev)
         amax = torch.empty((G, C3), dtype=torch.uint8, device=dev)
         amin = torch.empty((G, C3), dtype=torch.uint8, device=dev)
         L.call('mvp_sa_train_forward_f32', xyz, 3, *level, L.ptr(m2), L.ptr(i2), L.ptr(g2), L.ptr(b2), L.ptr(W3), C3, L.ptr(stat3), float(e3), float(mo3),
-               L.ptr(m3), L.ptr(i3), L.ptr(rm3), L.ptr(rv3), L.ptr(nb3), L.ptr(ymax), L.ptr(ymin), L.ptr(amax), L.ptr(amin), prec=prec)
+               L.ptr(m3), L.ptr(i3), L.ptr(rm3), L.ptr(rv3), L.ptr(nb3), L.ptr(ymax), L.ptr(ymin), L.ptr(amax), L.ptr(amin), prec=prec,
+               y2=L.ptr(y2) if 'fwd3' in loads else None)
         out = torch.empty((G, C3), dtype=torch.float32, device=dev)
         arg = torch.empty((G, C3), dtype=torch.uint8, device=dev)
         ysel = torch.empty((G, C3), dtype=torch.float32, device=dev)
@@ -1267,6 +1278,8 @@
                L.ptr(out), L.ptr(arg), L.ptr(ysel))
         ctx.save_for_backward(zf, xyz, centre, index, offsets, slots, dsum, gsum, zsum, wxyz, mi, g1, b1, g2, b2, g3, W2, W3, out, arg, ysel)
         ctx.dims = (B, N, M, K, C1, C2, C3)
+        ctx.y2 = y2 if 'bwd3' in loads or 'bwd2' in loads else None
+        ctx.y2_loads = loads
         return out.view(B, M, C3)
 
     @staticmethod
@@ -1294,13 +1307,18 @@
         dg3, db3 = dgb[2 * (C1 + C2):2 * (C1 + C2) + C3], dgb[2 * (C1 + C2) + C3:]
         level = (L.ptr(zf), L.ptr(xyz), L.ptr(centre), L.ptr(index), L.ptr(wxyz), B, N, M, K, C1, L.ptr(m1), L.ptr(i1), L.ptr(g1), L.ptr(b1), L.ptr(W2), C2,
                  L.ptr(m2), L.ptr(i2), L.ptr(g2), L.ptr(b2))
+        y2, ctx.y2 = ctx.y2, None
         dz2 = torch.empty((R, C2), dtype=torch.float32, device=dev)
         L.call('mvp_sa_train_backward_f32', zf, 3, *level, L.ptr(W3), C3, L.ptr(m3), L.ptr(i3), L.ptr(g3), L.ptr(stat3), L.ptr(dg3), L.ptr(db3), 1, None,
-               L.ptr(g), L.ptr(out), L.ptr(arg), L.ptr(dW3), C2, L.ptr(dz2), L.ptr(stat2), None, prec=prec)
+               L.ptr(g), L.ptr(out), L.ptr(arg), L.ptr(dW3), C2, L.ptr(dz2), L.ptr(stat2), None, prec=prec,
+               y2=L.ptr(y2) if 'bwd3' in ctx.y2_loads else None)
+        if 'bwd2' not in ctx.y2_loads:
+            y2 = None
         dz1 = torch.empty((R, C1), dtype=torch.float32, device=dev)
         L.call('mvp_sa_train_backward_f32', zf, 2, *level, None, 0, L.ptr(m2), L.ptr(i2), L.ptr(g2), L.ptr(stat2), L.ptr(dg2), L.ptr(db2), 1, L.ptr(dz2),
-               None, None, None, L.ptr(dW2), C1, L.ptr(dz1), L.ptr(stat1), L.ptr(tsum), prec=prec)
-        del dz2
+               None, None, None, L.ptr(dW2), C1, L.ptr(dz1), L.ptr(stat1), L.ptr(tsum), prec=prec,
+               y2=L.ptr(y2) if 'bwd2' in ctx.y2_loads else None)
+        del dz2, y2
         numel = 1
         for d in ctx.w_shape:
             numel *= d
```

After: 5383 chunks/s, median of 6. 2.5% higher.
